# second-state/qwen3_asr_rs

Hardware: AMD Instinct MI355X
Metric: audio-seconds/sec (RTFx) Qwen3-ASR-0.6B greedy, 30s clips (higher is better)
Workload: dtype bf16; 1 GPU; Qwen3-ASR-0.6b bf16, batch=1 x 30s synthetic 16kHz clip per GPU, 100 new tokens (fixed, EOS ignored); clips_per_gpu=1, parallelism=dp1 (independent utterances per GPU, no data-path collective)

## Files before the change

qwen3_asr_rs_amd/build.py:

```python
from __future__ import annotations

import hashlib
import os
import re
import subprocess
import sys
from concurrent.futures import ThreadPoolExecutor

HERE = os.path.dirname(os.path.abspath(__file__))
ROOT = os.path.dirname(HERE)
CSRC = os.path.join(HERE, "csrc")
OBJ_DIR = os.path.join(ROOT, "build", "q3asr")
LIB_DIR = os.path.join(HERE, "lib")
LIB_PATH = os.path.join(LIB_DIR, "libq3asr_hip.so")
BIN_DIR = os.path.join(HERE, "bin")
CLI_PATH = os.path.join(BIN_DIR, "asr")

SOURCES = ["engine.cpp", "model.cpp", "k_gemm.hip", "k_mel.hip", "k_conv1.hip", "k_norm.hip", "k_attn.hip", "k_decode.hip", "k_gemv.hip", "k_dattn.hip", "k_fattn.hip", "k_skinny.hip", "k_gemm16.hip", "k_gemm256.hip", "k_peaks.hip", "k_align.hip",
           "host_audio.cpp", "host_text.cpp", "host_abi.cpp", "host_align.cpp", "group.cpp", "ops.cpp", "k_ops.hip"]
HEADERS = ["dev.h", "kernels.h", "argmax.h", "model.h", "json.h", "host.h", "ops.h", "unicode_tables.h", os.path.join("..", "..", "include", "q3asr.h"),
           os.path.join("..", "..", "include", "q3asr_ops.h")]
HIPCC = os.environ.get("HIPCC", "/opt/rocm/bin/hipcc")
FLAGS = ["--offload-arch=gfx950", "-O3", "-std=c++17", "-fPIC", "-fno-slp-vectorize", "-Wall", "-Wno-unused-function", "-Wno-unused-variable"]
HIP_FLAGS = ["-x", "hip", "-save-temps=obj"]

_VARIANT = os.environ.get("Q3A_BUILD_VARIANT", "")
if _VARIANT:
    FLAGS = FLAGS + os.environ.get("Q3A_BUILD_DEFINES", "").split()
    OBJ_DIR = OBJ_DIR + "_" + _VARIANT
    LIB_PATH = os.path.join(LIB_DIR, f"libq3asr_hip_{_VARIANT}.so")
    CLI_PATH = os.path.join(BIN_DIR, f"asr_{_VARIANT}")


def _hash(paths) -> str:
    h = hashlib.sha1()
    for p in paths:
        with open(p, "rb") as f:
            h.update(f.read())
    h.update(" ".join(FLAGS + HIP_FLAGS).encode())
    return h.hexdigest()


def have_hipcc() -> bool:
    return os.path.exists(HIPCC) and os.access(HIPCC, os.X_OK)


def _compile(src: str, hdr_hash: str, force: bool) -> str:
    spath = os.path.join(CSRC, src)
    obj = os.path.join(OBJ_DIR, src + ".o")
    stamp = obj + ".stamp"
    want = _hash([spath]) + hdr_hash
    is_hip = src.endswith(".hip")
    if not force and os.path.exists(obj) and os.path.exists(stamp) and open(stamp).read() == want and (not is_hip or os.path.exists(isa_path(src))):
        return obj
    cmd = [HIPCC] + FLAGS + (HIP_FLAGS if is_hip else []) + ["-c", spath, "-o", obj]
    r = subprocess.run(cmd, capture_output=True, text=True)
    if r.returncode != 0:
        raise RuntimeError(f"hipcc failed for {src}:\n{r.stdout}\n{r.stderr}")
    if r.stderr.strip():
        sys.stderr.write(r.stderr)
    with open(stamp, "w") as f:
        f.write(want)
    return obj


_LABEL = re.compile(r"^([A-Za-z_][\w$]*):")
_PK_F32 = re.compile(r"^\s*(v_pk_(?:mul|fma|add)_f32)\b.*\bop_sel:\[([01,]+)\]")


def isa_path(src: str) -> str:
    return os.path.join(OBJ_DIR, os.path.splitext(src)[0] + "-hip-amdgcn-amd-amdhsa-gfx950.s")


def scan_isa(paths=None):
    if paths is None:
        paths = [isa_path(s) for s in SOURCES if s.endswith(".hip")]
    found = []
    for path in paths:
        kernel = "?"
        if not os.path.exists(path):
            raise RuntimeError(f"scan_isa: {path} is missing -- rebuild (`python -m qwen3_asr_rs_amd.build`): the device assembly is kept by "
                               "-save-temps=obj and an object without it is treated as stale")
        with open(path) as f:
            for line in f:
                lm = _LABEL.match(line)
                if lm:
                    kernel = lm.group(1)
                m = _PK_F32.match(line)
                if m and "1" in m.group(2):
                    found.append((os.path.basename(path), kernel, line.strip()))
    return found


def build(force: bool = False, verbose: bool = True) -> str:
    os.makedirs(OBJ_DIR, exist_ok=True)
    os.makedirs(LIB_DIR, exist_ok=True)
    hdr_hash = _hash([os.path.join(CSRC, h) for h in HEADERS])
    with ThreadPoolExecutor(max_workers=min(8, len(SOURCES))) as ex:
        objs = list(ex.map(lambda s: _compile(s, hdr_hash, force), SOURCES))
    hazards = scan_isa()
    if hazards and os.environ.get("Q3A_ALLOW_ISA_HAZARD", "0") in ("", "0"):
        lines = "\n".join(f"  {f}: {k}: {i}" for f, k, i in hazards[:20])
        raise RuntimeError(f"{len(hazards)} packed fp32 instruction(s) with an op_sel bit set in the device code (csrc/dev.h: unsafe on gfx950; "
                           f"Q3A_ALLOW_ISA_HAZARD=1 builds experiment variants anyway):\n{lines}")
    link_stamp = LIB_PATH + ".stamp"
    want = _hash(objs)
    if force or not os.path.exists(LIB_PATH) or not os.path.exists(link_stamp) or open(link_stamp).read() != want:
        cmd = [HIPCC, "--offload-arch=gfx950", "-shared", "-fPIC", "-o", LIB_PATH] + objs + ["-ldl", "-lpthread"]
        r = subprocess.run(cmd, capture_output=True, text=True)
        if r.returncode != 0:
            raise RuntimeError(f"link failed:\n{r.stdout}\n{r.stderr}")
        with open(link_stamp, "w") as f:
            f.write(want)
        if verbose:
            print(f"[q3asr build] linked {LIB_PATH}")
    elif verbose:
        print(f"[q3asr build] up to date: {LIB_PATH}")
    os.makedirs(BIN_DIR, exist_ok=True)
    cli_src = os.path.join(CSRC, "asr_main.cpp")
    cli_stamp = CLI_PATH + ".stamp"
    cli_want = _hash([cli_src, os.path.join(ROOT, "include", "q3asr.h")]) + want
    if force or not os.path.exists(CLI_PATH) or not os.path.exists(cli_stamp) or open(cli_stamp).read() != cli_want:
        cmd = ["g++", "-O2", "-std=c++17", "-o", CLI_PATH, cli_src, "-L" + LIB_DIR, "-lq3asr_hip", "-Wl,-rpath,$ORIGIN/../lib",
               "-Wl,-rpath,/opt/rocm/lib"]
        r = subprocess.run(cmd, capture_output=True, text=True)
        if r.returncode != 0:
            raise RuntimeError(f"CLI link failed:\n{r.stdout}\n{r.stderr}")
        with open(cli_stamp, "w") as f:
            f.write(cli_want)
        if verbose:
            print(f"[q3asr build] linked {CLI_PATH}")
    return LIB_PATH


if __name__ == "__main__":
    build(force="--force" in sys.argv)
```

qwen3_asr_rs_amd/csrc/engine.cpp:

```cpp
#include <hip/hip_runtime.h>

#include <sched.h>

#include <algorithm>
#include <atomic>
#include <chrono>
#include <cmath>
#include <cstdio>
#include <cstring>
#include <map>
#include <memory>
#include <mutex>
#include <string>
#include <thread>
#include <vector>

#include "../../include/q3asr.h"
#include "kernels.h"
#include "model.h"

using namespace q3a;

namespace {

thread_local std::string g_last_error;

#define HIPCHK(expr)                                                                                    \
  do {                                                                                                  \
    hipError_t _e = (expr);                                                                             \
    if (_e != hipSuccess)                                                                               \
      fail(std::string("HIP error: ") + hipGetErrorString(_e) + " at " + __FILE__ + ":" + std::to_string(__LINE__) + " (" #expr ")"); \
  } while (0)
#define KCHK(expr)                                  \
  do {                                              \
    const char* _m = (expr);                        \
    if (_m) fail(std::string("kernel launch: ") + _m); \
  } while (0)

constexpr int kAudioPad = 151676, kEos0 = 151643, kEos1 = 151645;
constexpr int kGemvMaxSeq = 2;

struct DevBuf {
  void* p = nullptr;
  size_t cap = 0;
  bool grew = false;
  void ensure(size_t bytes) {
    if (bytes <= cap) return;
    if (p) (void)hipFree(p);
    p = nullptr;
    cap = 0;
    size_t want = (bytes + 255) & ~size_t(255);
    HIPCHK(hipMalloc(&p, want));
    cap = want;
    grew = true;
  }
  void release() {
    if (p) (void)hipFree(p);
    p = nullptr;
    cap = 0;
  }
  template <typename T> T* as() const { return reinterpret_cast<T*>(p); }
};

template <typename T>
void upload(DevBuf& b, const std::vector<T>& v, hipStream_t s) {
  b.ensure(std::max<size_t>(v.size() * sizeof(T), 16));
  if (!v.empty()) HIPCHK(hipMemcpyAsync(b.p, v.data(), v.size() * sizeof(T), hipMemcpyHostToDevice, s));
}

struct ProfEvent {
  int kclass;
  double bytes;
  hipEvent_t a, b;
};

}

namespace q3a {
void set_thread_error(const std::string& msg) { g_last_error = msg; }
}
namespace q3a {
Knobs& knobs() {
  static Knobs k;
  static std::once_flag once;
  std::call_once(once, [] {
    auto env = [](const char* name, std::atomic<int>& dst) { if (const char* e = getenv(name)) dst.store(atoi(e)); };
    env("Q3A_GEMM256_MIN_TILES", k.gemm256_min_tiles);
    env("Q3A_GEMM256_PERSIST", k.gemm256_persist);
    env("Q3A_GEMM256_GROUP_M", k.gemm256_group_m);
    env("Q3A_DATTN_BATCHED_MIN_WGS", k.dattn_batched_min_wgs);
    env("Q3A_DECODE_GROUP", k.decode_group_size);
    env("Q3A_DECODE_PARALLEL", k.decode_parallel_groups);
    env("Q3A_FUSE_QKROPE", k.fuse_qkrope);
    env("Q3A_SKINNY_Q", k.skinny_q);
    env("Q3A_EOS_RUN_AHEAD", k.eos_run_ahead);
    env("Q3A_SKINNY_GLU_HP3", k.skinny_glu_hp3);
    env("Q3A_LM_HEAD_PRUNE", k.lm_head_prune);
  });
  return k;
}
}

struct q3a_engine {
  Dims d;
  ArenaLayout L;
  q3a_opts opts{};
  int device = 0;
  hipStream_t stream = nullptr;
  uint8_t* arena = nullptr;
  bool own_arena = false;
  uint32_t arena_flags = 0;
  std::string err;

  DevBuf dft, filt_t, pos_emb, rope_cos, rope_sin;
  int rope_positions = 0;

  int B = 0;
  std::vector<int64_t> n_samples, pcm_off, mel_off;
  std::vector<int> n_frames, n_chunks, T, tok_off;
  int total_chunks = 0, total_T = 0, max_frames = 0;
  bool have_mel = false, have_enc = false, have_prefill = false;
  std::vector<int> P, seq_off;
  int total_P = 0, max_ctx = 0, max_new = 0;
  std::vector<AttnSeg> enc_segs_h;
  int enc_max_seg = 0;

  DevBuf pcm, d_pcm_off, d_n_samples, d_mel_off, d_n_frames, mel, gmax, d_chunk_utt, d_chunk_frame0;
  DevBuf conv1, conv2, conv3, conv3_rowmap, convout_rowmap;
  DevBuf enc_x, enc_ln, enc_qkv, enc_ctx, enc_ffn, enc_segs, audio_embeds;
  DevBuf ids, audio_rowmap, row_seq, row_pos, dec_segs, last_rows;
  DevBuf dec_x, dec_ln, dec_qkv, dec_ctx, dec_act, kcache, vcache;
  DevBuf x_dec, d_pos, next_tok, out_ids, step_count, done, s_ln, s_qkv, s_ctx, s_act, logits, forced_tok, part_val, part_idx;
  DevBuf blk_lo, blk_hi;
  DevBuf part_sum, out_lp;
  DevBuf lm_q, lm_qs;
  int lm_q_cols = 0;
  DevBuf prune_stats;
  DevBuf attn_pm, attn_pl, attn_po;
  DevBuf nn_x, nn_ss;
  DevBuf rope_cur;
  DevBuf enc_ctx16, dec_ctx16;
  DevBuf dec_q16;
  int n_cu = 256;
  DevBuf n_done;
  int* host_prog = nullptr;
  int* host_prog_dev = nullptr;
  DevBuf zero_page;
  int part_stride = 0, attn_nsplit = 0;
  size_t kv_layer_elems = 0;

  int gsize = 32;
  int k_parallel_groups = 1, k_skinny_q = 1, k_dattn_batched_min_wgs = 128, k_skinny_glu_hp3 = 1, k_lm_head_prune = 1;
  std::vector<hipStream_t> chain_streams;
  std::vector<hipEvent_t> join_ev;
  hipEvent_t fork_ev = nullptr;

  static constexpr size_t kGraphCacheMax = 16;
  std::vector<std::pair<std::string, hipGraphExec_t>> graph_cache;
  int pos_hi_ = 0, live_nsplit_ = 0;
  int min_P_ = 0;

  hipStream_t up_stream = nullptr;
  void* pin_p = nullptr;
  size_t pin_cap = 0;
  std::vector<hipEvent_t> up_ev;
  hipEvent_t up_t0 = nullptr, up_t1 = nullptr;
  q3a_io_timings io{};
  bool geom_valid = false;

  q3a_timings timings{};
  hipEvent_t ev[5] = {nullptr, nullptr, nullptr, nullptr, nullptr};
  std::vector<ProfEvent>* prof = nullptr;
  std::map<std::string, DevBuf> taps;
  std::map<std::string, size_t> tap_bytes;

  bool precise() const { return opts.precise != 0; }
  bool token_lp() const { return opts.token_logprobs != 0; }
  bool kv_f32() const { return opts.precise != 0; }
  size_t kv_elem() const { return kv_f32() ? 4 : 2; }
  size_t act_elem() const { return precise() ? 4 : 2; }
  template <typename T> const T* w(uint64_t off) const { return reinterpret_cast<const T*>(arena + off); }
  const float* wf(uint64_t off) const { return w<float>(off); }
  const uint16_t* wh(uint64_t off) const { return w<uint16_t>(off); }

  static bool light_tap(const char* name) { return strcmp(name, "dec_last_hidden") == 0 || strcmp(name, "head_in") == 0; }
  void tap(const char* name, const void* ptr, size_t bytes) {
    if (!opts.debug_taps || bytes == 0 || (opts.debug_taps == 2 && !light_tap(name))) return;
    DevBuf& t = taps[name];
    t.ensure(bytes);
    tap_bytes[name] = bytes;
    HIPCHK(hipMemcpyAsync(t.p, ptr, bytes, hipMemcpyDeviceToDevice, stream));
  }
  void tap_act(const char* name, const void* ptr, size_t elems) {
    if (!opts.debug_taps || elems == 0 || opts.debug_taps == 2) return;
    if (precise()) return tap(name, ptr, elems * 4);
    DevBuf& t = taps[name];
    t.ensure(elems * 4);
    tap_bytes[name] = elems * 4;
    KCHK(launch_from_bf16((const uint16_t*)ptr, t.as<float>(), elems, stream));
  }

  void act_gemm(const DevBuf& x, int lda, const uint16_t* W, int M, int N, int K, const GemmEpilogue& ep, bool glu) {
    if (precise()) KCHK(launch_gemm(x.as<float>(), lda, W, M, N, K, ep, glu, true, stream));
    else KCHK(launch_gemm16(x.as<uint16_t>(), lda, W, M, N, K, ep, glu, stream));
  }
  void act_conv(const DevBuf& x, int imgs, int H, int Wd, int C, const uint16_t* W, int Cout, const GemmEpilogue& ep) {
    if (precise()) KCHK(launch_conv3x3s2_gemm(x.as<float>(), imgs, H, Wd, C, W, Cout, ep, true, stream));
    else KCHK(launch_conv3x3s2_gemm16(x.as<uint16_t>(), zero_page.as<uint16_t>(), imgs, H, Wd, C, W, Cout, ep, stream));
  }
  void act_out(GemmEpilogue& ep, const DevBuf& buf) const {
    if (precise()) ep.out = buf.as<float>(); else ep.out16 = buf.as<uint16_t>();
  }
  uint16_t* act16(const DevBuf& buf) const { return precise() ? nullptr : buf.as<uint16_t>(); }

  template <class F> void timed(int kclass, double bytes, F&& fn) {
    if (!prof) {
      fn();
      return;
    }
    ProfEvent pe{kclass, bytes, nullptr, nullptr};
    HIPCHK(hipEventCreate(&pe.a));
    HIPCHK(hipEventCreate(&pe.b));
    HIPCHK(hipEventRecord(pe.a, stream));
    fn();
    HIPCHK(hipEventRecord(pe.b, stream));
    prof->push_back(pe);
  }

  void init_common(const std::string& model_dir, int dev, const q3a_opts* o) {
    if (o) opts = *o; else q3a_opts_default(&opts);
    if (opts.max_new_tokens <= 0) opts.max_new_tokens = 4096;
    d = parse_config_file(model_dir + "/config.json");
    validate_dims(d);
    L = plan_arena(d);
    device = dev;
    int n_dev = 0;
    hipError_t e = hipGetDeviceCount(&n_dev);
    if (e != hipSuccess || n_dev == 0)
      fail("no HIP device available: libq3asr_hip has no CPU fallback (hipGetDeviceCount: " + std::string(hipGetErrorString(e)) + ")");
    if (dev < 0 || dev >= n_dev) fail("device index out of range");
    HIPCHK(hipSetDevice(dev));
    KCHK(skinny_init());
    (void)hipDeviceGetAttribute(&n_cu, hipDeviceAttributeMultiprocessorCount, dev);
    HIPCHK(hipStreamCreateWithFlags(&stream, hipStreamNonBlocking));
    for (auto& x : ev) HIPCHK(hipEventCreate(&x));
    HIPCHK(hipHostMalloc((void**)&host_prog, 64, hipHostMallocMapped));
    memset(host_prog, 0, 64);
    HIPCHK(hipHostGetDevicePointer((void**)&host_prog_dev, host_prog, 0));
    n_done.ensure(64);
    prune_stats.ensure(8);
    HIPCHK(hipMemsetAsync(prune_stats.p, 0, 8, stream));
  }

  void init_tables() {
    auto dftm = make_dft_matrix(400, 416);
    auto filt = make_mel_filterbank_T(d.n_mels, 400, 16000, 202);
    auto pe = make_sinusoid_rows(d.tokens_per_chunk(), d.enc_d);
    upload(dft, dftm, stream);
    upload(filt_t, filt, stream);
    upload(pos_emb, pe, stream);
    zero_page.ensure(256);
    HIPCHK(hipMemsetAsync(zero_page.p, 0, 256, stream));
    ensure_rope(8192);
    HIPCHK(hipStreamSynchronize(stream));
  }

  void ensure_rope(int n_pos) {
    if (n_pos <= rope_positions) return;
    int n = std::max(n_pos, 8192);
    std::vector<float> c, s;
    make_rope_tables(n, d.head_dim, d.rope_theta, c, s);
    HIPCHK(hipStreamSynchronize(stream));
    upload(rope_cos, c, stream);
    upload(rope_sin, s, stream);
    HIPCHK(hipStreamSynchronize(stream));
    rope_positions = n;
  }

  void init_lm_head_q() {
    const int cols = lm_head_q_cols(d.hidden);
    if (precise() || d.aligner() || cols == 0 || d.hidden % 8 != 0) return;
    lm_q.ensure((size_t)d.vocab * cols);
    lm_qs.ensure((size_t)d.vocab * 16);
    KCHK(launch_lm_head_quantize(wh(L.lm_head), d.vocab, d.hidden, lm_q.as<int8_t>(), lm_qs.as<float>(), stream));
    HIPCHK(hipStreamSynchronize(stream));
    lm_q_cols = cols;
  }

  void check_arena_header() {
    ArenaHeader h;
    HIPCHK(hipMemcpy(&h, arena, sizeof(h), hipMemcpyDeviceToHost));
    if (h.magic != kArenaMagic || h.version != kArenaVersion) fail("weight arena: bad magic/version");
    if (h.total_bytes != L.total) fail("weight arena: size does not match config.json");
    arena_flags = h.flags;
  }

  void set_batch(const int64_t* ns, int b) {
    have_mel = have_enc = have_prefill = false;
    if (b <= 0) { B = 0; fail("batch must be >= 1"); }
    if (geom_valid && b == B && (int)n_samples.size() == b && std::equal(ns, ns + b, n_samples.begin())) return;
    geom_valid = false;
    B = 0;
    for (int u = 0; u < b; ++u)
      if (ns[u] < 161) fail("utterance too short: reflection padding needs more than 160 samples (src/mel.rs:63-65)");
    n_samples.assign(ns, ns + b);
    pcm_off.resize(b); mel_off.resize(b); n_frames.resize(b); n_chunks.resize(b); T.resize(b); tok_off.resize(b);
    std::vector<int> chunk_utt, chunk_frame0, convout_map, conv3_map;
    enc_segs_h.clear();
    int64_t po = 0, mo = 0;
    int tok = 0;
    total_chunks = 0; max_frames = 0; enc_max_seg = 0;
    const int cf = d.chunk_frames(), tpc = d.tokens_per_chunk(), cpw = d.chunks_per_window();
    for (int u = 0; u < b; ++u) {
      pcm_off[u] = po;
      po += (ns[u] + 3) & ~int64_t(3);
      int F = (int)((ns[u] + 159) / 160);
      n_frames[u] = F;
      max_frames = std::max(max_frames, F);
      mel_off[u] = mo;
      mo += (int64_t)F * d.n_mels;
      int nc = (F + cf - 1) / cf;
      n_chunks[u] = nc;
      tok_off[u] = tok;
      std::vector<int> valid(nc);
      for (int c = 0; c < nc; ++c) {
        int frames = std::min(cf, F - c * cf);
        valid[c] = Dims::feat_len(frames);
        chunk_utt.push_back(u);
        chunk_frame0.push_back(c * cf);
        for (int t = 0; t < tpc; ++t) convout_map.push_back(t < valid[c] ? tok + t : -1);
        tok += valid[c];
      }
      T[u] = tok - tok_off[u];
      int t0 = tok_off[u];
      if (nc <= cpw) {
        enc_segs_h.push_back(AttnSeg{t0, T[u], (int64_t)t0 * 3 * d.enc_d});
        enc_max_seg = std::max(enc_max_seg, T[u]);
      } else {
        for (int c0 = 0; c0 < nc; c0 += cpw) {
          int len = 0;
          for (int c = c0; c < std::min(nc, c0 + cpw); ++c) len += valid[c];
          enc_segs_h.push_back(AttnSeg{t0, len, (int64_t)t0 * 3 * d.enc_d});
          enc_max_seg = std::max(enc_max_seg, len);
          t0 += len;
        }
      }
      total_chunks += nc;
    }
    total_T = tok;
    const int f3 = d.freq3();
    conv3_map.resize((size_t)total_chunks * f3 * tpc);
    for (int c = 0; c < total_chunks; ++c)
      for (int f = 0; f < f3; ++f)
        for (int t = 0; t < tpc; ++t) conv3_map[((size_t)c * f3 + f) * tpc + t] = (c * tpc + t) * f3 + f;
    pcm.ensure((size_t)po * 4);
    upload(d_pcm_off, pcm_off, stream);
    upload(d_n_samples, n_samples, stream);
    upload(d_mel_off, mel_off, stream);
    upload(d_n_frames, n_frames, stream);
    upload(d_chunk_utt, chunk_utt, stream);
    upload(d_chunk_frame0, chunk_frame0, stream);
    upload(convout_rowmap, convout_map, stream);
    upload(conv3_rowmap, conv3_map, stream);
    upload(enc_segs, enc_segs_h, stream);
    mel.ensure((size_t)mo * 4);
    gmax.ensure((size_t)b * 4);
    HIPCHK(hipStreamSynchronize(stream));
    B = b;
    geom_valid = true;
  }

  void upload_pcm(const float* host, const int64_t* ns, int b) {
    set_batch(ns, b);
    int64_t src = 0;
    for (int u = 0; u < b; ++u) {
      HIPCHK(hipMemcpyAsync(pcm.as<float>() + pcm_off[u], host + src, (size_t)ns[u] * 4, hipMemcpyHostToDevice, stream));
      src += ns[u];
    }
    HIPCHK(hipStreamSynchronize(stream));
  }

  void upload_ptrs_and_mel(const float* const* ptrs, const int64_t* ns, int b) {
    const auto w0 = std::chrono::steady_clock::now();
    set_batch(ns, b);
    static const int mode = [] { const char* e = getenv("Q3A_UPLOAD_MODE"); return e ? atoi(e) : 1; }();
    static const int thr_env = [] { const char* e = getenv("Q3A_UPLOAD_THREADS"); return e ? atoi(e) : -1; }();
    static const int pieces_env = [] { const char* e = getenv("Q3A_UPLOAD_PIECES"); return e ? atoi(e) : 8; }();
    io = q3a_io_timings{};
    io.mode = mode;
    HIPCHK(hipEventRecord(ev[0], stream));
    const size_t total = (size_t)(pcm_off[b - 1] + ((ns[b - 1] + 3) & ~int64_t(3))) * 4;
    bool staged = mode != 0;
    if (staged && total > pin_cap) {
      if (up_stream) HIPCHK(hipStreamSynchronize(up_stream));
      if (pin_p) (void)hipHostFree(pin_p);
      pin_p = nullptr; pin_cap = 0;
      const size_t want = (total + (size_t(1) << 20) - 1) & ~((size_t(1) << 20) - 1);
      if (hipHostMalloc(&pin_p, want, hipHostMallocDefault) == hipSuccess && pin_p) pin_cap = want;
      else { (void)hipGetLastError(); pin_p = nullptr; staged = false; io.mode = 0; }
    }
    if (!staged) {
      for (int u = 0; u < b; ++u)
        HIPCHK(hipMemcpyAsync(pcm.as<float>() + pcm_off[u], ptrs[u], (size_t)ns[u] * 4, hipMemcpyHostToDevice, stream));
      HIPCHK(hipStreamSynchronize(stream));
// ... 104 lines not shown
    ChunkTable ct{d_chunk_utt.as<int>(), d_chunk_frame0.as<int>()};
    KCHK(launch_conv1(mel.as<float>(), d_mel_off.as<int64_t>(), d_n_frames.as<int>(), ct, total_chunks, d.n_mels,
                      d.chunk_frames(), wf(L.conv1_w), wf(L.conv1_b), C, conv1.as<float>(), stream, act16(conv1)));
    tap_act("conv1", conv1.p, nch * H1 * W1 * C);
    {
      GemmEpilogue ep;
      act_out(ep, conv2); ep.ldo = C; ep.bias = wf(L.conv2_b); ep.act = 1;
      act_conv(conv1, total_chunks, H1, W1, C, wh(L.conv2_w), C, ep);
      tap_act("conv2", conv2.p, nch * H2 * W2 * C);
    }
    {
      GemmEpilogue ep;
      act_out(ep, conv3); ep.ldo = C; ep.bias = wf(L.conv3_b); ep.act = 1; ep.rowmap = conv3_rowmap.as<int>();
      act_conv(conv2, total_chunks, H2, W2, C, wh(L.conv3_w), C, ep);
      tap_act("conv3", conv3.p, nch * H3 * W3 * C);
    }
    {
      GemmEpilogue ep;
      ep.out = enc_x.as<float>(); ep.ldo = D;
      ep.bias = (arena_flags & kFlagConvOutBias) ? wf(L.conv_out_b) : nullptr;
      ep.rowmap = convout_rowmap.as<int>();
      ep.addend = pos_emb.as<float>(); ep.addend_period = W3;
      act_gemm(conv3, H3 * C, wh(L.conv_out_w), total_chunks * W3, D, H3 * C, ep, false);
      tap("enc_in", enc_x.p, Tt * D * 4);
    }
    AttnArgs at{};
    at.q = enc_qkv.as<float>(); at.q_rs = 3 * D;
    at.k = enc_qkv.as<float>() + D; at.v = enc_qkv.as<float>() + 2 * D; at.kv_hs = 64; at.kv_rs = 3 * D;
    if (qkv16) {
      at.q16 = enc_qkv.as<uint16_t>();
      at.k = enc_qkv.as<uint16_t>() + D; at.v = enc_qkv.as<uint16_t>() + 2 * D;
    }
    at.o = enc_ctx.as<float>(); at.o_rs = D;
    at.o16 = valu_attn ? nullptr : enc_ctx.as<uint16_t>();
    at.segs = enc_segs.as<AttnSeg>(); at.n_segs = (int)enc_segs_h.size(); at.max_len = enc_max_seg;
    at.n_kv_heads = d.enc_heads; at.scale_div = 8.0f;
    const DevBuf& ctx_in = (valu_attn && !sp) ? enc_ctx16 : enc_ctx;
    for (int li = 0; li < d.enc_layers; ++li) {
      const EncLayerOff& e = L.enc[li];
      KCHK(launch_layernorm(enc_x.as<float>(), wf(e.ln1_w), wf(e.ln1_b), enc_ln.as<float>(), total_T, D, 1e-5f, stream, act16(enc_ln)));
      {
        GemmEpilogue ep; ep.ldo = 3 * D; ep.bias = wf(e.qkv_b);
        if (qkv16) ep.out16 = enc_qkv.as<uint16_t>(); else ep.out = enc_qkv.as<float>();
        act_gemm(enc_ln, D, wh(e.qkv_w), total_T, 3 * D, D, ep, false);
      }
      if (valu_attn) {
        KCHK(launch_attn_enc(at, stream));
        if (!sp) KCHK(launch_to_bf16(enc_ctx.as<float>(), enc_ctx16.as<uint16_t>(), Tt * D, stream));
      } else {
        KCHK(launch_fattn_enc(at, stream));
      }
      {
        GemmEpilogue ep; ep.out = enc_x.as<float>(); ep.ldo = D; ep.bias = wf(e.out_b); ep.resid = enc_x.as<float>();
        act_gemm(ctx_in, D, wh(e.out_w), total_T, D, D, ep, false);
      }
      KCHK(launch_layernorm(enc_x.as<float>(), wf(e.ln2_w), wf(e.ln2_b), enc_ln.as<float>(), total_T, D, 1e-5f, stream, act16(enc_ln)));
      {
        GemmEpilogue ep; act_out(ep, enc_ffn); ep.ldo = Fn; ep.bias = wf(e.fc1_b); ep.act = 1;
        act_gemm(enc_ln, D, wh(e.fc1_w), total_T, Fn, D, ep, false);
      }
      {
        GemmEpilogue ep; ep.out = enc_x.as<float>(); ep.ldo = D; ep.bias = wf(e.fc2_b); ep.resid = enc_x.as<float>();
        act_gemm(enc_ffn, Fn, wh(e.fc2_w), total_T, D, Fn, ep, false);
      }
      if (li == 0) tap("enc_layer0", enc_x.p, Tt * D * 4);
      static const bool enc_layer_taps = [] { const char* e = getenv("Q3A_DEBUG_LAYER_TAPS"); return e && atoi(e) != 0; }();
      if (enc_layer_taps && opts.debug_taps == 1) {
        char name[32];
        snprintf(name, sizeof(name), "E%02d_x", li);
        tap(name, enc_x.p, Tt * D * 4);
      }
    }
    tap("enc_last", enc_x.p, Tt * D * 4);
    KCHK(launch_layernorm(enc_x.as<float>(), wf(L.ln_post_w), wf(L.ln_post_b), enc_ln.as<float>(), total_T, D, 1e-5f, stream, act16(enc_ln)));
    {
      GemmEpilogue ep; act_out(ep, enc_ffn); ep.ldo = D; ep.bias = wf(L.proj1_b); ep.act = 1;
      act_gemm(enc_ln, D, wh(L.proj1_w), total_T, D, D, ep, false);
    }
    {
      GemmEpilogue ep; ep.out = audio_embeds.as<float>(); ep.ldo = d.enc_out; ep.bias = wf(L.proj2_b);
      act_gemm(enc_ffn, D, wh(L.proj2_w), total_T, d.enc_out, D, ep, false);
    }
    tap("audio_embeds", audio_embeds.p, Tt * d.enc_out * 4);
    HIPCHK(hipGetLastError());
    have_enc = true;
  }

  void setup_prompts(const int32_t* ids_h, const int32_t* lens, int b, int max_new_req, bool before_encoder = false) {
    if (!have_enc && !before_encoder) fail("q3a_prefill: no encoder output (call q3a_encode first)");
    if (b != B) fail("q3a_prefill: batch size differs from the encoded batch");
    P.assign(lens, lens + b);
    seq_off.resize(b);
    std::vector<int> rowseq, rowpos, amap((size_t)total_T, -1), last(b);
    int off = 0, maxP = 0;
    for (int s = 0; s < b; ++s) {
      seq_off[s] = off;
      int na = 0;
      for (int i = 0; i < P[s]; ++i) {
        rowseq.push_back(s);
        rowpos.push_back(i);
        int id = ids_h[off + i];
        if (id < 0 || id >= d.vocab) fail("q3a_prefill: token id out of range");
        if (id == kAudioPad) {
          if (na >= T[s]) fail("q3a_prefill: more <|audio_pad|> tokens than encoder tokens");
          amap[(size_t)tok_off[s] + na] = off + i;
          ++na;
        }
      }
      if (na != T[s]) fail("q3a_prefill: number of <|audio_pad|> tokens does not match the encoder output length");
      if (P[s] <= 0) fail("q3a_prefill: empty prompt");
      last[s] = off + P[s] - 1;
      off += P[s];
      maxP = std::max(maxP, P[s]);
    }
    total_P = off;
    max_new = std::min(std::max(max_new_req, 1), opts.max_new_tokens);
    max_ctx = ((maxP + max_new + 1 + 127) / 128) * 128;
    pos_hi_ = maxP;
    min_P_ = *std::min_element(P.begin(), P.end());
    {
      static const int pad = [] { const char* e = getenv("Q3A_CTX_PAD"); return e ? atoi(e) : 0; }();
      if (pad > 0) max_ctx += (pad + 127) / 128 * 128;
    }
    ensure_rope(max_ctx + 1);
    std::vector<int> ids_v(ids_h, ids_h + total_P);
    std::vector<AttnSeg> segs(b);
    for (int s = 0; s < b; ++s)
      segs[s] = AttnSeg{seq_off[s], P[s], (int64_t)s * d.n_kv * max_ctx * 128};
    upload(ids, ids_v, stream);
    upload(row_seq, rowseq, stream);
    upload(row_pos, rowpos, stream);
    upload(audio_rowmap, amap, stream);
    upload(last_rows, last, stream);
    upload(dec_segs, segs, stream);
    upload(d_pos, P, stream);
    const size_t Pt = (size_t)total_P, H = d.hidden;
    const bool valu_attn = kv_f32() || opts.valu_attention;
    dec_x.ensure(Pt * H * 4); dec_ln.ensure(Pt * H * act_elem()); dec_qkv.ensure(Pt * d.qkv_dim() * 4);
    dec_ctx.ensure(Pt * d.q_dim() * (valu_attn ? 4 : act_elem())); dec_act.ensure(Pt * d.inter * act_elem());
    if (!valu_attn) dec_q16.ensure(Pt * d.q_dim() * 2);
    if (valu_attn && !precise()) dec_ctx16.ensure(Pt * d.q_dim() * 2);
    kv_layer_elems = (size_t)b * d.n_kv * max_ctx * 128;
    kcache.ensure(kv_layer_elems * d.dec_layers * kv_elem());
    vcache.ensure(kv_layer_elems * d.dec_layers * kv_elem());
    rope_cur.ensure((size_t)b * 128 * 4);
    {
      Knobs& kn = knobs();
      const int gs = kn.decode_group_size.load();
      gsize = (gs >= 1 && gs <= 32) ? gs : 32;
      k_parallel_groups = kn.decode_parallel_groups.load(); k_skinny_q = kn.skinny_q.load();
      k_dattn_batched_min_wgs = kn.dattn_batched_min_wgs.load();
      k_skinny_glu_hp3 = kn.skinny_glu_hp3.load();
      k_lm_head_prune = kn.lm_head_prune.load();
    }
    const size_t ng = (size_t)n_groups(b);
    nn_x.ensure(ng * 32 * H * 2); nn_ss.ensure((size_t)ng * (H / 8) * 32 * 4);
    x_dec.ensure((size_t)b * H * 4); next_tok.ensure((size_t)b * 4); forced_tok.ensure((size_t)b * 4);
    out_ids.ensure((size_t)b * max_new * 4); step_count.ensure((size_t)b * 4); done.ensure((size_t)b);
    s_ln.ensure((size_t)b * H * 4); s_qkv.ensure((size_t)b * d.qkv_dim() * 4); s_ctx.ensure(ng * 32 * d.q_dim() * 4);
    s_act.ensure(ng * 32 * d.inter * 4); logits.ensure((size_t)b * d.vocab * 4);
    part_stride = std::max(128, (d.vocab + 3) / 4);
    part_val.ensure((size_t)b * part_stride * 4); part_idx.ensure((size_t)b * part_stride * 4);
    if (token_lp()) { part_sum.ensure((size_t)b * part_stride * 4); out_lp.ensure((size_t)b * max_new * 4); }
    {
      const size_t nblk4 = ((size_t)(d.vocab + 15) / 16 + 3) & ~size_t(3);
      blk_lo.ensure(nblk4 * 4); blk_hi.ensure(nblk4 * 4);
    }
    attn_nsplit = (max_ctx + dattn_keys_per_split(kv_f32()) - 1) / dattn_keys_per_split(kv_f32());
    attn_pm.ensure((size_t)b * d.n_q * attn_nsplit * 4); attn_pl.ensure((size_t)b * d.n_q * attn_nsplit * 4);
    attn_po.ensure((size_t)b * d.n_q * attn_nsplit * 128 * 4);
    HIPCHK(hipMemsetAsync(step_count.p, 0, (size_t)b * 4, stream));
    HIPCHK(hipMemsetAsync(done.p, 0, (size_t)b, stream));
    HIPCHK(hipMemsetAsync(n_done.p, 0, 64, stream));
    HIPCHK(hipMemsetAsync(out_ids.p, 0, (size_t)b * max_new * 4, stream));
    if (token_lp()) HIPCHK(hipMemsetAsync(out_lp.p, 0, (size_t)b * max_new * 4, stream));
    HIPCHK(hipStreamSynchronize(stream));
    for (auto cs : chain_streams) HIPCHK(hipStreamSynchronize(cs));
    __atomic_store_n(&host_prog[0], 0, __ATOMIC_RELAXED);
    __atomic_store_n(&host_prog[1], 0, __ATOMIC_RELAXED);
    drain_retired_graphs();
    {
      bool any = false;
      for (auto* sb : step_bufs()) { any = any || sb->grew; sb->grew = false; }
      if (any) drop_graphs();
    }
  }

  std::vector<DevBuf*> step_bufs() {
    return {&kcache, &vcache, &x_dec, &d_pos, &next_tok, &out_ids, &step_count, &done, &s_ln, &s_qkv, &s_ctx, &s_act, &logits,
            &part_val, &part_idx, &part_sum, &out_lp, &blk_lo, &blk_hi, &prune_stats, &attn_pm, &attn_pl, &attn_po, &nn_x, &nn_ss, &rope_cur, &rope_cos, &rope_sin, &n_done, &forced_tok};
  }
  std::vector<const DevBuf*> step_bufs() const {
    auto v = const_cast<q3a_engine*>(this)->step_bufs();
    return std::vector<const DevBuf*>(v.begin(), v.end());
  }

  void* kc_layer(int l) { return (uint8_t*)kcache.p + (size_t)l * kv_layer_elems * kv_elem(); }
  void* vc_layer(int l) { return (uint8_t*)vcache.p + (size_t)l * kv_layer_elems * kv_elem(); }

  LmHeadPruneArgs prune_args(const GemvArgs& g) {
    LmHeadPruneArgs pa{};
    pa.g = g; pa.Wq = lm_q.as<int8_t>(); pa.qcols = lm_q_cols; pa.qs = lm_qs.as<float>();
    pa.blk_lo = blk_lo.as<float>(); pa.blk_hi = blk_hi.as<float>(); pa.stats = prune_stats.as<int>();
    return pa;
  }

  void run_head(int advance) {
    const int S = B, H = d.hidden, V = d.vocab;
    tap("head_in", x_dec.p, (size_t)S * H * 4);
    const double wbytes = 2.0 * V * H;
    int n_part = 0;
    const ArgmaxPartials part{part_val.as<float>(), part_idx.as<int>(), token_lp() ? part_sum.as<float>() : nullptr, part_stride};
    if (S <= kGemvMaxSeq) {
      GemvArgs g{};
      g.fast_math = precise() ? 0 : 1;
      g.x = x_dec.as<float>(); g.ldx = H; g.rms_w = wf(L.final_norm); g.eps = d.rms_eps;
      g.W = wh(L.lm_head); g.N = V; g.K = H; g.mode = 3; g.out = logits.as<float>(); g.ldo = V;
      g.part = part;
      LmHeadPruneArgs pa{};
      const bool prunable = S == 1 && !precise() && lm_q_cols > 0 && (pa = prune_args(g), !lm_head_prune_check(pa));
      if (prunable && opts.debug_taps == 1) {
        DevBuf& t = taps["lm_head_bound"];
        t.ensure((size_t)V * 8);
        tap_bytes["lm_head_bound"] = (size_t)V * 8;
        LmHeadPruneArgs pd = pa;
        pd.dbg = t.as<float>(); pd.stats = nullptr;
        KCHK(launch_lm_head_approx(pd, stream));
      }
      if (prunable && k_lm_head_prune && !head_logits_) {
        g.out = nullptr; pa.g.out = nullptr;
        n_part = lm_head_rescore_groups(g, n_cu);
        timed(Q3A_KC_GEMV_LM_HEAD, (double)V * lm_q_cols, [&] { KCHK(launch_lm_head_approx(pa, stream)); });
        timed(Q3A_KC_ARGMAX, 0, [&] { KCHK(launch_lm_head_rescore(pa, n_part, stream)); });
      } else {
        n_part = gemv_blocks(g);
        timed(Q3A_KC_GEMV_LM_HEAD, wbytes, [&] { KCHK(launch_gemv(g, S, stream)); });
      }
    } else if (!precise()) {
      timed(Q3A_KC_NORM, 0, [&] { KCHK(launch_rmsnorm(x_dec.as<float>(), wf(L.final_norm), s_ln.as<float>(), S, H, d.rms_eps, stream, s_ln.as<uint16_t>())); });
      GemmEpilogue ep; ep.out = logits.as<float>(); ep.ldo = V;
      if (S <= 32 && V % 4 == 0 && H % 64 == 0 && part_stride >= (V + 63) / 64) {
        ep.part = part;
        if (!head_logits_) ep.out = nullptr;
        n_part = (V + 63) / 64;
        timed(Q3A_KC_GEMM, wbytes, [&] { KCHK(launch_gemm16(s_ln.as<uint16_t>(), H, wh(L.lm_head), S, V, H, ep, false, stream)); });
      } else {
        timed(Q3A_KC_GEMM, wbytes, [&] { KCHK(launch_gemm16(s_ln.as<uint16_t>(), H, wh(L.lm_head), S, V, H, ep, false, stream)); });
        n_part = 128;
        timed(Q3A_KC_ARGMAX, 0, [&] { KCHK(launch_argmax_partials(logits.as<float>(), V, S, part, n_part, stream)); });
      }
    } else {
      timed(Q3A_KC_NORM, 0, [&] { KCHK(launch_rmsnorm(x_dec.as<float>(), wf(L.final_norm), s_ln.as<float>(), S, H, d.rms_eps, stream)); });
      timed(Q3A_KC_GEMM, wbytes, [&] { batched_proj(s_ln.as<float>(), H, wh(L.lm_head), V, H, nullptr, 0, logits.as<float>(), V, nullptr); });
      n_part = 128;
      timed(Q3A_KC_ARGMAX, 0, [&] { KCHK(launch_argmax_partials(logits.as<float>(), V, S, part, n_part, stream)); });
    }
    FinalizeArgs f{};
    f.part = part; f.n_part = n_part; f.out_lp = part.sum ? out_lp.as<float>() : nullptr;
    f.V = V; f.next_tok = next_tok.as<int>(); f.out_ids = out_ids.as<int>();
    f.out_stride = max_new; f.step_count = step_count.as<int>(); f.pos = d_pos.as<int>(); f.advance = advance;
    f.done = done.as<uint8_t>(); f.n_done = n_done.as<int>(); f.n_seq = S; f.host_progress = host_prog_dev; f.embed = wh(L.embed); f.H = H; f.x_next = x_dec.as<float>(); f.eos0 = kEos0; f.eos1 = kEos1;
    f.cos_t = rope_cos.as<float>(); f.sin_t = rope_sin.as<float>(); f.rope_cur = rope_cur.as<float>();
    f.nn = first_layer_norm_out();
    timed(Q3A_KC_ARGMAX, 0, [&] { KCHK(launch_argmax_finalize(f, S, stream)); });
  }

  void run_prefill() {
    run_prefill_layers();
    const int H = d.hidden;
    KCHK(launch_gather_rows(dec_x.as<float>(), last_rows.as<int>(), B, H, x_dec.as<float>(), stream));
    tap("dec_last_hidden", x_dec.p, (size_t)B * H * 4);
    run_head(0);
    tap("logits", logits.p, (size_t)B * d.vocab * 4);
    HIPCHK(hipGetLastError());
    have_prefill = true;
  }

  void run_prefill_layers() {
    const int H = d.hidden, I = d.inter, QD = d.q_dim(), QKV = d.qkv_dim();
    const bool sp = precise();
    KCHK(launch_embed(ids.as<int>(), total_P, wh(L.embed), H, kAudioPad, dec_x.as<float>(), stream));
    scatter_audio_rows();
    tap("dec_embed", dec_x.p, (size_t)total_P * H * 4);
    AttnArgs at{};
    at.q = dec_qkv.as<float>(); at.q_rs = QKV; at.kv_hs = (int64_t)max_ctx * 128; at.kv_rs = 128;
    at.o = dec_ctx.as<float>(); at.o_rs = QD; at.segs = dec_segs.as<AttnSeg>(); at.n_segs = B;
    at.max_len = *std::max_element(P.begin(), P.end()); at.n_kv_heads = d.n_kv;
    at.scale_div = sqrtf((float)d.head_dim);
    const bool valu_attn = kv_f32() || opts.valu_attention;
    at.o16 = valu_attn ? nullptr : dec_ctx.as<uint16_t>();
    if (!valu_attn) { at.q16 = dec_q16.as<uint16_t>(); at.q_rs = QD; }
    const DevBuf& ctx_in = (valu_attn && !sp) ? dec_ctx16 : dec_ctx;
    const bool qkv_bias = arena_flags & kFlagDecQkvBias, o_bias = arena_flags & kFlagDecOBias, mlp_bias = arena_flags & kFlagDecMlpBias;
    const bool fuse_rope = knobs().fuse_qkrope.load() != 0 && !valu_attn && !precise() && d.head_dim == 128 && gemm256_eligible(total_P, QKV, H) && H % 64 == 0;
    for (int li = 0; li < d.dec_layers; ++li) {
      const DecLayerOff& l = L.dec[li];
      KCHK(launch_rmsnorm(dec_x.as<float>(), wf(l.in_ln), dec_ln.as<float>(), total_P, H, d.rms_eps, stream, act16(dec_ln)));
      RopeKvArgs rk{};
      rk.qkv = dec_qkv.as<float>(); rk.row_seq = row_seq.as<int>(); rk.row_pos = row_pos.as<int>();
      rk.q_norm = wf(l.q_norm); rk.k_norm = wf(l.k_norm); rk.eps = d.rms_eps;
      rk.cos_t = rope_cos.as<float>(); rk.sin_t = rope_sin.as<float>();
      rk.kcache = kc_layer(li); rk.vcache = vc_layer(li); rk.n_q = d.n_q; rk.n_kv = d.n_kv; rk.max_ctx = max_ctx;
      rk.q16 = valu_attn ? nullptr : dec_q16.as<uint16_t>();
      if (fuse_rope) {
        KCHK(launch_gemm256_qkrope(dec_ln.as<uint16_t>(), H, wh(l.qkv_w), total_P, H, qkv_bias ? wf(l.qkv_b) : nullptr, rk, stream));
      } else {
        GemmEpilogue ep; ep.out = dec_qkv.as<float>(); ep.ldo = QKV; ep.bias = qkv_bias ? wf(l.qkv_b) : nullptr;
        act_gemm(dec_ln, H, wh(l.qkv_w), total_P, QKV, H, ep, false);
        KCHK(launch_qknorm_rope_kv(rk, total_P, kv_f32(), stream));
      }
      at.k = kc_layer(li); at.v = vc_layer(li);
      static const bool layer_taps = [] { const char* e = getenv("Q3A_DEBUG_LAYER_TAPS"); return e && atoi(e) != 0; }();
      auto ltap = [&](const char* what, const void* ptr, size_t bytes) {
        if (!layer_taps || !opts.debug_taps) return;
        char name[32];
        snprintf(name, sizeof(name), "L%02d_%s", li, what);
        tap(name, ptr, bytes);
      };
      const size_t act_b = sp ? 4 : 2;
      if (fuse_rope) {
        ltap("qkvs", dec_qkv.p, std::min((size_t)1024, (size_t)total_P) * QKV * 4);
      }
      ltap("k", kc_layer(li), (size_t)B * d.n_kv * max_ctx * 128 * kv_elem());
      ltap("v", vc_layer(li), (size_t)B * d.n_kv * max_ctx * 128 * kv_elem());
      if (valu_attn) {
        KCHK(launch_attn_prefill(at, d.n_q / d.n_kv, kv_f32(), stream));
        if (!sp) KCHK(launch_to_bf16(dec_ctx.as<float>(), dec_ctx16.as<uint16_t>(), (size_t)total_P * QD, stream));
      } else {
        KCHK(launch_fattn_prefill(at, d.n_q / d.n_kv, stream));
      }
      ltap("attn", ctx_in.p, (size_t)total_P * QD * act_b);
      {
        GemmEpilogue ep; ep.out = dec_x.as<float>(); ep.ldo = H; ep.resid = dec_x.as<float>(); ep.bias = o_bias ? wf(l.o_b) : nullptr;
        act_gemm(ctx_in, QD, wh(l.o_w), total_P, H, QD, ep, false);
      }
      ltap("o", dec_x.p, (size_t)total_P * H * 4);
      KCHK(launch_rmsnorm(dec_x.as<float>(), wf(l.post_ln), dec_ln.as<float>(), total_P, H, d.rms_eps, stream, act16(dec_ln)));
      ltap("ln2", dec_ln.p, (size_t)total_P * H * act_b);
      {
        GemmEpilogue ep; act_out(ep, dec_act); ep.ldo = I; ep.bias = mlp_bias ? wf(l.gu_b) : nullptr;
        act_gemm(dec_ln, H, wh(l.gu_w), total_P, 2 * I, H, ep, true);
      }
      ltap("act", dec_act.p, (size_t)total_P * I * act_b);
      {
        GemmEpilogue ep; ep.out = dec_x.as<float>(); ep.ldo = H; ep.resid = dec_x.as<float>(); ep.bias = mlp_bias ? wf(l.down_b) : nullptr;
        act_gemm(dec_act, I, wh(l.down_w), total_P, H, I, ep, false);
      }
      ltap("x", dec_x.p, (size_t)total_P * H * 4);
      if (li == 0) tap("dec_layer0", dec_x.p, (size_t)total_P * H * 4);
    }
  }

  void require_asr(const char* what) const {
    if (d.aligner()) fail(std::string(what) + ": this engine holds a forced aligner (classify_num in config.json); use q3a_align*");
  }
  void require_aligner(const char* what) const {
    if (!d.aligner()) fail(std::string(what) + ": not a forced-aligner checkpoint (config.json has no thinker_config.classify_num)");
  }
  std::vector<int> align_marker_rows(const int32_t* ids_h, const int32_t* lens, int b, int stride, int32_t* counts) const {
    std::vector<int> rows;
    int off = 0;
    for (int s = 0; s < b; ++s) {
      int n = 0;
      for (int i = 0; i < lens[s]; ++i)
        if (ids_h[off + i] == d.timestamp_token_id) { rows.push_back(off + i); ++n; }
      if (n > stride)
        fail("q3a_align: utterance " + std::to_string(s) + " has " + std::to_string(n) + " timestamp markers, more than stride " + std::to_string(stride));
      counts[s] = n;
      off += lens[s];
    }
    return rows;
  }
  void run_align(const std::vector<int>& rows, const int32_t* counts, int stride, int32_t* out_classes, float* logits_out) {
    const int M = (int)rows.size(), N = d.classify_num, H = d.hidden;
    have_prefill = false;
    HIPCHK(hipEventRecord(ev[2], stream));
    run_prefill_layers();
    HIPCHK(hipEventRecord(ev[3], stream));
    if (M > 0) {
      upload(align_rows, rows, stream);
      const int planes = precise() ? 2 : 1, n_part = align_head_parts(N);
      align_xn.ensure((size_t)planes * align_rows_padded(M) * H * 2);
      align_pval.ensure((size_t)M * n_part * 4); align_pidx.ensure((size_t)M * n_part * 4);
      align_cls.ensure((size_t)M * 4);
      if (logits_out) align_logits.ensure((size_t)M * N * 4);
      AlignHeadArgs a{};
      a.x = dec_x.as<float>(); a.ldx = H; a.rows = align_rows.as<int>(); a.M = M;
      a.norm_w = wf(L.final_norm); a.eps = d.rms_eps; a.W = wh(L.lm_head); a.N = N; a.K = H;
      a.planes = planes; a.xn = align_xn.as<uint16_t>();
      a.part = ArgmaxPartials{align_pval.as<float>(), align_pidx.as<int>(), nullptr, n_part};
      a.classes = align_cls.as<int>();
      a.logits = logits_out ? align_logits.as<float>() : nullptr; a.ldl = N;
      KCHK(launch_align_head(a, stream));
    }
    HIPCHK(hipEventRecord(ev[4], stream));
    HIPCHK(hipStreamSynchronize(stream));
    HIPCHK(hipGetLastError());
    std::vector<int> cls((size_t)M);
    if (M > 0) HIPCHK(hipMemcpy(cls.data(), align_cls.p, (size_t)M * 4, hipMemcpyDeviceToHost));
    if (M > 0 && logits_out) HIPCHK(hipMemcpy(logits_out, align_logits.p, (size_t)M * N * 4, hipMemcpyDeviceToHost));
    for (int s = 0, k = 0; s < B; ++s)
      for (int i = 0; i < counts[s]; ++i) out_classes[(size_t)s * stride + i] = cls[k++];
    float ms = 0.f;
    HIPCHK(hipEventElapsedTime(&ms, ev[2], ev[4])); timings.prefill_ms = ms;
    HIPCHK(hipEventElapsedTime(&ms, ev[3], ev[4])); align_head_ms = ms;
    timings.decode_ms = 0.f; timings.decode_steps = 0; timings.batch = B; timings.total_audio_tokens = total_T;
    timings.total_prompt_tokens = total_P;
  }
  DevBuf align_rows, align_xn, align_pval, align_pidx, align_cls, align_logits;
  float align_head_ms = 0.f;

  void scatter_audio_rows();

  bool prenorm_path() const { return B > kGemvMaxSeq && !precise(); }
  bool skinny_q() const {
    auto whole = [](int K) { const int st = K / 32, per = (st + 7) / 8, unr = per <= 2 ? 2 : per <= 4 ? 4 : per <= 8 ? 8 : 12; return K % 256 == 0 && per % unr == 0; };
// ... 9 lines not shown
  float* s_act_g(int g) const { return s_act.as<float>() + (size_t)g * 32 * d.inter; }
  NextNormOut first_layer_norm_out() const {
    NextNormOut nn{};
    if (prenorm_path()) {
      nn.next_w = wf(L.dec[0].in_ln); nn.next_xw16f = nn_x.as<uint16_t>(); nn.next_ss = nn_ss.as<float>(); nn.nparts = nn_parts();
      nn.group_stride_x = (long)nn_x_stride(); nn.group_stride_ss = (long)nn_ss_stride(); nn.group_size = gsize;
    }
    return nn;
  }

  void batched_proj(const float* x, int ldx, const uint16_t* W, int N, int K, const float* bias, int mode, float* out,
                    int ldo, const float* resid) {
    const int S = B;
    if (S <= 32) {
      SkinnyArgs sk{};
      sk.fast_math = precise() ? 0 : 1;
      sk.x = x; sk.ldx = ldx; sk.S = S; sk.W = W; sk.N = N; sk.K = K; sk.bias = bias; sk.mode = mode; sk.out = out; sk.ldo = ldo; sk.resid = resid;
      KCHK(launch_skinny(sk, precise(), stream));
    } else {
      GemmEpilogue ep; ep.out = out; ep.ldo = ldo; ep.bias = bias; ep.resid = (mode == 1) ? resid : nullptr;
      KCHK(launch_gemm(x, ldx, W, S, N, K, ep, mode == 2, precise(), stream));
    }
  }

  void decode_layer(int li, int grp, int s0, int S, hipStream_t ks) {
    const int H = d.hidden, I = d.inter, QD = d.q_dim(), QKV = d.qkv_dim();
    const bool qkv_bias = arena_flags & kFlagDecQkvBias, o_bias = arena_flags & kFlagDecOBias, mlp_bias = arena_flags & kFlagDecMlpBias;
    const bool gemv = B <= kGemvMaxSeq;
    const DecLayerOff& l = L.dec[li];
    float* const x = x_dec.as<float>() + (size_t)s0 * H;
    float* const qkv = s_qkv.as<float>() + (size_t)s0 * QKV;
    const size_t kv_seq = (size_t)d.n_kv * max_ctx * 128 * kv_elem();
    DecodeAttnArgs da{};
    da.qkv = qkv; da.pos = d_pos.as<int>() + s0; da.eps = d.rms_eps;
    da.rope_cur = rope_cur.as<float>() + (size_t)s0 * 128;
    da.pm = attn_pm.as<float>() + (size_t)s0 * d.n_q * attn_nsplit; da.pl = attn_pl.as<float>() + (size_t)s0 * d.n_q * attn_nsplit;
    da.po = attn_po.as<float>() + (size_t)s0 * d.n_q * attn_nsplit * 128; da.nsplit = live_nsplit_;
    da.n_q = d.n_q; da.n_kv = d.n_kv; da.max_ctx = max_ctx; da.scale_div = sqrtf((float)d.head_dim);
    da.q_norm = wf(l.q_norm); da.k_norm = wf(l.k_norm);
    da.kcache = (uint8_t*)kc_layer(li) + (size_t)s0 * kv_seq; da.vcache = (uint8_t*)vc_layer(li) + (size_t)s0 * kv_seq;
    if (gemv) {
      GemvArgs g{};
      g.fast_math = precise() ? 0 : 1;
      g.x = x; g.ldx = H; g.rms_w = wf(l.in_ln); g.eps = d.rms_eps; g.W = wh(l.qkv_w); g.N = QKV; g.K = H;
      g.bias = qkv_bias ? wf(l.qkv_b) : nullptr; g.mode = 0; g.out = qkv; g.ldo = QKV;
      timed(Q3A_KC_GEMV, 2.0 * QKV * H, [&] { KCHK(launch_gemv(g, S, ks)); });
      timed(Q3A_KC_DECODE_ATTN, 0, [&] { KCHK(launch_decode_attn(da, S, kv_f32(), ks)); });
      GemvArgs o{};
      o.fast_math = precise() ? 0 : 1;
      if (std::min(S, 4) * d.n_q * live_nsplit_ <= GEMV_ATTN_MAX_TABLE) {
        o.attn_pm = da.pm; o.attn_pl = da.pl; o.attn_po = da.po;
        o.attn_nsplit = live_nsplit_; o.attn_heads = d.n_q; o.attn_fast_exp = precise() ? 0 : 1;
      } else {
        timed(Q3A_KC_DECODE_ATTN, 0, [&] { KCHK(launch_attn_combine(da.pm, da.pl, da.po, live_nsplit_, S, d.n_q, s_ctx_g(grp), ks)); });
        o.x = s_ctx_g(grp);
      }
      o.ldx = QD; o.W = wh(l.o_w); o.N = H; o.K = QD; o.bias = o_bias ? wf(l.o_b) : nullptr;
      o.mode = 1; o.out = x; o.ldo = H; o.resid = x;
      timed(Q3A_KC_GEMV_O, 2.0 * H * QD, [&] { KCHK(launch_gemv(o, S, ks)); });
      GemvArgs u{};
      u.fast_math = precise() ? 0 : 1;
      u.x = x; u.ldx = H; u.rms_w = wf(l.post_ln); u.eps = d.rms_eps; u.W = wh(l.gu_w); u.N = 2 * I; u.K = H;
      u.bias = mlp_bias ? wf(l.gu_b) : nullptr; u.mode = 2; u.out = s_act_g(grp); u.ldo = I;
      timed(Q3A_KC_GEMV, 4.0 * I * H, [&] { KCHK(launch_gemv(u, S, ks)); });
      GemvArgs dn{};
      dn.fast_math = precise() ? 0 : 1;
      dn.x = s_act_g(grp); dn.ldx = I; dn.W = wh(l.down_w); dn.N = H; dn.K = I; dn.bias = mlp_bias ? wf(l.down_b) : nullptr;
      dn.mode = 1; dn.out = x; dn.ldo = H; dn.resid = x;
      timed(Q3A_KC_GEMV_DOWN, 2.0 * H * I, [&] { KCHK(launch_gemv(dn, S, ks)); });
      return;
    }
    const bool b16 = !precise(), pre = prenorm_path();
    SkinnyArgs q{};
    q.fast_math = precise() ? 0 : 1;
    q.x = x; q.ldx = H; q.S = S; q.eps = d.rms_eps; q.W = wh(l.qkv_w); q.N = QKV; q.K = H;
    if (pre) { q.xw16f = nn_x_g(grp); q.ss_parts = nn_ss_g(grp); q.ss_nparts = nn_parts(); }
    else q.rms_w = wf(l.in_ln);
    q.bias = qkv_bias ? wf(l.qkv_b) : nullptr; q.mode = 0; q.out = qkv; q.ldo = QKV;
    timed(Q3A_KC_GEMM, 2.0 * QKV * H, [&] { KCHK(launch_skinny(q, precise(), ks)); });
    if (S * d.n_kv >= k_dattn_batched_min_wgs) {
      if (b16) { da.out16 = reinterpret_cast<uint16_t*>(s_ctx_g(grp)); da.out_frag = 1; } else da.out = s_ctx_g(grp);
      da.trim_prologue = min_P_ < 2 * 128;
      timed(Q3A_KC_DECODE_ATTN, 0, [&] { KCHK(launch_decode_attn_batched(da, S, kv_f32(), ks)); });
    } else {
      timed(Q3A_KC_DECODE_ATTN, 0, [&] { KCHK(launch_decode_attn(da, S, kv_f32(), ks)); });
      timed(Q3A_KC_DECODE_ATTN, 0, [&] { KCHK(launch_attn_combine(da.pm, da.pl, da.po, live_nsplit_, S, d.n_q, s_ctx_g(grp), ks, b16 ? reinterpret_cast<uint16_t*>(s_ctx_g(grp)) : nullptr, b16)); });
    }
    SkinnyArgs o{};
    o.fast_math = precise() ? 0 : 1;
    o.x = s_ctx_g(grp); o.x16 = b16 ? reinterpret_cast<uint16_t*>(s_ctx_g(grp)) : nullptr; o.x16_frag = b16; o.ldx = QD; o.S = S; o.W = wh(l.o_w); o.N = H; o.K = QD;
    o.bias = o_bias ? wf(l.o_b) : nullptr; o.mode = 1; o.out = x; o.ldo = H; o.resid = x;
    if (pre) { o.next_w = wf(l.post_ln); o.next_xw16f = nn_x_g(grp); o.next_ss = nn_ss_g(grp); }
    o.qsplit = b16 && skinny_q();
    timed(Q3A_KC_GEMM, 2.0 * H * QD, [&] { KCHK(launch_skinny(o, precise(), ks)); });
    SkinnyArgs u{};
    u.fast_math = precise() ? 0 : 1;
    u.x = x; u.ldx = H; u.S = S; u.eps = d.rms_eps; u.W = wh(l.gu_w); u.N = 2 * I; u.K = H;
    if (pre) { u.xw16f = nn_x_g(grp); u.ss_parts = nn_ss_g(grp); u.ss_nparts = nn_parts(); }
    else u.rms_w = wf(l.post_ln);
    u.bias = mlp_bias ? wf(l.gu_b) : nullptr; u.mode = 2; u.out = s_act_g(grp); u.out16 = b16 ? reinterpret_cast<uint16_t*>(s_act_g(grp)) : nullptr; u.out16_frag = b16; u.ldo = I;
    u.n_cu = n_cu;
    u.glu_hp3 = k_skinny_glu_hp3;
    timed(Q3A_KC_GEMM, 4.0 * I * H, [&] { KCHK(launch_skinny(u, precise(), ks)); });
    SkinnyArgs dn{};
    dn.fast_math = precise() ? 0 : 1;
    dn.x = s_act_g(grp); dn.x16 = b16 ? reinterpret_cast<uint16_t*>(s_act_g(grp)) : nullptr; dn.x16_frag = b16; dn.ldx = I; dn.S = S; dn.W = wh(l.down_w); dn.N = H; dn.K = I;
    dn.bias = mlp_bias ? wf(l.down_b) : nullptr; dn.mode = 1; dn.out = x; dn.ldo = H; dn.resid = x;
    dn.qsplit = b16 && skinny_q();
    if (pre && li + 1 < d.dec_layers) {
      dn.next_w = wf(L.dec[li + 1].in_ln); dn.next_xw16f = nn_x_g(grp); dn.next_ss = nn_ss_g(grp);
    }
    timed(Q3A_KC_GEMM, 2.0 * H * I, [&] { KCHK(launch_skinny(dn, precise(), ks)); });
  }

  void enqueue_decode_step() {
    const int ng = n_groups(B);
    const bool chains = ng > 1 && !prof && k_parallel_groups != 0;
    if (chains) {
      ensure_chain_streams(ng - 1);
      HIPCHK(hipEventRecord(fork_ev, stream));
    }
    for (int g = 0; g < ng; ++g) {
      const int s0 = ng == 1 ? 0 : g * gsize;
      const int S = ng == 1 ? B : std::min(gsize, B - s0);
      hipStream_t ks = (chains && g > 0) ? chain_streams[g - 1] : stream;
      if (chains && g > 0) HIPCHK(hipStreamWaitEvent(ks, fork_ev, 0));
      for (int li = 0; li < d.dec_layers; ++li) decode_layer(li, g, s0, S, ks);
      if (chains && g > 0) {
        HIPCHK(hipEventRecord(join_ev[g - 1], ks));
        HIPCHK(hipStreamWaitEvent(stream, join_ev[g - 1], 0));
      }
    }
    run_head(1);
  }
  void ensure_chain_streams(int n) {
    while ((int)chain_streams.size() < n) {
      hipStream_t s2;
      hipEvent_t e2;
      HIPCHK(hipStreamCreateWithFlags(&s2, hipStreamNonBlocking));
      HIPCHK(hipEventCreateWithFlags(&e2, hipEventDisableTiming));
      chain_streams.push_back(s2);
      join_ev.push_back(e2);
    }
    if (!fork_ev) HIPCHK(hipEventCreateWithFlags(&fork_ev, hipEventDisableTiming));
  }

  std::string make_graph_sig() const {
    uint64_t h = 1469598103934665603ull;
    for (const DevBuf* sb : step_bufs()) {
      uint64_t v = (uint64_t)(uintptr_t)sb->p;
      for (int i = 0; i < 8; ++i) { h ^= (v >> (8 * i)) & 0xff; h *= 1099511628211ull; }
    }
    char buf[256];
    snprintf(buf, sizeof(buf), "%d.%d.%d.%d.%d.%d.%d.%d.%d.%d/%d/%d/%d/%p/%016llx", B, gsize, k_parallel_groups, k_skinny_q,
             k_dattn_batched_min_wgs, k_skinny_glu_hp3, k_lm_head_prune, (int)(min_P_ < 256), (int)head_logits_, (int)token_lp(), live_nsplit_,
             max_ctx, max_new, (const void*)arena, (unsigned long long)h);
    return buf;
  }

  bool uses_key_splits() const {
    if (B <= kGemvMaxSeq) return true;
    const int ng = n_groups(B);
    const int smallest = ng == 1 ? B : std::min(gsize, B - (ng - 1) * gsize);
    return smallest * d.n_kv < k_dattn_batched_min_wgs;
  }
  hipGraphExec_t graph_for_step() {
    const std::string sig = make_graph_sig();
    for (size_t i = 0; i < graph_cache.size(); ++i)
      if (graph_cache[i].first == sig) {
        if (i + 1 != graph_cache.size()) std::rotate(graph_cache.begin() + i, graph_cache.begin() + i + 1, graph_cache.end());
        return graph_cache.back().second;
      }
    hipGraph_t g = nullptr;
    hipGraphExec_t exec = nullptr;
    HIPCHK(hipStreamBeginCapture(stream, hipStreamCaptureModeThreadLocal));
    try {
      enqueue_decode_step();
    } catch (...) {
      hipGraph_t tmp = nullptr;
      (void)hipStreamEndCapture(stream, &tmp);
      if (tmp) (void)hipGraphDestroy(tmp);
      throw;
    }
    HIPCHK(hipStreamEndCapture(stream, &g));
    const hipError_t ie = hipGraphInstantiate(&exec, g, nullptr, nullptr, 0);
    (void)hipGraphDestroy(g);
    HIPCHK(ie);
    if (graph_cache.size() >= kGraphCacheMax) {
      retired_graphs.push_back(graph_cache.front().second);
      graph_cache.erase(graph_cache.begin());
    }
    graph_cache.emplace_back(sig, exec);
    return exec;
  }
  std::vector<hipGraphExec_t> retired_graphs;
  void drain_retired_graphs() {
    for (auto ge : retired_graphs) (void)hipGraphExecDestroy(ge);
    retired_graphs.clear();
  }
  void drop_graphs() {
    drain_retired_graphs();
    for (auto& ge : graph_cache) (void)hipGraphExecDestroy(ge.second);
    graph_cache.clear();
  }

  void decode_steps(int n) {
    if (!have_prefill) fail("decode: no prefill state");
    if (n <= 0) return;
    const bool eager = !opts.use_graph || prof;
    const int kps = dattn_keys_per_split(kv_f32());
    for (int i = 0; i < n; ++i) {
      live_nsplit_ = uses_key_splits() ? std::min(attn_nsplit, pos_hi_ / kps + 1) : attn_nsplit;
      if (eager) enqueue_decode_step();
      else HIPCHK(hipGraphLaunch(graph_for_step(), stream));
      ++pos_hi_;
    }
    if (eager) HIPCHK(hipGetLastError());
  }

  void prepare_prompts(const int32_t* lang_ids, int n_prefix, int max_new_req, int fixed_new) {
    if (B <= 0) fail("q3a_run_resident: no batch uploaded");
    if (fixed_new > 0) max_new_req = fixed_new;
    if (max_new_req <= 0) max_new_req = opts.max_new_tokens;
    std::vector<int32_t> ids_v, lens(B);
    for (int s = 0; s < B; ++s) {
      int32_t len = 0;
      q3a_build_prompt(T[s], lang_ids, n_prefix, nullptr, &len);
      size_t o = ids_v.size();
      ids_v.resize(o + len);
      q3a_build_prompt(T[s], lang_ids, n_prefix, ids_v.data() + o, &len);
      lens[s] = len;
    }
    setup_prompts(ids_v.data(), lens.data(), B, max_new_req, true);
  }

  void run_resident(int fixed_new, bool mel_enqueued = false) {
    if (B <= 0) fail("q3a_run_resident: no batch uploaded");
    if (!mel_enqueued) {
      HIPCHK(hipEventRecord(ev[0], stream));
      run_mel();
      HIPCHK(hipEventRecord(ev[1], stream));
    }
    run_encoder();
    HIPCHK(hipEventRecord(ev[2], stream));
    run_prefill();
    HIPCHK(hipEventRecord(ev[3], stream));
    int steps = 0;
    static const bool host_timing = [] { const char* e = getenv("Q3A_DEBUG_HOST_TIMING"); return e && atoi(e) != 0; }();
    const auto h0 = std::chrono::steady_clock::now();
    if (fixed_new > 0) {
      steps = fixed_new - 1;
      decode_steps(steps);
      if (host_timing) fprintf(stderr, "[q3a host timing] %d graph launches enqueued in %.1f us\n", steps,
                               std::chrono::duration<double, std::micro>(std::chrono::steady_clock::now() - h0).count());
    } else {
      const int ahead = std::max(1, knobs().eos_run_ahead.load());
      const int limit = max_new - 1;
      unsigned spins = 0;
      while (steps < limit) {
        if (__atomic_load_n(&host_prog[1], __ATOMIC_RELAXED)) break;
        const int fin = __atomic_load_n(&host_prog[0], __ATOMIC_RELAXED);
        if (steps - std::max(fin - 1, 0) < ahead) {
          decode_steps(1);
          ++steps;
          spins = 0;
        } else if (++spins > 64) {
          sched_yield();
          if ((spins & 0xffff) == 0) {
            const hipError_t q = hipStreamQuery(stream);
            if (q != hipSuccess && q != hipErrorNotReady) HIPCHK(q);
            if (q == hipSuccess && steps - std::max(__atomic_load_n(&host_prog[0], __ATOMIC_RELAXED) - 1, 0) >= ahead)
              fail("greedy loop: the stream drained but the device-side progress counter did not advance");
          }
        }
      }
    }
    HIPCHK(hipEventRecord(ev[4], stream));
    HIPCHK(hipStreamSynchronize(stream));
    HIPCHK(hipGetLastError());
    float ms;
    HIPCHK(hipEventElapsedTime(&ms, ev[0], ev[1])); timings.mel_ms = ms;
    HIPCHK(hipEventElapsedTime(&ms, ev[1], ev[2])); timings.encoder_ms = ms;
    HIPCHK(hipEventElapsedTime(&ms, ev[2], ev[3])); timings.prefill_ms = ms;
    HIPCHK(hipEventElapsedTime(&ms, ev[3], ev[4])); timings.decode_ms = ms;
    HIPCHK(hipEventElapsedTime(&ms, ev[0], ev[4])); timings.total_ms = ms;
    timings.decode_steps = steps; timings.batch = B; timings.total_audio_tokens = total_T; timings.total_prompt_tokens = total_P;
  }

  void fetch_ids(int32_t* out, int stride, int32_t* out_lens) {
    if (!have_prefill) fail("q3a_fetch_ids: nothing generated");
    std::vector<int> all((size_t)B * max_new);
    HIPCHK(hipMemcpy(all.data(), out_ids.p, all.size() * 4, hipMemcpyDeviceToHost));
    generated_lens(all, out_lens);
    for (int s = 0; s < B; ++s)
      for (int i = 0; i < std::min(out_lens[s], stride); ++i) out[(size_t)s * stride + i] = all[(size_t)s * max_new + i];
  }
  void generated_lens(const std::vector<int>& all, int32_t* out_lens) {
    std::vector<int> sc(B);
    HIPCHK(hipMemcpy(sc.data(), step_count.p, (size_t)B * 4, hipMemcpyDeviceToHost));
    for (int s = 0; s < B; ++s) {
      int n = std::min(sc[s], max_new), len = 0;
      for (; len < n; ++len) {
        int t = all[(size_t)s * max_new + len];
        if (!fixed_mode_ && (t == kEos0 || t == kEos1)) break;
      }
      out_lens[s] = len;
    }
  }
// ... 368 lines not shown
  for (int u = 0; u < B; ++u)
    if (!pcm16k[u]) fail("q3a_transcribe_batch: null utterance pointer");
  const auto w0 = std::chrono::steady_clock::now();
  HIPCHK(hipSetDevice(e->device));
  e->fixed_mode_ = fixed_new_tokens > 0;
  e->head_logits_ = e->opts.debug_taps != 0;
  e->set_batch(n_samples, B);
  e->prepare_prompts(lang_prefix_ids, n_prefix, max_new, fixed_new_tokens);
  e->upload_ptrs_and_mel(pcm16k, n_samples, B);
  e->run_resident(fixed_new_tokens, true);
  e->fetch_ids(out_ids, stride, out_lens);
  if (e->io.mode != 0) {
    float ms = 0.f;
    if (hipEventSynchronize(e->up_t1) != hipSuccess || hipEventElapsedTime(&ms, e->up_t0, e->up_t1) != hipSuccess) { (void)hipGetLastError(); ms = 0.f; }
    e->io.h2d_ms = ms;
  }
  e->io.wall_ms = std::chrono::duration<float, std::milli>(std::chrono::steady_clock::now() - w0).count();
  Q3A_CATCH(e)
}

int32_t q3a_transcribe_batch(q3a_engine* e, const float* pcm16k, const int64_t* n_samples, int32_t B,
                             const int32_t* lang_prefix_ids, int32_t n_prefix, int32_t max_new, int32_t fixed_new_tokens,
                             int32_t* out_ids, int32_t stride, int32_t* out_lens) {
  if (!e) return 1;
  if (e->d.aligner()) {
    e->err = g_last_error = "q3a_transcribe_batch: this engine holds a forced aligner (classify_num in config.json); use q3a_align*";
    return 1;
  }
  if (!pcm16k || !n_samples || B < 1) { e->err = "q3a_transcribe_batch: bad argument"; return 1; }
  std::vector<const float*> ptrs((size_t)B);
  int64_t off = 0;
  for (int u = 0; u < B; ++u) { ptrs[u] = pcm16k + off; off += n_samples[u]; }
  return q3a_transcribe_batch_ptrs(e, ptrs.data(), n_samples, B, lang_prefix_ids, n_prefix, max_new, fixed_new_tokens, out_ids, stride, out_lens);
}

int32_t q3a_io_timings_last(const q3a_engine* e, q3a_io_timings* out) {
  if (!e || !out) return 1;
  *out = e->io;
  return 0;
}

int32_t q3a_stage_timings(const q3a_engine* e, q3a_timings* out) {
  if (!e || !out) return 1;
  *out = e->timings;
  return 0;
}

int32_t q3a_profile_decode_step(q3a_engine* e, q3a_kernel_profile* out) {
  if (!e || !out) return 1;
  Q3A_TRY(e)
  HIPCHK(hipSetDevice(e->device));
  if (!e->have_prefill) fail("q3a_profile_decode_step: no decode state");
  std::vector<ProfEvent> evs;
  e->prof = &evs;
  try {
    e->decode_steps(1);
    HIPCHK(hipStreamSynchronize(e->stream));
  } catch (...) {
    e->prof = nullptr;
    throw;
  }
  e->prof = nullptr;
  memset(out, 0, sizeof(*out));
  for (auto& pe : evs) {
    float ms = 0.f;
    HIPCHK(hipEventElapsedTime(&ms, pe.a, pe.b));
    out->total_us[pe.kclass] += ms * 1000.f;
    out->launches[pe.kclass] += 1;
    out->weight_bytes[pe.kclass] += pe.bytes;
    (void)hipEventDestroy(pe.a);
    (void)hipEventDestroy(pe.b);
  }
  Q3A_CATCH(e)
}

int32_t q3a_profile_weight_stream(q3a_engine* e, int32_t reps, float* avg_us, double* bytes_per_launch, int32_t* launches) {
  if (!e) return 1;
  Q3A_TRY(e)
  HIPCHK(hipSetDevice(e->device));
  if (!e->have_prefill) fail("q3a_profile_weight_stream: no decode state");
  if (e->B > kGemvMaxSeq) fail("q3a_profile_weight_stream: the GEMV path serves at most 2 sequences");
  if (reps < 1) reps = 1;
  const Dims& d = e->d;
  const int S = e->B, H = d.hidden, I = d.inter, QKV = d.qkv_dim();
  auto sweep = [&]() {
    for (int li = 0; li < d.dec_layers; ++li) {
      const DecLayerOff& l = e->L.dec[li];
      GemvArgs g{};
      g.fast_math = e->precise() ? 0 : 1;
      g.x = e->x_dec.as<float>(); g.ldx = H; g.rms_w = e->wf(l.in_ln); g.eps = d.rms_eps; g.W = e->wh(l.qkv_w); g.N = QKV; g.K = H;
      g.mode = 0; g.out = e->s_qkv.as<float>(); g.ldo = QKV;
      KCHK(launch_gemv(g, S, e->stream));
      GemvArgs u{};
      u.fast_math = e->precise() ? 0 : 1;
      u.x = e->x_dec.as<float>(); u.ldx = H; u.rms_w = e->wf(l.post_ln); u.eps = d.rms_eps; u.W = e->wh(l.gu_w); u.N = 2 * I; u.K = H;
      u.mode = 2; u.out = e->s_act.as<float>(); u.ldo = I;
      KCHK(launch_gemv(u, S, e->stream));
    }
  };
  hipGraph_t g = nullptr;
  hipGraphExec_t ge = nullptr;
  HIPCHK(hipStreamBeginCapture(e->stream, hipStreamCaptureModeThreadLocal));
  try {
    for (int r = 0; r < reps; ++r) sweep();
  } catch (...) {
    hipGraph_t tmp = nullptr;
    (void)hipStreamEndCapture(e->stream, &tmp);
    if (tmp) (void)hipGraphDestroy(tmp);
    throw;
  }
  HIPCHK(hipStreamEndCapture(e->stream, &g));
  HIPCHK(hipGraphInstantiate(&ge, g, nullptr, nullptr, 0));
  (void)hipGraphDestroy(g);
  HIPCHK(hipGraphLaunch(ge, e->stream));
  HIPCHK(hipStreamSynchronize(e->stream));
  hipEvent_t a, b;
  HIPCHK(hipEventCreate(&a));
  HIPCHK(hipEventCreate(&b));
  float ms = 0.f;
  constexpr int kReplays = 3;
  for (int rep = 0; rep < kReplays; ++rep) {
    HIPCHK(hipEventRecord(a, e->stream));
    HIPCHK(hipGraphLaunch(ge, e->stream));
    HIPCHK(hipEventRecord(b, e->stream));
    HIPCHK(hipStreamSynchronize(e->stream));
    float t = 0.f;
    HIPCHK(hipEventElapsedTime(&t, a, b));
    ms += t / kReplays;
  }
  HIPCHK(hipGetLastError());
  (void)hipEventDestroy(a);
  (void)hipEventDestroy(b);
  (void)hipGraphExecDestroy(ge);
  const int n = reps * d.dec_layers * 2;
  if (avg_us) *avg_us = ms * 1000.f / (float)n;
  if (bytes_per_launch) *bytes_per_launch = (2.0 * QKV * H + 4.0 * I * H) / 2.0;
  if (launches) *launches = n;
  Q3A_CATCH(e)
}

int32_t q3a_debug_read(q3a_engine* e, const char* name, void* dst, uint64_t bytes, uint64_t* actual) {
  if (!e) return 1;
  Q3A_TRY(e)
  HIPCHK(hipSetDevice(e->device));
  if (strcmp(name, "lm_head_prune_stats") == 0) {
    if (actual) *actual = 8;
    if (dst) {
      if (bytes < 8) fail("q3a_debug_read: destination too small");
      HIPCHK(hipStreamSynchronize(e->stream));
      HIPCHK(hipMemcpy(dst, e->prune_stats.p, 8, hipMemcpyDeviceToHost));
    }
    return 0;
  }
  if (strcmp(name, "align_head_ms") == 0) {
    if (actual) *actual = 4;
    if (dst) {
      if (bytes < 4) fail("q3a_debug_read: destination too small");
      memcpy(dst, &e->align_head_ms, 4);
    }
    return 0;
  }
  auto it = e->taps.find(name);
  if (it == e->taps.end()) fail(std::string("q3a_debug_read: no tap named '") + name + "' (opts.debug_taps set?)");
  size_t n = e->tap_bytes[name];
  if (actual) *actual = n;
  if (dst) {
    if (bytes < n) fail("q3a_debug_read: destination too small");
    HIPCHK(hipStreamSynchronize(e->stream));
    HIPCHK(hipMemcpy(dst, it->second.p, n, hipMemcpyDeviceToHost));
  }
  Q3A_CATCH(e)
}

int32_t q3a_debug_set(const char* key, int32_t value) {
  if (!key) return 1;
  Knobs& kn = knobs();
  if (strcmp(key, "gemm256_min_tiles") == 0) { kn.gemm256_min_tiles = value; return 0; }
  if (strcmp(key, "gemm256_persist") == 0) { kn.gemm256_persist = value; return 0; }
  if (strcmp(key, "gemm256_group_m") == 0) { kn.gemm256_group_m = value; return 0; }
  if (strcmp(key, "dattn_batched_min_wgs") == 0) { kn.dattn_batched_min_wgs = value; return 0; }
  if (strcmp(key, "decode_group_size") == 0) { kn.decode_group_size = value; return 0; }
  if (strcmp(key, "decode_parallel_groups") == 0) { kn.decode_parallel_groups = value; return 0; }
  if (strcmp(key, "fuse_qkrope") == 0) { kn.fuse_qkrope = value; return 0; }
  if (strcmp(key, "skinny_q") == 0) { kn.skinny_q = value; return 0; }
  if (strcmp(key, "eos_run_ahead") == 0) { kn.eos_run_ahead = value; return 0; }
  if (strcmp(key, "skinny_glu_hp3") == 0) { kn.skinny_glu_hp3 = value; return 0; }
  if (strcmp(key, "lm_head_prune") == 0) { kn.lm_head_prune = value; return 0; }
  g_last_error = std::string("q3a_debug_set: unknown key '") + key + "'";
  return 1;
}

int32_t q3a_selftest_gemm(int32_t device, int32_t M, int32_t N, int32_t K, int32_t split, float* max_abs_err,
                          float* ref_abs_max) {
  q3a_engine* e = nullptr;
  Q3A_TRY(e)
  int n_dev = 0;
  if (hipGetDeviceCount(&n_dev) != hipSuccess || n_dev == 0) fail("no HIP device available");
  HIPCHK(hipSetDevice(device));
  std::vector<float> X((size_t)M * K);
  std::vector<uint16_t> W((size_t)N * K);
  uint32_t st = 12345u;
  auto rnd = [&]() { st = st * 1664525u + 1013904223u; return ((st >> 8) & 0xffff) / 65536.0f - 0.5f; };
  for (auto& v : X) v = rnd();
  for (auto& v : W) { float f = rnd(); uint32_t u; memcpy(&u, &f, 4); v = (uint16_t)(u >> 16); }
  DevBuf dX, dW, dY, dR;
  dX.ensure(X.size() * 4); dW.ensure(W.size() * 2); dY.ensure((size_t)M * N * 4); dR.ensure((size_t)M * N * 4);
  HIPCHK(hipMemcpy(dX.p, X.data(), X.size() * 4, hipMemcpyHostToDevice));
  HIPCHK(hipMemcpy(dW.p, W.data(), W.size() * 2, hipMemcpyHostToDevice));
  GemmEpilogue ep; ep.out = dY.as<float>(); ep.ldo = N;
  KCHK(launch_gemm(dX.as<float>(), K, dW.as<uint16_t>(), M, N, K, ep, false, split != 0, nullptr));
  launch_gemm_ref(dX.as<float>(), dW.as<uint16_t>(), dR.as<float>(), M, N, K, nullptr);
  HIPCHK(hipDeviceSynchronize());
  HIPCHK(hipGetLastError());
  std::vector<float> Y((size_t)M * N), R((size_t)M * N);
  HIPCHK(hipMemcpy(Y.data(), dY.p, Y.size() * 4, hipMemcpyDeviceToHost));
  HIPCHK(hipMemcpy(R.data(), dR.p, R.size() * 4, hipMemcpyDeviceToHost));
  float me = 0.f, rm = 0.f;
  for (size_t i = 0; i < Y.size(); ++i) { me = std::max(me, std::fabs(Y[i] - R[i])); rm = std::max(rm, std::fabs(R[i])); }
  if (max_abs_err) *max_abs_err = me;
  if (ref_abs_max) *ref_abs_max = rm;
  dX.release(); dW.release(); dY.release(); dR.release();
  Q3A_CATCH(e)
}

int32_t q3a_selftest_gemm16(int32_t device, int32_t M, int32_t N, int32_t K, int32_t reps, float* max_abs_err,
                            float* ref_abs_max, float* avg_us_bf16, float* avg_us_f32) {
  q3a_engine* e = nullptr;
  Q3A_TRY(e)
  int n_dev = 0;
  if (hipGetDeviceCount(&n_dev) != hipSuccess || n_dev == 0) fail("no HIP device available");
  HIPCHK(hipSetDevice(device));
  std::vector<float> X((size_t)M * K);
  std::vector<uint16_t> W((size_t)N * K);
  uint32_t st = 777u;
  auto rnd = [&]() { st = st * 1664525u + 1013904223u; return ((st >> 8) & 0xffff) / 65536.0f - 0.5f; };
  auto trunc16 = [](float f) { uint32_t u; memcpy(&u, &f, 4); u &= 0xffff0000u; memcpy(&f, &u, 4); return f; };
  for (auto& v : X) v = trunc16(rnd());
  for (auto& v : W) { float f = rnd(); uint32_t u; memcpy(&u, &f, 4); v = (uint16_t)(u >> 16); }
  DevBuf dX, dX16, dW, dY, dR;
  dX.ensure(X.size() * 4); dX16.ensure(X.size() * 2); dW.ensure(W.size() * 2); dY.ensure((size_t)M * N * 4); dR.ensure((size_t)M * N * 4);
  HIPCHK(hipMemcpy(dX.p, X.data(), X.size() * 4, hipMemcpyHostToDevice));
  HIPCHK(hipMemcpy(dW.p, W.data(), W.size() * 2, hipMemcpyHostToDevice));
  KCHK(launch_to_bf16(dX.as<float>(), dX16.as<uint16_t>(), X.size(), nullptr));
  GemmEpilogue ep; ep.out = dY.as<float>(); ep.ldo = N;
  KCHK(launch_gemm16(dX16.as<uint16_t>(), K, dW.as<uint16_t>(), M, N, K, ep, false, nullptr));
  launch_gemm_ref(dX.as<float>(), dW.as<uint16_t>(), dR.as<float>(), M, N, K, nullptr);
  HIPCHK(hipDeviceSynchronize());
  HIPCHK(hipGetLastError());
  std::vector<float> Y((size_t)M * N), R((size_t)M * N);
  HIPCHK(hipMemcpy(Y.data(), dY.p, Y.size() * 4, hipMemcpyDeviceToHost));
  HIPCHK(hipMemcpy(R.data(), dR.p, R.size() * 4, hipMemcpyDeviceToHost));
  float me = 0.f, rm = 0.f;
  for (size_t i = 0; i < Y.size(); ++i) { me = std::max(me, std::fabs(Y[i] - R[i])); rm = std::max(rm, std::fabs(R[i])); }
  {
    const int P = 7;
    std::vector<float> bias(N), addend((size_t)P * N), resid((size_t)M * N);
    std::vector<int> rowmap(M);
    for (auto& v : bias) v = rnd();
    for (auto& v : addend) v = rnd();
    for (auto& v : resid) v = rnd();
    for (int m = 0; m < M; ++m) rowmap[m] = (m % 11 == 5) ? -1 : M - 1 - m;
    DevBuf dB, dA, dS, dM, dY2, dY16;
    dB.ensure(bias.size() * 4); dA.ensure(addend.size() * 4); dS.ensure(resid.size() * 4); dM.ensure(rowmap.size() * 4);
    dY2.ensure((size_t)M * N * 4); dY16.ensure((size_t)M * N * 2);
    HIPCHK(hipMemcpy(dB.p, bias.data(), bias.size() * 4, hipMemcpyHostToDevice));
    HIPCHK(hipMemcpy(dA.p, addend.data(), addend.size() * 4, hipMemcpyHostToDevice));
    HIPCHK(hipMemcpy(dS.p, resid.data(), resid.size() * 4, hipMemcpyHostToDevice));
    HIPCHK(hipMemcpy(dM.p, rowmap.data(), rowmap.size() * 4, hipMemcpyHostToDevice));
    HIPCHK(hipMemset(dY2.p, 0, (size_t)M * N * 4));
    GemmEpilogue e2; e2.out = dY2.as<float>(); e2.ldo = N; e2.bias = dB.as<float>(); e2.addend = dA.as<float>(); e2.addend_period = P;
    e2.rowmap = dM.as<int>(); e2.resid = dS.as<float>();
    KCHK(launch_gemm16(dX16.as<uint16_t>(), K, dW.as<uint16_t>(), M, N, K, e2, false, nullptr));
    HIPCHK(hipDeviceSynchronize());
    std::vector<float> Y2((size_t)M * N);
    HIPCHK(hipMemcpy(Y2.data(), dY2.p, Y2.size() * 4, hipMemcpyDeviceToHost));
    std::vector<char> hit(M, 0);
    for (int m = 0; m < M; ++m) {
      const int o = rowmap[m];
      if (o < 0) continue;
      hit[o] = 1;
      for (int n = 0; n < N; ++n) {
        const float want = R[(size_t)m * N + n] + bias[n] + addend[(size_t)(m % P) * N + n] + resid[(size_t)o * N + n];
        me = std::max(me, std::fabs(Y2[(size_t)o * N + n] - want));
      }
    }
    for (int o = 0; o < M; ++o)
      if (!hit[o])
        for (int n = 0; n < N; ++n)
          if (Y2[(size_t)o * N + n] != 0.f) fail("selftest_gemm16: a row dropped by the row map was written");
    auto bf = [](uint16_t h) { uint32_t u = (uint32_t)h << 16; float f; memcpy(&f, &u, 4); return f; };
    GemmEpilogue e3; e3.out16 = dY16.as<uint16_t>(); e3.ldo = N; e3.bias = dB.as<float>();
    KCHK(launch_gemm16(dX16.as<uint16_t>(), K, dW.as<uint16_t>(), M, N, K, e3, false, nullptr));
    HIPCHK(hipDeviceSynchronize());
    std::vector<uint16_t> Y16((size_t)M * N);
    HIPCHK(hipMemcpy(Y16.data(), dY16.p, Y16.size() * 2, hipMemcpyDeviceToHost));
    for (size_t i = 0; i < Y16.size(); ++i) {
      const float want = R[i] + bias[i % N];
      if (std::fabs(bf(Y16[i]) - want) > std::fabs(want) / 128.f + 1e-4f * std::max(rm, 1.f)) fail("selftest_gemm16: bf16 output with bias is off by more than an ulp");
    }
    if (N % 32 == 0) {
      GemmEpilogue e4; e4.out16 = dY16.as<uint16_t>(); e4.ldo = N / 2;
      KCHK(launch_gemm16(dX16.as<uint16_t>(), K, dW.as<uint16_t>(), M, N, K, e4, true, nullptr));
      HIPCHK(hipDeviceSynchronize());
      HIPCHK(hipMemcpy(Y16.data(), dY16.p, (size_t)M * (N / 2) * 2, hipMemcpyDeviceToHost));
      for (int m = 0; m < M; ++m)
        for (int c = 0; c < N / 2; ++c) {
          const float g = R[(size_t)m * N + (c / 16) * 32 + c % 16], u = R[(size_t)m * N + (c / 16) * 32 + 16 + c % 16];
          const float want = g / (1.f + std::exp(-g)) * u;
          if (std::fabs(bf(Y16[(size_t)m * (N / 2) + c]) - want) > std::fabs(want) / 64.f + 1e-3f * std::max(rm * rm, 1.f))
            fail("selftest_gemm16: SwiGLU epilogue is off");
        }
    }
    dB.release(); dA.release(); dS.release(); dM.release(); dY2.release(); dY16.release();
  }
  if (max_abs_err) *max_abs_err = me;
  if (ref_abs_max) *ref_abs_max = rm;
  if (reps > 0) {
    hipEvent_t a, b;
    HIPCHK(hipEventCreate(&a));
    HIPCHK(hipEventCreate(&b));
    float ms = 0.f;
    HIPCHK(hipEventRecord(a, nullptr));
    for (int r = 0; r < reps; ++r) KCHK(launch_gemm16(dX16.as<uint16_t>(), K, dW.as<uint16_t>(), M, N, K, ep, false, nullptr));
    HIPCHK(hipEventRecord(b, nullptr));
    HIPCHK(hipEventSynchronize(b));
    HIPCHK(hipEventElapsedTime(&ms, a, b));
    if (avg_us_bf16) *avg_us_bf16 = ms * 1000.f / reps;
    HIPCHK(hipEventRecord(a, nullptr));
    for (int r = 0; r < reps; ++r) KCHK(launch_gemm(dX.as<float>(), K, dW.as<uint16_t>(), M, N, K, ep, false, false, nullptr));
    HIPCHK(hipEventRecord(b, nullptr));
    HIPCHK(hipEventSynchronize(b));
    HIPCHK(hipEventElapsedTime(&ms, a, b));
    if (avg_us_f32) *avg_us_f32 = ms * 1000.f / reps;
    (void)hipEventDestroy(a);
    (void)hipEventDestroy(b);
  }
  dX.release(); dX16.release(); dW.release(); dY.release(); dR.release();
  Q3A_CATCH(e)
}

// ... 2 lines not shown
```

qwen3_asr_rs_amd/csrc/k_decode.hip:

```cpp
#include "argmax.h"

namespace q3a {

namespace {

__global__ void embed_kernel(const int* __restrict__ ids, const uint16_t* __restrict__ embed, int H, int skip_id,
                             float* __restrict__ out) {
  const int r = blockIdx.x;
  const int id = ids[r];
  if (id == skip_id) return;
  const uint2* src = reinterpret_cast<const uint2*>(embed + (size_t)id * H);
  float4* dst = reinterpret_cast<float4*>(out + (size_t)r * H);
  for (int i = threadIdx.x; i < H / 4; i += blockDim.x) {
    const uint2 v = src[i];
    dst[i] = make_float4(bf16lo(v.x), bf16hi(v.x), bf16lo(v.y), bf16hi(v.y));
  }
}

__device__ __forceinline__ void embed_row(const uint16_t* __restrict__ embed, int id, int H, float* __restrict__ x_next, int s,
                                          const NextNormOut& nn, float* red) {
  const int tid = threadIdx.x, nthr = blockDim.x;
  const uint2* src = reinterpret_cast<const uint2*>(embed + (size_t)id * H);
  float4* dst = reinterpret_cast<float4*>(x_next + (size_t)s * H);
  const int gs = nn.group_size > 0 ? nn.group_size : 32;
  const int sl = s % gs;
  uint16_t* const xw = nn.next_xw16f + (size_t)(s / gs) * nn.group_stride_x;
  float* const nss = nn.next_ss + (size_t)(s / gs) * nn.group_stride_ss;
  float ss = 0.f;
  for (int i = tid; i < H / 4; i += nthr) {
    const uint2 v = src[i];
    const float4 f = make_float4(bf16lo(v.x), bf16hi(v.x), bf16lo(v.y), bf16hi(v.y));
    dst[i] = f;
    if (nn.next_w) {
      const float4 w = reinterpret_cast<const float4*>(nn.next_w)[i];
      ss += f.x * f.x + f.y * f.y + f.z * f.z + f.w * f.w;
      uint2 pk;
      pk.x = pack_bf16x2(f.x * w.x, f.y * w.y);
      pk.y = pack_bf16x2(f.z * w.z, f.w * w.w);
      *reinterpret_cast<uint2*>(xw + skinny_frag_index(sl, 4 * i)) = pk;
    }
  }
  if (nn.next_w) {
    ss = wave_sum(ss);
    if ((tid & 63) == 0) red[tid >> 6] = ss;
    __syncthreads();
    if (tid == 0) {
      float t = 0.f;
      for (int w = 0; w < (nthr + 63) / 64; ++w) t += red[w];
      nss[sl] = t;
    }
    for (int p = 1 + tid; p < nn.nparts; p += nthr) nss[(size_t)p * 32 + sl] = 0.f;
  }
}

__global__ void set_tokens_kernel(const int* __restrict__ tok, const uint16_t* __restrict__ embed, int H,
                                  float* __restrict__ x_next, int* __restrict__ next_tok, NextNormOut nn) {
  __shared__ float red[16];
  const int s = blockIdx.x;
  const int id = tok[s];
  if (threadIdx.x == 0) next_tok[s] = id;
  embed_row(embed, id, H, x_next, s, nn, red);
}

template <typename KVT>
__global__ __launch_bounds__(256) void qknorm_rope_kv_kernel(RopeKvArgs a, int rows) {
  const int lane = threadIdx.x & 63;
  const int nvec = a.n_q + 2 * a.n_kv;
  const long vi = (long)blockIdx.x * 4 + (threadIdx.x >> 6);
  if (vi >= (long)rows * nvec) return;
  const int row = (int)(vi / nvec), hv = (int)(vi % nvec);
  float* base = a.qkv + (size_t)row * nvec * 128 + (size_t)hv * 128;
  float x1 = base[lane], x2 = base[lane + 64];
  const int pos = a.row_pos[row], seq = a.row_seq[row];
  if (hv < a.n_q) {
    head_norm_rope(x1, x2, a.q_norm, a.eps, a.cos_t, a.sin_t, pos, lane);
    if (a.q16) {
      uint16_t* q = a.q16 + (size_t)row * a.n_q * 128 + (size_t)hv * 128;
      q[lane] = (uint16_t)f32_to_bf16_bits(x1);
      q[lane + 64] = (uint16_t)f32_to_bf16_bits(x2);
    } else {
      base[lane] = x1;
      base[lane + 64] = x2;
    }
  } else {
    const bool is_k = hv < a.n_q + a.n_kv;
    const int kvh = is_k ? hv - a.n_q : hv - a.n_q - a.n_kv;
    if (is_k) head_norm_rope(x1, x2, a.k_norm, a.eps, a.cos_t, a.sin_t, pos, lane);
    KVT* c = reinterpret_cast<KVT*>(is_k ? a.kcache : a.vcache) + (((size_t)seq * a.n_kv + kvh) * a.max_ctx + pos) * 128;
    KvIo<KVT>::store(c + lane, x1);
    KvIo<KVT>::store(c + lane + 64, x2);
  }
}

template <bool LP>
__global__ __launch_bounds__(256) void argmax_partial_kernel(const float* __restrict__ logits, int V, ArgmaxPartials p) {
  __shared__ float bv[4], bs[LP ? 4 : 1];
  __shared__ int bi[4];
  const int s = blockIdx.y, tid = threadIdx.x, lane = tid & 63, wave = tid >> 6;
  const int per = (V + gridDim.x - 1) / gridDim.x;
  const int lo = blockIdx.x * per, hi = min(V, lo + per);
  const float* lg = logits + (size_t)s * V;
  ArgmaxAcc<LP> m;
  for (int i = lo + tid; i < hi; i += 256) {
    const float v = lg[i];
    if constexpr (LP) {
      if (v > m.v) m.s = lse_term(m.s, m.v, v) + 1.f;
      else m.s += lse_term(1.f, v, m.v);
    }
    if (v > m.v) { m.v = v; m.i = i; }
  }
#pragma unroll
  for (int o = 32; o > 0; o >>= 1) m.merge_lane(o);
  if (lane == 0) {
    bv[wave] = m.v; bi[wave] = m.i;
    if constexpr (LP) bs[wave] = m.s;
  }
  __syncthreads();
  if (tid == 0) {
    for (int w = 1; w < 4; ++w) m.merge(bv[w], bi[w], bs[LP ? w : 0]);
    m.store(p, s, blockIdx.x);
  }
}

template <bool LP>
__global__ __launch_bounds__(1024) void argmax_finalize_kernel(FinalizeArgs a) {
  __shared__ float bv[16], bs[LP ? 16 : 1];
  __shared__ int bi[16];
  __shared__ int tok_s;
  const int s = blockIdx.x, tid = threadIdx.x, lane = tid & 63, wave = tid >> 6;
  constexpr int FIN_PRE = 10;
  const int np = a.pos[s] + a.advance;
  const int sc = a.step_count[s];
  const int was_done = a.done[s];
  ArgmaxAcc<LP> pre[FIN_PRE];
#pragma unroll
  for (int j = 0; j < FIN_PRE; ++j) {
    const int i = tid + j * 1024;
    pre[j] = ArgmaxAcc<LP>::load(a.part, s, i < a.n_part ? i : a.n_part - 1);
  }
  float rope_v = 0.f;
  if (a.rope_cur && tid < 128) rope_v = tid < 64 ? a.cos_t[(size_t)np * 64 + tid] : a.sin_t[(size_t)np * 64 + tid - 64];
  ArgmaxAcc<LP> m;
#pragma unroll
  for (int j = 0; j < FIN_PRE; ++j) {
    const bool in = tid + j * 1024 < a.n_part;
    m.merge(in ? pre[j].v : -INFINITY, pre[j].i, LP && in ? pre[j].s : 0.f);
  }
  for (int i = tid + FIN_PRE * 1024; i < a.n_part; i += 1024) m.merge(ArgmaxAcc<LP>::load(a.part, s, i));
#pragma unroll
  for (int o = 32; o > 0; o >>= 1) m.merge_lane(o);
  if (lane == 0) {
    bv[wave] = m.v; bi[wave] = m.i;
    if constexpr (LP) bs[wave] = m.s;
  }
  __syncthreads();
  if (tid == 0) {
    for (int w = 1; w < 16; ++w) m.merge(bv[w], bi[w], bs[LP ? w : 0]);
    int idx = m.i;
    float lp = 0.f;
    if constexpr (LP) {
      lp = -logf(m.s);
      if (lp > 0.f) lp = 0.f;
    }
    if (idx < 0 || idx >= a.V) { idx = 0; lp = __int_as_float(0x7fc00000); }
    tok_s = idx;
    a.next_tok[s] = idx;
    if (sc < a.out_stride) a.out_ids[(size_t)s * a.out_stride + sc] = idx;
    if constexpr (LP) {
      if (sc < a.out_stride) a.out_lp[(size_t)s * a.out_stride + sc] = lp;
    }
    a.step_count[s] = sc + 1;
    a.pos[s] = np;
    if ((idx == a.eos0 || idx == a.eos1) && !was_done) {
      a.done[s] = 1;
      if (a.n_done) {
        const int n = atomicAdd(a.n_done, 1) + 1;
        if (n == a.n_seq && a.host_progress) __hip_atomic_store(a.host_progress + 1, 1, __ATOMIC_RELAXED, __HIP_MEMORY_SCOPE_SYSTEM);
      }
    }
    if (s == 0 && a.host_progress) __hip_atomic_store(a.host_progress, sc + 1, __ATOMIC_RELAXED, __HIP_MEMORY_SCOPE_SYSTEM);
  }
  __syncthreads();
  if (a.rope_cur && tid < 128) a.rope_cur[(size_t)s * 128 + tid] = rope_v;
  embed_row(a.embed, tok_s, a.H, a.x_next, s, a.nn, bv);
}

}

const char* launch_embed(const int* ids, int rows, const uint16_t* embed, int H, int skip_id, float* out,
                         hipStream_t s) {
  if (rows <= 0) return nullptr;
  hipLaunchKernelGGL(embed_kernel, dim3(rows), dim3(256), 0, s, ids, embed, H, skip_id, out);
  return nullptr;
}
const char* launch_set_tokens(const int* tok, int S, const uint16_t* embed, int H, float* x_next, int* next_tok,
                              hipStream_t s, const NextNormOut& nn) {
  if (nn.next_w && S > 32 && (nn.group_stride_x <= 0 || nn.group_stride_ss <= 0)) return "set_tokens: more than 32 sequences need group strides";
  hipLaunchKernelGGL(set_tokens_kernel, dim3(S), dim3(256), 0, s, tok, embed, H, x_next, next_tok, nn);
  return nullptr;
}
const char* launch_qknorm_rope_kv(const RopeKvArgs& a, int rows, bool kv_f32, hipStream_t s) {
  if (rows <= 0) return nullptr;
  const long nvec = (long)rows * (a.n_q + 2 * a.n_kv);
  const int blocks = (int)((nvec + 3) / 4);
  if (kv_f32) hipLaunchKernelGGL((qknorm_rope_kv_kernel<float>), dim3(blocks), dim3(256), 0, s, a, rows);
  else hipLaunchKernelGGL((qknorm_rope_kv_kernel<uint16_t>), dim3(blocks), dim3(256), 0, s, a, rows);
  return nullptr;
}
const char* launch_argmax_partials(const float* logits, int V, int S, const ArgmaxPartials& p, int nblk, hipStream_t s) {
  if (S <= 0) return nullptr;
  if (!p.val) return "argmax: partial buffer missing";
  if (const char* e = argmax_partials_check(p, nblk)) return e;
  if (p.sum) hipLaunchKernelGGL(argmax_partial_kernel<true>, dim3(nblk, S), dim3(256), 0, s, logits, V, p);
  else hipLaunchKernelGGL(argmax_partial_kernel<false>, dim3(nblk, S), dim3(256), 0, s, logits, V, p);
  return nullptr;
}
const char* launch_argmax_finalize(const FinalizeArgs& a, int S, hipStream_t s) {
  if (S <= 0) return nullptr;
  if (!a.part.val) return "argmax_finalize: partial buffer missing";
  if (const char* e = argmax_partials_check(a.part, a.n_part)) return e;
  if (!a.part.sum != !a.out_lp) return "argmax_finalize: part.sum and out_lp go together";
  if (a.part.sum) hipLaunchKernelGGL(argmax_finalize_kernel<true>, dim3(S), dim3(1024), 0, s, a);
  else hipLaunchKernelGGL(argmax_finalize_kernel<false>, dim3(S), dim3(1024), 0, s, a);
  return nullptr;
}

}
```

qwen3_asr_rs_amd/csrc/k_gemv.hip:

```cpp
#include <algorithm>

#include "argmax.h"


namespace q3a {

int gemv_rows_per_wave(const GemvArgs& a) {
  const int logical = (a.mode == 2) ? a.N / 2 : a.N;
  static const int mid = [] { const char* e = getenv("Q3A_GEMV_PR_MID"); return e ? atoi(e) : 2; }();
  static const int small = [] { const char* e = getenv("Q3A_GEMV_PR_SMALL"); return e ? atoi(e) : 1; }();
  if (logical >= 32768 && a.K <= 2048) return 4;
  if (logical >= 4096 || a.mode == 2) return (mid == 4 || mid == 2) ? mid : 2;
  return (small == 1 || small == 2 || small == 4) ? small : 1;
}
int gemv_blocks(const GemvArgs& a) {
  const int pr = gemv_rows_per_wave(a);
  const int rows_per_wave = (a.mode == 2) ? pr / 2 : pr;
  const int logical = (a.mode == 2) ? a.N / 2 : a.N;
  return (logical + 4 * rows_per_wave - 1) / (4 * rows_per_wave);
}

namespace {

constexpr int ATTN_F_MAX = 1024;
struct AttnTables {
  float m[ATTN_F_MAX], l[ATTN_F_MAX], f[ATTN_F_MAX];
};
__device__ __forceinline__ void attn_scales(const GemvArgs& a, int nb, AttnTables& t) {
  const int ns = a.attn_nsplit, n = nb * a.attn_heads * ns;
  for (int i = threadIdx.x; i < n; i += 256) {
    t.m[i] = a.attn_pm[i];
    t.l[i] = a.attn_pl[i];
  }
  __syncthreads();
  for (int i = threadIdx.x; i < n; i += 256) {
    const int base = (i / ns) * ns;
    float M = -INFINITY;
    for (int sp = 0; sp < ns; ++sp) M = fmaxf(M, t.m[base + sp]);
    float L = 0.f;
    for (int sp = 0; sp < ns; ++sp) {
      const float m = t.m[base + sp];
      if (m != -INFINITY) L += t.l[base + sp] * expf(m - M);
    }
    const float mi = t.m[i];
    t.f[i] = (mi == -INFINITY) ? 0.f : expf(mi - M) / L;
  }
  __syncthreads();
}
__device__ __forceinline__ void attn_combined8(const GemvArgs& a, int b, int k, const AttnTables& t, float (&x)[8]) {
  const int h = k >> 7, d = k & 127;
  const int ns = a.attn_nsplit;
  const int base = (b * a.attn_heads + h) * ns;
#pragma unroll
  for (int e = 0; e < 8; ++e) x[e] = 0.f;
  for (int sp0 = 0; sp0 < ns; sp0 += 4) {
    float4 o0[4], o1[4];
    float f[4];
#pragma unroll
    for (int j = 0; j < 4; ++j) {
      const int sp = sp0 + j, spc = sp < ns ? sp : ns - 1;
      f[j] = sp < ns ? t.f[base + spc] : 0.f;
      o0[j] = *reinterpret_cast<const float4*>(a.attn_po + (size_t)(base + spc) * 128 + d);
      o1[j] = *reinterpret_cast<const float4*>(a.attn_po + (size_t)(base + spc) * 128 + d + 4);
    }
#pragma unroll
    for (int j = 0; j < 4; ++j) {
      x[0] += o0[j].x * f[j]; x[1] += o0[j].y * f[j]; x[2] += o0[j].z * f[j]; x[3] += o0[j].w * f[j];
      x[4] += o1[j].x * f[j]; x[5] += o1[j].y * f[j]; x[6] += o1[j].z * f[j]; x[7] += o1[j].w * f[j];
    }
  }
}

template <bool FAST, int CH>
__device__ __forceinline__ void attn_merge8_ch(const GemvArgs& a, int b, int k, float (&x)[8]) {
  auto ex = [](float v) { return FAST ? __expf(v) : expf(v); };
  const int h = k >> 7, d = k & 127;
  const int ns = a.attn_nsplit;
  const int base = (b * a.attn_heads + h) * ns;
  float M = -INFINITY, L = 0.f;
#pragma unroll
  for (int e = 0; e < 8; ++e) x[e] = 0.f;
  for (int sp0 = 0; sp0 < ns; sp0 += CH) {
    float m[CH], l[CH];
    float4 o0[CH], o1[CH];
#pragma unroll
    for (int j = 0; j < CH; ++j) {
      const int sp = sp0 + j, spc = sp < ns ? sp : ns - 1;
      m[j] = a.attn_pm[base + spc];
      l[j] = a.attn_pl[base + spc];
      if (sp >= ns) m[j] = -INFINITY;
      o0[j] = *reinterpret_cast<const float4*>(a.attn_po + (size_t)(base + spc) * 128 + d);
      o1[j] = *reinterpret_cast<const float4*>(a.attn_po + (size_t)(base + spc) * 128 + d + 4);
    }
#ifndef Q3A_NO_MERGE_FENCE
    asm volatile("" ::: "memory");
#endif
    float Mn = M;
#pragma unroll
    for (int j = 0; j < CH; ++j) Mn = fmaxf(Mn, m[j]);
    if (Mn == -INFINITY) continue;
    if (sp0 > 0) {
      const float sc = (M == -INFINITY) ? 0.f : ex(M - Mn);
      L *= sc;
#pragma unroll
      for (int e = 0; e < 8; ++e) x[e] *= sc;
    }
#pragma unroll
    for (int j = 0; j < CH; ++j) {
      const float f = ex(m[j] - Mn);
      L += l[j] * f;
      x[0] += o0[j].x * f; x[1] += o0[j].y * f; x[2] += o0[j].z * f; x[3] += o0[j].w * f;
      x[4] += o1[j].x * f; x[5] += o1[j].y * f; x[6] += o1[j].z * f; x[7] += o1[j].w * f;
    }
    M = Mn;
  }
  const float inv = 1.0f / L;
#pragma unroll
  for (int e = 0; e < 8; ++e) x[e] *= inv;
}
template <bool FAST>
__device__ __forceinline__ void attn_merge8(const GemvArgs& a, int b, int k, float (&x)[8]) {
  if (a.attn_nsplit <= 4) attn_merge8_ch<FAST, 4>(a, b, k, x);
  else attn_merge8_ch<FAST, 8>(a, b, k, x);
}

template <int PR>
__device__ __forceinline__ void gemv_rows(const GemvArgs& a, int g, int (&prow)[PR]) {
#pragma unroll
  for (int i = 0; i < PR; ++i) {
    if (a.mode == 2) {
      const int j = g * (PR / 2) + (i >> 1);
      prow[i] = (j / 16) * 32 + (j % 16) + ((i & 1) ? 16 : 0);
    } else {
      prow[i] = g * PR + i;
    }
    if (prow[i] >= a.N) prow[i] = -1;
  }
}

__device__ __forceinline__ float dot8(const uint4& w, const float (&x)[8], float s) {
  f32x2_t a = f32x2_t{bf16lo(w.x), bf16hi(w.x)} * f32x2_t{x[0], x[1]};
  a += f32x2_t{bf16lo(w.y), bf16hi(w.y)} * f32x2_t{x[2], x[3]};
  a += f32x2_t{bf16lo(w.z), bf16hi(w.z)} * f32x2_t{x[4], x[5]};
  a += f32x2_t{bf16lo(w.w), bf16hi(w.w)} * f32x2_t{x[6], x[7]};
  return s + (a.x + a.y);
}

template <int NB, int PR, bool LP>
__device__ __forceinline__ void gemv_epilogue(const GemvArgs& a, int g, const int (&prow)[PR], float (&acc)[PR][NB],
                                              float (*am_v)[NB], int (*am_i)[NB], float (*am_s)[NB]) {
  const int tid = threadIdx.x, lane = tid & 63, wave = tid >> 6;
  if (a.mode == 3) {
    ArgmaxAcc<LP> m[NB];
    float lv[LP ? PR : 1][NB];
#pragma unroll
// ... 107 lines not shown
  };
  auto request_w = [&]() {
#pragma unroll
    for (int it = 0; it < KI; ++it)
#pragma unroll
      for (int i = 0; i < PR; ++i) {
        const int row = prow[i] >= 0 ? prow[i] : a.N - 1;
        wq[it][i] = ld_stream16(a.W + (size_t)row * K + kk[it]);
      }
  };
  constexpr int MCH = MF > 0 ? MF : 1;
  float mg_m[MCH], mg_l[MCH];
  float4 mg_o0[MCH], mg_o1[MCH];
  const int mg_k = lane * 8 + wave * 512;
  const bool mg_on = wave < KI && mg_k < K;
  if constexpr (ATTN && MF > 0) {
    const int kc = mg_k < K ? mg_k : 0;
    const int h = kc >> 7, d = kc & 127, ns = a.attn_nsplit, base = h * ns;
    typedef float __attribute__((ext_vector_type(4), aligned(4))) f4u_t;
#pragma unroll
    for (int j = 0; j < MCH; j += 4) {
      const f4u_t m4 = *reinterpret_cast<const f4u_t*>(a.attn_pm + base + j), l4 = *reinterpret_cast<const f4u_t*>(a.attn_pl + base + j);
#pragma unroll
      for (int e = 0; e < 4; ++e) {
        mg_m[j + e] = j + e < ns ? m4[e] : -INFINITY;
        mg_l[j + e] = l4[e];
      }
    }
#pragma unroll
    for (int j = 0; j < MCH; ++j) {
      const int spc = j < ns ? j : ns - 1;
      mg_o0[j] = *reinterpret_cast<const float4*>(a.attn_po + (size_t)(base + spc) * 128 + d);
      mg_o1[j] = *reinterpret_cast<const float4*>(a.attn_po + (size_t)(base + spc) * 128 + d + 4);
    }
    __builtin_amdgcn_sched_barrier(0);
  }
  if (RMS || XL) { request_x(); request_w(); } else { request_w(); request_x(); }
  float bv[PR], rv[PR];
#pragma unroll
  for (int i = 0; i < PR; ++i) {
    const int n = prow[i] >= 0 ? prow[i] : 0;
    bv[i] = a.bias ? a.bias[n] : 0.f;
    rv[i] = a.mode == 1 ? a.resid[n] : 0.f;
  }
  __builtin_amdgcn_sched_barrier(0);
  Q3A_STAMP_AT(a.stamp, blockIdx.x, 1);
  if constexpr (ATTN && MF > 0) {
    if (mg_on) {
      const bool fast = a.attn_fast_exp != 0;
      float Mn = -INFINITY;
#pragma unroll
      for (int j = 0; j < MCH; ++j) Mn = fmaxf(Mn, mg_m[j]);
      float L = 0.f, v[8];
#pragma unroll
      for (int e = 0; e < 8; ++e) v[e] = 0.f;
#pragma unroll
      for (int j = 0; j < MCH; ++j) {
        const float f = fast ? __expf(mg_m[j] - Mn) : expf(mg_m[j] - Mn);
        L += mg_l[j] * f;
        v[0] += mg_o0[j].x * f; v[1] += mg_o0[j].y * f; v[2] += mg_o0[j].z * f; v[3] += mg_o0[j].w * f;
        v[4] += mg_o1[j].x * f; v[5] += mg_o1[j].y * f; v[6] += mg_o1[j].z * f; v[7] += mg_o1[j].w * f;
      }
      const float inv = 1.0f / L;
#pragma unroll
      for (int e = 0; e < 8; ++e) v[e] *= inv;
      *reinterpret_cast<float4*>(x_s + mg_k) = make_float4(v[0], v[1], v[2], v[3]);
      *reinterpret_cast<float4*>(x_s + mg_k + 4) = make_float4(v[4], v[5], v[6], v[7]);
    }
    __syncthreads();
#pragma unroll
    for (int it = 0; it < KI; ++it) {
      xr[it][0] = *reinterpret_cast<const float4*>(x_s + kk[it]);
      xr[it][1] = *reinterpret_cast<const float4*>(x_s + kk[it] + 4);
    }
  } else if (ATTN) {
#pragma unroll
    for (int it = 0; it < KI; ++it) {
      if ((it & 3) == wave && kin[it]) {
        float v[8];
        if (a.attn_fast_exp) attn_merge8<true>(a, 0, kk[it], v); else attn_merge8<false>(a, 0, kk[it], v);
        *reinterpret_cast<float4*>(x_s + kk[it]) = make_float4(v[0], v[1], v[2], v[3]);
        *reinterpret_cast<float4*>(x_s + kk[it] + 4) = make_float4(v[4], v[5], v[6], v[7]);
      }
    }
    __syncthreads();
#pragma unroll
    for (int it = 0; it < KI; ++it) {
      xr[it][0] = *reinterpret_cast<const float4*>(x_s + kk[it]);
      xr[it][1] = *reinterpret_cast<const float4*>(x_s + kk[it] + 4);
    }
  }
  if constexpr (XL) {
#pragma unroll
    for (int j = 0; j < XLN; ++j) {
      const int k = (tid + j * 256) * 4;
      if (k < KI * 512) {
        *reinterpret_cast<float4*>(xl_x + k) = xl_rx[j];
        if (RMS) *reinterpret_cast<float4*>(xl_w + k) = xl_rw[j];
      }
    }
    __syncthreads();
#pragma unroll
    for (int it = 0; it < KI; ++it) {
      xr[it][0] = *reinterpret_cast<const float4*>(xl_x + kk[it]);
      xr[it][1] = *reinterpret_cast<const float4*>(xl_x + kk[it] + 4);
      if (RMS) {
        nr[it][0] = *reinterpret_cast<const float4*>(xl_w + kk[it]);
        nr[it][1] = *reinterpret_cast<const float4*>(xl_w + kk[it] + 4);
      }
    }
  }
  Q3A_STAMP_AT(a.stamp, blockIdx.x, 2);
  float x[KI][8];
  float ss = 0.f;
#pragma unroll
  for (int it = 0; it < KI; ++it) {
    const float4 v0 = xr[it][0], v1 = xr[it][1];
    const float xv[8] = {v0.x, v0.y, v0.z, v0.w, v1.x, v1.y, v1.z, v1.w};
#pragma unroll
    for (int e = 0; e < 8; ++e) x[it][e] = (K == KI * 512 || kin[it]) ? xv[e] : 0.f;
    if (RMS) {
      const float4 w0 = nr[it][0], w1 = nr[it][1];
      const float wv[8] = {w0.x, w0.y, w0.z, w0.w, w1.x, w1.y, w1.z, w1.w};
#pragma unroll
      for (int e = 0; e < 8; ++e) { ss += x[it][e] * x[it][e]; x[it][e] *= wv[e]; }
    }
  }
  float acc[PR][1];
#pragma unroll
  for (int i = 0; i < PR; ++i) acc[i][0] = 0.f;
#pragma unroll
  for (int it = 0; it < KI; ++it)
#pragma unroll
    for (int i = 0; i < PR; ++i) acc[i][0] = dot8(wq[it][i], x[it], acc[i][0]);
  if (wave == 0) asm volatile("" ::"v"(acc[0][0]));
  Q3A_STAMP_AT(a.stamp, blockIdx.x, 3);
  float rstd = 1.0f;
  if (RMS) rstd = rstd_of(wave_sum_fast(ss) / (float)K + a.eps, a.fast_math != 0);
#pragma unroll
  for (int i = 0; i < PR; ++i) acc[i][0] = wave_sum_fast(acc[i][0]) * rstd + bv[i];
  if (lane != 0) return;
  if (a.mode != 2) {
#pragma unroll
    for (int i = 0; i < PR; ++i)
      if (prow[i] >= 0) a.out[prow[i]] = acc[i][0] + rv[i];
  } else {
#pragma unroll
    for (int i = 0; i + 1 < PR; i += 2)
      if (prow[i] >= 0) a.out[g * (PR / 2) + (i >> 1)] = silu_sel(acc[i][0], a.fast_math != 0) * acc[i + 1][0];
  }
  Q3A_STAMP_AT(a.stamp, blockIdx.x, 4);
}

template <int PR, int KI, bool LP = false>
__device__ __forceinline__ void gemv1_head_block(const GemvArgs& a, int blk, float (&am_v)[4][1], int (&am_i)[4][1], float* am_s,
                                                 ArgmaxAcc<LP>& out) {
  const int tid = threadIdx.x, lane = tid & 63, wave = tid >> 6;
  const int K = a.K;
  const int g = blk * 4 + wave;
  int prow[PR];
  gemv_rows<PR>(a, g, prow);
  bool kin[KI];
  int kk[KI];
#pragma unroll
  for (int it = 0; it < KI; ++it) {
    const int k = lane * 8 + it * 512;
    kin[it] = k < K;
    kk[it] = kin[it] ? k : 0;
  }
  float4 xr[KI][2], nr[KI][2];
  uint4 wq[KI][PR];
#pragma unroll
  for (int it = 0; it < KI; ++it) {
    xr[it][0] = *reinterpret_cast<const float4*>(a.x + kk[it]);
    xr[it][1] = *reinterpret_cast<const float4*>(a.x + kk[it] + 4);
    nr[it][0] = *reinterpret_cast<const float4*>(a.rms_w + kk[it]);
    nr[it][1] = *reinterpret_cast<const float4*>(a.rms_w + kk[it] + 4);
  }
#pragma unroll
  for (int it = 0; it < KI; ++it)
#pragma unroll
    for (int i = 0; i < PR; ++i) {
      const int row = prow[i] >= 0 ? prow[i] : a.N - 1;
      wq[it][i] = ld_stream16(a.W + (size_t)row * K + kk[it]);
    }
  float bv[PR];
#pragma unroll
  for (int i = 0; i < PR; ++i) bv[i] = a.bias ? a.bias[prow[i] >= 0 ? prow[i] : 0] : 0.f;
  __builtin_amdgcn_sched_barrier(0);
  float x[KI][8];
  float ss = 0.f;
#pragma unroll
  for (int it = 0; it < KI; ++it) {
    const float4 v0 = xr[it][0], v1 = xr[it][1];
    const float xv[8] = {v0.x, v0.y, v0.z, v0.w, v1.x, v1.y, v1.z, v1.w};
#pragma unroll
    for (int e = 0; e < 8; ++e) x[it][e] = (K == KI * 512 || kin[it]) ? xv[e] : 0.f;
    const float4 w0 = nr[it][0], w1 = nr[it][1];
    const float wv[8] = {w0.x, w0.y, w0.z, w0.w, w1.x, w1.y, w1.z, w1.w};
#pragma unroll
    for (int e = 0; e < 8; ++e) { ss += x[it][e] * x[it][e]; x[it][e] *= wv[e]; }
  }
  float acc[PR];
#pragma unroll
  for (int i = 0; i < PR; ++i) acc[i] = 0.f;
#pragma unroll
  for (int it = 0; it < KI; ++it)
#pragma unroll
    for (int i = 0; i < PR; ++i) acc[i] = dot8(wq[it][i], x[it], acc[i]);
  const float rstd = rstd_of(wave_sum_fast(ss) / (float)K + a.eps, a.fast_math != 0);
#pragma unroll
  for (int i = 0; i < PR; ++i) acc[i] = wave_sum_fast(acc[i]) * rstd + bv[i];
  ArgmaxAcc<LP> m;
#pragma unroll
  for (int i = 0; i < PR; ++i) {
    if (prow[i] < 0) continue;
    if (lane == 0 && a.out) a.out[prow[i]] = acc[i];
    if (acc[i] > m.v) { m.v = acc[i]; m.i = prow[i]; }
  }
  if (lane == 0) { am_v[wave][0] = m.v; am_i[wave][0] = m.i; }
  if constexpr (LP) {
    float ws = 0.f;
#pragma unroll
    for (int i = 0; i < PR; ++i) ws += prow[i] < 0 ? 0.f : lse_term(1.f, acc[i], m.v);
    if (lane == 0) am_s[wave] = ws;
  }
  __syncthreads();
  if (tid == 0) {
    out = {am_v[0][0], am_i[0][0], LP ? am_s[0] : 0.f};
    for (int w = 1; w < 4; ++w) out.merge(am_v[w][0], am_i[w][0], LP ? am_s[w] : 0.f);
  }
}

template <int PR, int KI, bool LP = false>
__global__ __launch_bounds__(256) void gemv1_head_kernel(GemvArgs a) {
  __shared__ float am_v[4][1];
  __shared__ int am_i[4][1];
  __shared__ float am_s[LP ? 4 : 1];
  ArgmaxAcc<LP> r;
  gemv1_head_block<PR, KI, LP>(a, blockIdx.x, am_v, am_i, am_s, r);
  if (threadIdx.x == 0) r.store(a.part, 0, blockIdx.x);
}

struct LmHeadArgsDev {
  GemvArgs g;
  const int8_t* Wq; const float* qs; int qcols;
  float gamma;
  float* blk_lo; float* blk_hi; int n_blk;
  float* dbg;
  int* stats;
};

__device__ __forceinline__ float dotq8(uint32_t lo, uint32_t hi, const float (&x)[8], float s) {
  f32x2_t a = f32x2_t{(float)(int8_t)lo, (float)(int8_t)(lo >> 8)} * f32x2_t{x[0], x[1]};
  a += f32x2_t{(float)(int8_t)(lo >> 16), (float)((int32_t)lo >> 24)} * f32x2_t{x[2], x[3]};
  a += f32x2_t{(float)(int8_t)hi, (float)(int8_t)(hi >> 8)} * f32x2_t{x[4], x[5]};
  a += f32x2_t{(float)(int8_t)(hi >> 16), (float)((int32_t)hi >> 24)} * f32x2_t{x[6], x[7]};
  return s + (a.x + a.y);
}

__global__ __launch_bounds__(256) void lm_head_quantize_kernel(const uint16_t* W, int N, int K, int cols, int8_t* Q, float* qs) {
  const int lane = threadIdx.x & 63, r = blockIdx.x * 4 + (threadIdx.x >> 6);
  if (r >= N) return;
  const uint16_t* w = W + (size_t)r * K;
  float m = 0.f;
  for (int k = lane; k < K; k += 64) m = fmaxf(m, fabsf(__uint_as_float((uint32_t)w[k] << 16)));
  m = wave_max(m);
  const bool fin = isfinite(m);
  const float s = fin ? (float)((double)m / 127.0) : 0.f;
  double dn = 0.0, wn = 0.0, qn = 0.0;
  for (int k = lane; k < K; k += 64) {
    const double v = __uint_as_float((uint32_t)w[k] << 16);
    const double q = s > 0.f ? fmin(127.0, fmax(-127.0, rint(v / (double)s))) : 0.0;
    Q[(size_t)r * cols + ((k % 512) / 8) * (cols / 64) + (k / 512) * 8 + k % 8] = (int8_t)q;
    const double e = v - (double)s * q;
    dn += e * e; wn += v * v; qn += q * q;
  }
#pragma unroll
  for (int o = 32; o >= 1; o >>= 1) {
    dn += __shfl_xor(dn, o); wn += __shfl_xor(wn, o); qn += __shfl_xor(qn, o);
  }
  if (lane == 0) {
    auto up = [](double v) {
      v *= 1.0 + 0x1p-40;
      const float f = (float)v;
      return (double)f < v ? nextafterf(f, INFINITY) : f;
    };
    float4 o = make_float4(s, up(sqrt(dn)), up(sqrt(wn)), up((double)s * sqrt(qn)));
    if (!fin || !isfinite(o.y) || !isfinite(o.z)) o = make_float4(0.f, INFINITY, INFINITY, 0.f);
    reinterpret_cast<float4*>(qs)[r] = o;
  }
}

template <int KI>
__global__ __launch_bounds__(256) void lm_head_approx_kernel(LmHeadArgsDev p) {
  constexpr int R = 16, NQ = KI / 2;
  const GemvArgs& a = p.g;
  const int lane = threadIdx.x & 63, wave = threadIdx.x >> 6;
  const int K = a.K, blk = blockIdx.x * 4 + wave;
  if (blk >= p.n_blk) return;
  bool kin[KI];
  int kk[KI];
#pragma unroll
  for (int it = 0; it < KI; ++it) {
    const int k = lane * 8 + it * 512;
    kin[it] = k < K;
    kk[it] = kin[it] ? k : 0;
  }
  float4 xr[KI][2], nr[KI][2];
#pragma unroll
  for (int it = 0; it < KI; ++it) {
    xr[it][0] = *reinterpret_cast<const float4*>(a.x + kk[it]);
    xr[it][1] = *reinterpret_cast<const float4*>(a.x + kk[it] + 4);
    nr[it][0] = *reinterpret_cast<const float4*>(a.rms_w + kk[it]);
    nr[it][1] = *reinterpret_cast<const float4*>(a.rms_w + kk[it] + 4);
  }
  uint4 wq[R][NQ];
#pragma unroll
  for (int i = 0; i < R; ++i) {
    const int r = blk * R + i, row = r < a.N ? r : a.N - 1;
#pragma unroll
    for (int j = 0; j < NQ; ++j) wq[i][j] = ld_stream16(p.Wq + (size_t)row * p.qcols + lane * (KI * 8) + j * 16);
  }
  const int my_r = blk * R + lane;
  const bool my_valid = lane < R && my_r < a.N;
  const float4 q = reinterpret_cast<const float4*>(p.qs)[my_valid ? my_r : 0];
  __builtin_amdgcn_sched_barrier(0);
  float x[KI][8];
  float ss = 0.f, yy = 0.f;
#pragma unroll
  for (int it = 0; it < KI; ++it) {
    const float4 v0 = xr[it][0], v1 = xr[it][1];
    const float xv[8] = {v0.x, v0.y, v0.z, v0.w, v1.x, v1.y, v1.z, v1.w};
#pragma unroll
    for (int e = 0; e < 8; ++e) x[it][e] = (K == KI * 512 || kin[it]) ? xv[e] : 0.f;
    const float4 w0 = nr[it][0], w1 = nr[it][1];
    const float wv[8] = {w0.x, w0.y, w0.z, w0.w, w1.x, w1.y, w1.z, w1.w};
#pragma unroll
    for (int e = 0; e < 8; ++e) { ss += x[it][e] * x[it][e]; x[it][e] *= wv[e]; }
#pragma unroll
    for (int e = 0; e < 8; ++e) yy += x[it][e] * x[it][e];
  }
  float acc[R];
#pragma unroll
  for (int i = 0; i < R; ++i) {
    acc[i] = 0.f;
#pragma unroll
    for (int j = 0; j < NQ; ++j) {
      acc[i] = dotq8(wq[i][j].x, wq[i][j].y, x[2 * j], acc[i]);
      acc[i] = dotq8(wq[i][j].z, wq[i][j].w, x[2 * j + 1], acc[i]);
    }
  }
  const float rstd = rstd_of(wave_sum_fast(ss) / (float)K + a.eps, a.fast_math != 0);
  const float ny = sqrtf(wave_sum_fast(yy));
  float mine = 0.f;
#pragma unroll
  for (int i = 0; i < R; ++i) {
    const float t = wave_sum_fast(acc[i]);
    if (lane == i) mine = t;
  }
  const float av = (mine * q.x) * rstd;
  const float ev = (rstd * ny) * (q.y + p.gamma * (q.z + q.w)) * (1.0f + 0x1p-10f) + fabsf(av) * 0x1p-20f + 1e-30f;
  float lo = -INFINITY, hi = -INFINITY;
  if (my_valid) {
    lo = av - ev;
    hi = av + ev;
    if (!(lo <= hi) || hi == INFINITY) { lo = -INFINITY; hi = INFINITY; }
    if (p.dbg) { p.dbg[(size_t)my_r * 2] = av; p.dbg[(size_t)my_r * 2 + 1] = ev; }
  }
  lo = wave_max(lo);
  hi = wave_max(hi);
  if (lane == 0) { p.blk_lo[blk] = lo; p.blk_hi[blk] = hi; }
}

template <int PR, int KI>
__global__ __launch_bounds__(256) void lm_head_rescore_kernel(LmHeadArgsDev p) {
  __shared__ float am_v[4][1];
  __shared__ int am_i[4][1];
  __shared__ float red[4];
  __shared__ int cand[256];
  constexpr int PRE = 10;
  const int tid = threadIdx.x, lane = tid & 63, wave = tid >> 6;
  const int nb = p.n_blk, n4 = (nb + 3) / 4, G = gridDim.x;
  const float4* lo4 = reinterpret_cast<const float4*>(p.blk_lo);
  float4 lv[PRE];
#pragma unroll
  for (int j = 0; j < PRE; ++j) {
    const int i4 = tid + j * 256;
    lv[j] = lo4[i4 < n4 ? i4 : n4 - 1];
  }
  const int mb = blockIdx.x + tid * G;
  const float hv = p.blk_hi[mb < nb ? mb : nb - 1];
  float t = -INFINITY;
  auto fold = [&](const float4& v, int i4) {
    const int i = i4 * 4;
    if (i < nb) t = fmaxf(t, v.x);
    if (i + 1 < nb) t = fmaxf(t, v.y);
    if (i + 2 < nb) t = fmaxf(t, v.z);
    if (i + 3 < nb) t = fmaxf(t, v.w);
  };
#pragma unroll
  for (int j = 0; j < PRE; ++j) fold(lv[j], tid + j * 256);
  for (int i4 = tid + PRE * 256; i4 < n4; i4 += 256) fold(lo4[i4], i4);
  t = wave_max(t);
  if (lane == 0) red[wave] = t;
  cand[tid] = 0;
  __syncthreads();
  const float T = fmaxf(fmaxf(red[0], red[1]), fmaxf(red[2], red[3]));
  if (mb < nb) cand[tid] = !(hv < T);
  __syncthreads();
  const int nj = (nb - blockIdx.x + G - 1) / G;
  ArgmaxAcc<false> best;
  int nc = 0;
  for (int j = 0; j < nj; ++j) {
    if (!cand[j]) continue;
    ArgmaxAcc<false> r;
    gemv1_head_block<PR, KI>(p.g, blockIdx.x + j * G, am_v, am_i, nullptr, r);
    if (tid == 0) best.merge(r);
    ++nc;
    __syncthreads();
  }
  if (tid == 0) {
    best.store(p.g.part, 0, blockIdx.x);
    if (p.stats) {
      if (nc) atomicAdd(&p.stats[0], nc);
      if (blockIdx.x == 0) atomicAdd(&p.stats[1], 1);
    }
  }
}

template <int NB, int PR, int PF, bool LP = false>
__global__ __launch_bounds__(256) void gemvn_kernel(GemvArgs a) {
  extern __shared__ __attribute__((aligned(16))) float xs[];
  __shared__ float red[NB][4];
  __shared__ float am_v[4][NB];
  __shared__ int am_i[4][NB];
  __shared__ float am_s[LP ? 4 : 1][NB];
  const int tid = threadIdx.x, lane = tid & 63, wave = tid >> 6;
  const int K = a.K;
  const int g = blockIdx.x * 4 + wave;
  int prow[PR];
  gemv_rows<PR>(a, g, prow);
  uint4 wq[PF][PR];
#pragma unroll
  for (int it = 0; it < PF; ++it) {
    const int k = lane * 8 + it * 512;
#pragma unroll
    for (int i = 0; i < PR; ++i)
      wq[it][i] = ld_stream16(a.W + (size_t)(prow[i] >= 0 ? prow[i] : a.N - 1) * K + (k < K ? k : 0));
  }
  __shared__ AttnTables f_s;
  if (a.attn_po) attn_scales(a, NB, f_s);
#pragma unroll
  for (int b = 0; b < NB; ++b) {
    float ss = 0.f;
    for (int k = tid * 8; k < K; k += 2048) {
      float x[8];
      if (a.attn_po) {
        attn_combined8(a, b, k, f_s, x);
      } else {
        const float4 v0 = *reinterpret_cast<const float4*>(a.x + (size_t)b * a.ldx + k);
        const float4 v1 = *reinterpret_cast<const float4*>(a.x + (size_t)b * a.ldx + k + 4);
        x[0] = v0.x; x[1] = v0.y; x[2] = v0.z; x[3] = v0.w; x[4] = v1.x; x[5] = v1.y; x[6] = v1.z; x[7] = v1.w;
      }
      if (a.rms_w) {
        const float4 w0 = *reinterpret_cast<const float4*>(a.rms_w + k);
        const float4 w1 = *reinterpret_cast<const float4*>(a.rms_w + k + 4);
        const float wv[8] = {w0.x, w0.y, w0.z, w0.w, w1.x, w1.y, w1.z, w1.w};
#pragma unroll
        for (int e = 0; e < 8; ++e) { ss += x[e] * x[e]; x[e] *= wv[e]; }
      }
      *reinterpret_cast<float4*>(xs + (size_t)b * K + k) = make_float4(x[0], x[1], x[2], x[3]);
      *reinterpret_cast<float4*>(xs + (size_t)b * K + k + 4) = make_float4(x[4], x[5], x[6], x[7]);
    }
    if (a.rms_w) {
      ss = wave_sum_fast(ss);
      if (lane == 0) red[b][wave] = ss;
    }
  }
  __syncthreads();
  float acc[PR][NB];
#pragma unroll
  for (int i = 0; i < PR; ++i)
#pragma unroll
    for (int b = 0; b < NB; ++b) acc[i][b] = 0.f;
  auto fma_all = [&](const uint4 (&w)[PR], int k) {
#pragma unroll
    for (int b = 0; b < NB; ++b) {
      const float4 xa = *reinterpret_cast<const float4*>(xs + (size_t)b * K + k);
      const float4 xb = *reinterpret_cast<const float4*>(xs + (size_t)b * K + k + 4);
      const float x[8] = {xa.x, xa.y, xa.z, xa.w, xb.x, xb.y, xb.z, xb.w};
#pragma unroll
      for (int i = 0; i < PR; ++i) acc[i][b] = dot8(w[i], x, acc[i][b]);
    }
  };
#pragma unroll
  for (int it = 0; it < PF; ++it) {
    const int k = lane * 8 + it * 512;
    if (k < K) fma_all(wq[it], k);
  }
  for (int k = lane * 8 + PF * 512; k < K; k += 512) {
    uint4 w[PR];
#pragma unroll
    for (int i = 0; i < PR; ++i)
      w[i] = ld_stream16(a.W + (size_t)(prow[i] >= 0 ? prow[i] : a.N - 1) * K + k);
    fma_all(w, k);
  }
#pragma unroll
  for (int b = 0; b < NB; ++b) {
    float rstd = 1.0f;
    if (a.rms_w) rstd = rstd_of((red[b][0] + red[b][1] + red[b][2] + red[b][3]) / (float)K + a.eps, a.fast_math != 0);
#pragma unroll
    for (int i = 0; i < PR; ++i) acc[i][b] = wave_sum_fast(acc[i][b]) * rstd;
  }
  gemv_epilogue<NB, PR, LP>(a, g, prow, acc, am_v, am_i, am_s);
}

template <int PR, int KI>
void launch1k(const GemvArgs& a, hipStream_t s) {
  const dim3 grid(gemv_blocks(a)), block(256);
  if (a.attn_po) {
    if constexpr (KI <= 4) {
      if (a.attn_nsplit <= 4) { hipLaunchKernelGGL((gemv1_kernel<PR, KI, false, true, 4>), grid, block, 0, s, a); return; }
      if (a.attn_nsplit <= 8) { hipLaunchKernelGGL((gemv1_kernel<PR, KI, false, true, 8>), grid, block, 0, s, a); return; }
    }
    hipLaunchKernelGGL((gemv1_kernel<PR, KI, false, true>), grid, block, 0, s, a);
  } else if (a.rms_w) {
    if (a.mode == 3) {
      if (a.part.sum) hipLaunchKernelGGL((gemv1_head_kernel<PR, KI, true>), grid, block, 0, s, a);
      else hipLaunchKernelGGL((gemv1_head_kernel<PR, KI>), grid, block, 0, s, a);
      return;
    }
    if constexpr (KI == 2) { hipLaunchKernelGGL((gemv1_kernel<PR, KI, true, false, 0, true>), grid, block, 0, s, a); return; }
    hipLaunchKernelGGL((gemv1_kernel<PR, KI, true, false>), grid, block, 0, s, a);
  } else {
    hipLaunchKernelGGL((gemv1_kernel<PR, KI, false, false>), grid, block, 0, s, a);
  }
}
template <int PR>
void launch1(const GemvArgs& a, hipStream_t s) {
  if (a.K <= 1024) launch1k<PR, 2>(a, s);
  else if (a.K <= 2048) launch1k<PR, 4>(a, s);
  else if constexpr (PR < 4) {
    if (a.K <= 3072) launch1k<PR, 6>(a, s); else launch1k<PR, 12>(a, s);
  }
}
template <int NB, int PR, int PF>
void launchn(const GemvArgs& a, hipStream_t s) {
  if (a.part.sum) hipLaunchKernelGGL((gemvn_kernel<NB, PR, PF, true>), dim3(gemv_blocks(a)), dim3(256), (size_t)NB * a.K * sizeof(float), s, a);
  else hipLaunchKernelGGL((gemvn_kernel<NB, PR, PF>), dim3(gemv_blocks(a)), dim3(256), (size_t)NB * a.K * sizeof(float), s, a);
}

}

static LmHeadArgsDev lm_head_dev_args(const LmHeadPruneArgs& a) {
  LmHeadArgsDev p{};
  p.g = a.g; p.Wq = a.Wq; p.qs = a.qs; p.qcols = a.qcols; p.blk_lo = a.blk_lo; p.blk_hi = a.blk_hi; p.n_blk = lm_head_prune_blocks(a.g);
  p.dbg = a.dbg; p.stats = a.stats;
  const double nu = (double)a.qcols * 0x1p-24;
  p.gamma = (float)(nu / (1.0 - nu)) * (1.0f + 0x1p-20f);
  return p;
}
int lm_head_prune_blocks(const GemvArgs& g) { return (g.N + 15) / 16; }
const char* launch_lm_head_quantize(const uint16_t* W, int N, int K, int8_t* Q, float* qs, hipStream_t s) {
  const int cols = lm_head_q_cols(K);
  if (cols == 0 || K % 8 != 0) return "lm_head_quantize: hidden size beyond the one-sequence GEMV";
  if (hipMemsetAsync(Q, 0, (size_t)N * cols, s) != hipSuccess) return "lm_head_quantize: memset failed";
  hipLaunchKernelGGL(lm_head_quantize_kernel, dim3((N + 3) / 4), dim3(256), 0, s, W, N, K, cols, Q, qs);
  return nullptr;
}
const char* lm_head_prune_check(const LmHeadPruneArgs& a) {
  const GemvArgs& g = a.g;
  if (g.mode != 3 || !g.rms_w || !g.x || g.attn_po || g.bias) return "lm_head_prune: needs the plain mode-3 GEMV with a fused norm";
  if (g.part.sum) return "lm_head_prune: token log-probabilities need every logit (the full GEMV)";
  if (gemv_rows_per_wave(g) != 4 || gemv_blocks(g) != lm_head_prune_blocks(g)) return "lm_head_prune: the GEMV does not run 16-row blocks here";
  if (g.K % 8 != 0 || a.qcols != lm_head_q_cols(g.K)) return "lm_head_prune: int8 row width does not match the hidden size";
  if (!a.Wq || !a.qs || !a.blk_lo || !a.blk_hi || !g.part.val) return "lm_head_prune: missing buffer";
  if (const char* e = argmax_partials_check(g.part, 1)) return e;
  return nullptr;
}
const char* launch_lm_head_approx(const LmHeadPruneArgs& a, hipStream_t s) {
  if (const char* e = lm_head_prune_check(a)) return e;
  const LmHeadArgsDev p = lm_head_dev_args(a);
  const dim3 grid((p.n_blk + 3) / 4), block(256);
  if (a.qcols == 1024) hipLaunchKernelGGL(lm_head_approx_kernel<2>, grid, block, 0, s, p);
  else hipLaunchKernelGGL(lm_head_approx_kernel<4>, grid, block, 0, s, p);
  return nullptr;
}
int lm_head_rescore_groups(const GemvArgs& g, int n_cu) {
  const int nb = lm_head_prune_blocks(g);
  return std::min(nb, std::max(n_cu > 0 ? n_cu : 256, (nb + 255) / 256));
}
const char* launch_lm_head_rescore(const LmHeadPruneArgs& a, int groups, hipStream_t s) {
  if (const char* e = lm_head_prune_check(a)) return e;
  const LmHeadArgsDev p = lm_head_dev_args(a);
  if (groups < 1 || groups > a.g.part.stride || (p.n_blk + groups - 1) / groups > 256) return "lm_head_prune: bad rescore grid";
  if (a.qcols == 1024) hipLaunchKernelGGL((lm_head_rescore_kernel<4, 2>), dim3(groups), dim3(256), 0, s, p);
  else hipLaunchKernelGGL((lm_head_rescore_kernel<4, 4>), dim3(groups), dim3(256), 0, s, p);
  return nullptr;
}

const char* launch_gemv(const GemvArgs& a0, int NB, hipStream_t s) {
  if (a0.K % 8 != 0) return "gemv: K must be a multiple of 8";
  if (a0.K > 6144) return "gemv: K > 6144 unsupported";
  if (a0.mode == 2 && a0.N % 32 != 0) return "gemv: GLU needs N % 32 == 0";
  if (a0.mode == 3 && !a0.rms_w) return "gemv: mode 3 (the lm_head) needs the fused final norm";
  if (a0.mode == 3 && !a0.part.val) return "gemv: argmax partial buffer missing";
  if (const char* e = argmax_partials_check(a0.part, a0.mode == 3 ? gemv_blocks(a0) : 0)) return e;
  if (a0.part.sum && a0.mode != 3) return "gemv: log-sum partials need mode 3";
  if (a0.attn_po && (a0.K % 128 != 0 || a0.K != a0.attn_heads * 128)) return "gemv: attention-partial input needs K = heads*128";
  if (a0.attn_po && a0.rms_w) return "gemv: attention-partial input cannot be combined with a fused RMSNorm";
  if (a0.attn_po && (NB < 4 ? NB : 4) * a0.attn_heads * a0.attn_nsplit > ATTN_F_MAX) return "gemv: too many attention splits for the LDS scale table";
  const int pr = gemv_rows_per_wave(a0);
  const int nb_cap = (int)((64 * 1024) / ((size_t)a0.K * 4));
  int done = 0;
  while (done < NB) {
    GemvArgs a = a0;
    if (a0.x) a.x = a0.x + (size_t)done * a0.ldx;
    if (a0.out) a.out = a0.out + (size_t)done * a0.ldo;
    if (a0.resid) a.resid = a0.resid + (size_t)done * a0.ldo;
    a.part = a0.part.at(done);
    if (a0.attn_po) {
      const size_t adv = (size_t)done * a0.attn_heads * a0.attn_nsplit;
      a.attn_pm = a0.attn_pm + adv; a.attn_pl = a0.attn_pl + adv; a.attn_po = a0.attn_po + adv * 128;
    }
    int nb = NB - done;
    if (nb >= 4 && nb_cap >= 4) nb = 4;
    else if (nb >= 2 && nb_cap >= 2) nb = 2;
    else nb = 1;
    if (nb == 1) {
      if (pr == 4) launch1<4>(a, s); else if (pr == 2) launch1<2>(a, s); else launch1<1>(a, s);
    } else if (nb == 2) {
      if (pr == 4) launchn<2, 4, 2>(a, s); else if (pr == 2) launchn<2, 2, 4>(a, s); else launchn<2, 1, 6>(a, s);
    } else {
      if (pr == 4) launchn<4, 4, 2>(a, s); else if (pr == 2) launchn<4, 2, 4>(a, s); else launchn<4, 1, 6>(a, s);
    }
    done += nb;
  }
  return nullptr;
}

}
```

qwen3_asr_rs_amd/csrc/kernels.h:

```cpp
#pragma once
#include <hip/hip_runtime.h>
#include <stdint.h>

#include <atomic>

#ifndef Q3A_STAMP_FIELD
#ifdef Q3A_STAMP
#define Q3A_STAMP_FIELD unsigned long long* stamp = nullptr;
#else
#define Q3A_STAMP_FIELD
#endif
#endif

namespace q3a {

struct ArgmaxPartials {
  float* val = nullptr;
  int* idx = nullptr;
  float* sum = nullptr;
  int stride = 0;
  ArgmaxPartials at(size_t rows) const {
    const size_t o = rows * stride;
    return {val ? val + o : nullptr, idx ? idx + o : nullptr, sum ? sum + o : nullptr, stride};
  }
};
inline const char* argmax_partials_check(const ArgmaxPartials& p, int n_part) {
  if (!p.val != !p.idx) return "argmax partials: val and idx go together";
  if (p.sum && !p.val) return "argmax partials: the log-sum channel needs val and idx";
  if (p.val && p.stride < n_part) return "argmax partials: buffer too small";
  return nullptr;
}

struct AlignHeadArgs {
  const float* x; int ldx;
  const int* rows; int M;
  const float* norm_w; float eps;
  const uint16_t* W; int N; int K;
  int planes;
  uint16_t* xn;
  ArgmaxPartials part;
  int* classes;
  float* logits; int ldl;
};
int align_rows_padded(int M);
int align_head_parts(int N);
const char* launch_align_head(const AlignHeadArgs& a, hipStream_t s);

struct GemmEpilogue {
  float* out = nullptr;
  uint16_t* out16 = nullptr;
  int ldo = 0;
  const float* bias = nullptr;
  int act = 0;
  const float* resid = nullptr;
  const int* rowmap = nullptr;
  const float* addend = nullptr;
  int addend_period = 1;
  ArgmaxPartials part;
  Q3A_STAMP_FIELD
};
const char* launch_gemm(const float* X, int lda, const uint16_t* W, int M, int N, int K, const GemmEpilogue& ep,
                        bool glu, bool split, hipStream_t s);
const char* launch_conv3x3s2_gemm(const float* X, int imgs, int H, int Wd, int C, const uint16_t* Wt, int Cout,
                                  const GemmEpilogue& ep, bool split, hipStream_t s);
void launch_gemm_ref(const float* X, const uint16_t* W, float* Y, int M, int N, int K, hipStream_t s);
const char* launch_gemm16(const uint16_t* X, int lda, const uint16_t* W, int M, int N, int K, const GemmEpilogue& ep,
                          bool glu, hipStream_t s);
const char* launch_conv3x3s2_gemm16(const uint16_t* X, const uint16_t* zero_page, int imgs, int H, int Wd, int C,
                                    const uint16_t* Wt, int Cout, const GemmEpilogue& ep, hipStream_t s);
bool gemm256_eligible(int M, int N, int K);
const char* launch_gemm16_small(const uint16_t* X, int lda, const uint16_t* W, int M, int N, int K, const GemmEpilogue& ep,
                                bool glu, hipStream_t s);
struct Knobs {
  std::atomic<int> gemm256_min_tiles{128};
  std::atomic<int> gemm256_persist{1};
  std::atomic<int> gemm256_group_m{0};
  std::atomic<int> dattn_batched_min_wgs{128};
  std::atomic<int> decode_group_size{0};
  std::atomic<int> decode_parallel_groups{1};
  std::atomic<int> fuse_qkrope{1};
  std::atomic<int> skinny_q{1};
  std::atomic<int> eos_run_ahead{1};
  std::atomic<int> skinny_glu_hp3{1};
  std::atomic<int> lm_head_prune{1};
};
Knobs& knobs();
const char* launch_gemm256(const uint16_t* X, int lda, const uint16_t* W, int M, int N, int K, const GemmEpilogue& ep,
                           bool glu, hipStream_t s);
const char* launch_conv3x3s2_gemm256(const uint16_t* X, const uint16_t* zero_page, int imgs, int H, int Wd, int C,
                                     const uint16_t* Wt, int Cout, const GemmEpilogue& ep, hipStream_t s);
const char* launch_to_bf16(const float* x, uint16_t* y, size_t n, hipStream_t s);
const char* launch_from_bf16(const uint16_t* x, float* y, size_t n, hipStream_t s);

struct MelBatch {
  const float* pcm;
  const int64_t* pcm_off;
  const int64_t* n_samples;
  const int64_t* mel_off;
  const int* n_frames;
  float* mel;
  unsigned* gmax_key;
};
const char* launch_mel(const MelBatch& mb, int B, int max_frames, const float* dft ,
                       const float* filt_t , hipStream_t s);

struct ChunkTable {
  const int* chunk_utt;
  const int* chunk_frame0;
};
const char* launch_conv1(const float* mel, const int64_t* mel_off, const int* n_frames, const ChunkTable& ct,
                         int n_chunks, int n_mels, int chunk_frames, const float* w ,
                         const float* b, int Cout, float* out, hipStream_t s, uint16_t* out16 = nullptr);

const char* launch_layernorm(const float* x, const float* w, const float* b, float* y, int rows, int D, float eps,
                             hipStream_t s, uint16_t* y16 = nullptr);
const char* launch_rmsnorm(const float* x, const float* w, float* y, int rows, int D, float eps, hipStream_t s,
                           uint16_t* y16 = nullptr);

struct AttnSeg {
  int q_row0;
  int len;
  int64_t kv_off;
};
struct AttnArgs {
  const float* q; int q_rs;
  const uint16_t* q16;
  const void* k; const void* v; int64_t kv_hs; int kv_rs;
  float* o; int o_rs;
  uint16_t* o16;
  const AttnSeg* segs; int n_segs; int max_len;
  int n_kv_heads;
  float scale_div;
};
const char* launch_attn_enc(const AttnArgs& a, hipStream_t s);
const char* launch_attn_prefill(const AttnArgs& a, int group, bool kv_f32, hipStream_t s);
const char* launch_fattn_enc(const AttnArgs& a, hipStream_t s);
const char* launch_fattn_prefill(const AttnArgs& a, int group, hipStream_t s);

const char* launch_embed(const int* ids, int rows, const uint16_t* embed, int H, int skip_id, float* out, hipStream_t s);
struct RopeKvArgs {
  float* qkv;
  const int* row_seq;
  const int* row_pos;
  const float* q_norm; const float* k_norm; float eps;
  const float* cos_t; const float* sin_t;
  void* kcache; void* vcache;
  int n_q, n_kv, max_ctx;
  uint16_t* q16;
};
const char* launch_qknorm_rope_kv(const RopeKvArgs& a, int rows, bool kv_f32, hipStream_t s);
int gemm256_split_rows(int M, int N);
const char* launch_gemm256_qkrope(const uint16_t* X, int lda, const uint16_t* W, int M, int K, const float* bias,
                                  const RopeKvArgs& a, hipStream_t s);
const char* launch_gather_rows(const float* src, const int* row_idx, int n, int D, float* dst, hipStream_t s);
const char* launch_scatter_rows(const float* src, const int* dst_row, int n, int D, float* dst, hipStream_t s);

struct GemvArgs {
  const float* x; int ldx;
  const float* rms_w;
  float eps;
  const uint16_t* W; int N; int K;
  const float* bias;
  int mode;
  float* out; int ldo;
  const float* resid;
  ArgmaxPartials part;
  const float* attn_pm; const float* attn_pl; const float* attn_po; int attn_nsplit; int attn_heads;
  int attn_fast_exp;
  int fast_math;
  Q3A_STAMP_FIELD
};
const char* launch_gemv(const GemvArgs& a, int NB, hipStream_t s);
constexpr int GEMV_ATTN_MAX_TABLE = 1024;
int gemv_blocks(const GemvArgs& a);
int gemv_rows_per_wave(const GemvArgs& a);

struct LmHeadPruneArgs {
  GemvArgs g;
  const int8_t* Wq; int qcols;
  const float* qs;
  float* blk_lo; float* blk_hi;
  float* dbg;
  int* stats;
};
inline int lm_head_q_cols(int hidden) { return hidden <= 1024 ? 1024 : hidden <= 2048 ? 2048 : 0; }
const char* launch_lm_head_quantize(const uint16_t* W, int N, int K, int8_t* Q, float* qs, hipStream_t s);
int lm_head_prune_blocks(const GemvArgs& g);
int lm_head_rescore_groups(const GemvArgs& g, int n_cu);
const char* lm_head_prune_check(const LmHeadPruneArgs& a);
const char* launch_lm_head_approx(const LmHeadPruneArgs& a, hipStream_t s);
const char* launch_lm_head_rescore(const LmHeadPruneArgs& a, int groups, hipStream_t s);

struct SkinnyArgs {
  const float* x; int ldx; int S;
  const uint16_t* x16;
  int x16_frag;
  int out16_frag;
  const float* rms_w; float eps;
  const uint16_t* W; int N; int K;
  const float* bias;
  int mode;
  float* out; int ldo;
  uint16_t* out16;
  const float* resid;
  const uint16_t* xw16f; const float* ss_parts; int ss_nparts;
  const float* next_w; uint16_t* next_xw16f; float* next_ss;
  int qsplit;
  int qs_halves;
  int glu_hp3;
  int n_cu;
  int fast_math;
  Q3A_STAMP_FIELD
};
struct NextNormOut {
  const float* next_w;
  uint16_t* next_xw16f;
  float* next_ss;
  int nparts;
  long group_stride_x, group_stride_ss;
  int group_size;
};
const char* launch_skinny(const SkinnyArgs& a, bool split, hipStream_t s);
const char* skinny_init();
__host__ __device__ inline size_t skinny_frag_index(int s, int k) {
  return ((((size_t)(k >> 5) * 2 + (s >> 4)) * 4 + ((k >> 3) & 3)) * 16 + (s & 15)) * 8 + (k & 7);
}

struct DecodeAttnArgs {
  const float* qkv;
  const int* pos;
  const float* q_norm; const float* k_norm; float eps;
  const float* rope_cur;
  void* kcache; void* vcache;
  float* pm; float* pl;
  float* po;
  int nsplit;
  int n_q, n_kv, max_ctx;
  float scale_div;
  float* out;
  uint16_t* out16;
  int out_frag;
  int trim_prologue;
  Q3A_STAMP_FIELD
};
#ifndef Q3A_DATTN_SPLIT_KEYS
#define Q3A_DATTN_SPLIT_KEYS 128
#endif
constexpr int DATTN_KEYS_PER_SPLIT_BF16 = Q3A_DATTN_SPLIT_KEYS, DATTN_KEYS_PER_SPLIT_F32 = 128;
inline int dattn_keys_per_split(bool kv_f32) { return kv_f32 ? DATTN_KEYS_PER_SPLIT_F32 : DATTN_KEYS_PER_SPLIT_BF16; }
const char* launch_decode_attn(const DecodeAttnArgs& a, int S, bool kv_f32, hipStream_t s);
const char* launch_decode_attn_batched(const DecodeAttnArgs& a, int S, bool kv_f32, hipStream_t s);
const char* launch_attn_combine(const float* pm, const float* pl, const float* po, int nsplit, int S, int n_q, float* out,
                                hipStream_t s, uint16_t* out16 = nullptr, bool frag = false);

struct FinalizeArgs {
  ArgmaxPartials part;
  int n_part;
  int V;
  int* next_tok;
  int* out_ids;
  int out_stride;
  int* step_count;
  int* pos;
  int advance;
  uint8_t* done;
  int* n_done;
  int n_seq;
  int* host_progress;
  const uint16_t* embed; int H;
  float* x_next;
  int eos0, eos1;
  const float* cos_t; const float* sin_t;
  float* rope_cur;
  NextNormOut nn;
  float* out_lp;
};
const char* launch_argmax_partials(const float* logits, int V, int S, const ArgmaxPartials& p, int nblk, hipStream_t s);
const char* launch_argmax_finalize(const FinalizeArgs& a, int S, hipStream_t s);
const char* launch_set_tokens(const int* tok, int S, const uint16_t* embed, int H, float* x_next, int* next_tok, hipStream_t s,
                              const NextNormOut& nn = NextNormOut{});

}
```

Measured before the change: 486.0 audio-seconds/sec.

## Fuse LM-head candidate rescoring with argmax finalize in one select kernel

Adds an lm_head_select kernel that takes the int8 approximate LM-head bounds, gathers the candidate vocabulary rows whose upper bound reaches the threshold, rescans them exactly in bf16 and commits the token directly. If few rows survive, one workgroup does the work. Otherwise the work is spread across CUs and the last block to arrive on an atomic counter does the reduction. This replaces the separate rescore and argmax_finalize launches on each decode step, cutting launch and sync overhead. It depends on an atomic arrival counter and extra per-row and per-group bound buffers, and it only applies when no log-prob channel is requested.

```diff
diff --git a/qwen3_asr_rs_amd/build.py b/qwen3_asr_rs_amd/build.py
--- a/qwen3_asr_rs_amd/build.py
+++ b/qwen3_asr_rs_amd/build.py
@@ -18,7 +18,7 @@
 
 SOURCES = ["engine.cpp", "model.cpp", "k_gemm.hip", "k_mel.hip", "k_conv1.hip", "k_norm.hip", "k_attn.hip", "k_decode.hip", "k_gemv.hip", "k_dattn.hip", "k_fattn.hip", "k_skinny.hip", "k_gemm16.hip", "k_gemm256.hip", "k_peaks.hip", "k_align.hip",
            "host_audio.cpp", "host_text.cpp", "host_abi.cpp", "host_align.cpp", "group.cpp", "ops.cpp", "k_ops.hip"]
-HEADERS = ["dev.h", "kernels.h", "argmax.h", "model.h", "json.h", "host.h", "ops.h", "unicode_tables.h", os.path.join("..", "..", "include", "q3asr.h"),
+HEADERS = ["dev.h", "kernels.h", "argmax.h", "finalize.h", "model.h", "json.h", "host.h", "ops.h", "unicode_tables.h", os.path.join("..", "..", "include", "q3asr.h"),
            os.path.join("..", "..", "include", "q3asr_ops.h")]
 HIPCC = os.environ.get("HIPCC", "/opt/rocm/bin/hipcc")
 FLAGS = ["--offload-arch=gfx950", "-O3", "-std=c++17", "-fPIC", "-fno-slp-vectorize", "-Wall", "-Wno-unused-function", "-Wno-unused-variable"]
diff --git a/qwen3_asr_rs_amd/csrc/engine.cpp b/qwen3_asr_rs_amd/csrc/engine.cpp
--- a/qwen3_asr_rs_amd/csrc/engine.cpp
+++ b/qwen3_asr_rs_amd/csrc/engine.cpp
@@ -96,6 +96,7 @@
     env("Q3A_EOS_RUN_AHEAD", k.eos_run_ahead);
     env("Q3A_SKINNY_GLU_HP3", k.skinny_glu_hp3);
     env("Q3A_LM_HEAD_PRUNE", k.lm_head_prune);
+    env("Q3A_LM_HEAD_SELECT", k.lm_head_select);
   });
   return k;
 }
@@ -136,6 +137,9 @@
   DevBuf lm_q, lm_qs;
   int lm_q_cols = 0;
   DevBuf prune_stats;
+  DevBuf row_hi, grp_lo, grp_hi;
+  DevBuf sel_stats;
+  DevBuf sel_arrive;
   DevBuf attn_pm, attn_pl, attn_po;
   DevBuf nn_x, nn_ss;
   DevBuf rope_cur;
@@ -150,7 +154,7 @@
   size_t kv_layer_elems = 0;
 
   int gsize = 32;
-  int k_parallel_groups = 1, k_skinny_q = 1, k_dattn_batched_min_wgs = 128, k_skinny_glu_hp3 = 1, k_lm_head_prune = 1;
+  int k_parallel_groups = 1, k_skinny_q = 1, k_dattn_batched_min_wgs = 128, k_skinny_glu_hp3 = 1, k_lm_head_prune = 1, k_lm_head_select = 1;
   std::vector<hipStream_t> chain_streams;
   std::vector<hipEvent_t> join_ev;
   hipEvent_t fork_ev = nullptr;
@@ -250,6 +254,10 @@
     n_done.ensure(64);
     prune_stats.ensure(8);
     HIPCHK(hipMemsetAsync(prune_stats.p, 0, 8, stream));
+    sel_stats.ensure(16);
+    HIPCHK(hipMemsetAsync(sel_stats.p, 0, 16, stream));
+    sel_arrive.ensure(64);
+    HIPCHK(hipMemsetAsync(sel_arrive.p, 0, 64, stream));
   }
 
   void init_tables() {
@@ -660,6 +668,7 @@
       k_dattn_batched_min_wgs = kn.dattn_batched_min_wgs.load();
       k_skinny_glu_hp3 = kn.skinny_glu_hp3.load();
       k_lm_head_prune = kn.lm_head_prune.load();
+      k_lm_head_select = kn.lm_head_select.load();
     }
     const size_t ng = (size_t)n_groups(b);
     nn_x.ensure(ng * 32 * H * 2); nn_ss.ensure((size_t)ng * (H / 8) * 32 * 4);
@@ -673,6 +682,7 @@
     {
       const size_t nblk4 = ((size_t)(d.vocab + 15) / 16 + 3) & ~size_t(3);
       blk_lo.ensure(nblk4 * 4); blk_hi.ensure(nblk4 * 4);
+      row_hi.ensure((size_t)d.vocab * 4); grp_lo.ensure(nblk4); grp_hi.ensure(nblk4);
     }
     attn_nsplit = (max_ctx + dattn_keys_per_split(kv_f32()) - 1) / dattn_keys_per_split(kv_f32());
     attn_pm.ensure((size_t)b * d.n_q * attn_nsplit * 4); attn_pl.ensure((size_t)b * d.n_q * attn_nsplit * 4);
@@ -696,7 +706,7 @@
 
   std::vector<DevBuf*> step_bufs() {
     return {&kcache, &vcache, &x_dec, &d_pos, &next_tok, &out_ids, &step_count, &done, &s_ln, &s_qkv, &s_ctx, &s_act, &logits,
-            &part_val, &part_idx, &part_sum, &out_lp, &blk_lo, &blk_hi, &prune_stats, &attn_pm, &attn_pl, &attn_po, &nn_x, &nn_ss, &rope_cur, &rope_cos, &rope_sin, &n_done, &forced_tok};
+            &part_val, &part_idx, &part_sum, &out_lp, &blk_lo, &blk_hi, &prune_stats, &row_hi, &grp_lo, &grp_hi, &sel_stats, &sel_arrive, &attn_pm, &attn_pl, &attn_po, &nn_x, &nn_ss, &rope_cur, &rope_cos, &rope_sin, &n_done, &forced_tok};
   }
   std::vector<const DevBuf*> step_bufs() const {
     auto v = const_cast<q3a_engine*>(this)->step_bufs();
@@ -710,6 +720,7 @@
     LmHeadPruneArgs pa{};
     pa.g = g; pa.Wq = lm_q.as<int8_t>(); pa.qcols = lm_q_cols; pa.qs = lm_qs.as<float>();
     pa.blk_lo = blk_lo.as<float>(); pa.blk_hi = blk_hi.as<float>(); pa.stats = prune_stats.as<int>();
+    if (k_lm_head_select) { pa.row_hi = row_hi.as<float>(); pa.grp_lo = grp_lo.as<float>(); pa.grp_hi = grp_hi.as<float>(); }
     return pa;
   }
 
@@ -719,6 +730,13 @@
     const double wbytes = 2.0 * V * H;
     int n_part = 0;
     const ArgmaxPartials part{part_val.as<float>(), part_idx.as<int>(), token_lp() ? part_sum.as<float>() : nullptr, part_stride};
+    FinalizeArgs f{};
+    f.part = part; f.out_lp = part.sum ? out_lp.as<float>() : nullptr;
+    f.V = V; f.next_tok = next_tok.as<int>(); f.out_ids = out_ids.as<int>();
+    f.out_stride = max_new; f.step_count = step_count.as<int>(); f.pos = d_pos.as<int>(); f.advance = advance;
+    f.done = done.as<uint8_t>(); f.n_done = n_done.as<int>(); f.n_seq = S; f.host_progress = host_prog_dev; f.embed = wh(L.embed); f.H = H; f.x_next = x_dec.as<float>(); f.eos0 = kEos0; f.eos1 = kEos1;
+    f.cos_t = rope_cos.as<float>(); f.sin_t = rope_sin.as<float>(); f.rope_cur = rope_cur.as<float>();
+    f.nn = first_layer_norm_out();
     if (S <= kGemvMaxSeq) {
       GemvArgs g{};
       g.fast_math = precise() ? 0 : 1;
@@ -737,6 +755,15 @@
       }
       if (prunable && k_lm_head_prune && !head_logits_) {
         g.out = nullptr; pa.g.out = nullptr;
+        LmHeadSelectArgs sel{};
+        sel.groups = lm_head_select_groups(part, n_cu); sel.stats = sel_stats.as<int>();
+        sel.arrive = sel_arrive.as<unsigned int>(); sel.force_dist = k_lm_head_select == 2;
+        f.n_part = sel.groups;
+        if (k_lm_head_select && !lm_head_select_check(pa, f, sel)) {
+          timed(Q3A_KC_GEMV_LM_HEAD, (double)V * lm_q_cols, [&] { KCHK(launch_lm_head_approx(pa, stream)); });
+          timed(Q3A_KC_ARGMAX, 0, [&] { KCHK(launch_lm_head_select(pa, f, sel, stream)); });
+          return;
+        }
         n_part = lm_head_rescore_groups(g, n_cu);
         timed(Q3A_KC_GEMV_LM_HEAD, (double)V * lm_q_cols, [&] { KCHK(launch_lm_head_approx(pa, stream)); });
         timed(Q3A_KC_ARGMAX, 0, [&] { KCHK(launch_lm_head_rescore(pa, n_part, stream)); });
@@ -763,13 +790,7 @@
       n_part = 128;
       timed(Q3A_KC_ARGMAX, 0, [&] { KCHK(launch_argmax_partials(logits.as<float>(), V, S, part, n_part, stream)); });
     }
-    FinalizeArgs f{};
-    f.part = part; f.n_part = n_part; f.out_lp = part.sum ? out_lp.as<float>() : nullptr;
-    f.V = V; f.next_tok = next_tok.as<int>(); f.out_ids = out_ids.as<int>();
-    f.out_stride = max_new; f.step_count = step_count.as<int>(); f.pos = d_pos.as<int>(); f.advance = advance;
-    f.done = done.as<uint8_t>(); f.n_done = n_done.as<int>(); f.n_seq = S; f.host_progress = host_prog_dev; f.embed = wh(L.embed); f.H = H; f.x_next = x_dec.as<float>(); f.eos0 = kEos0; f.eos1 = kEos1;
-    f.cos_t = rope_cos.as<float>(); f.sin_t = rope_sin.as<float>(); f.rope_cur = rope_cur.as<float>();
-    f.nn = first_layer_norm_out();
+    f.n_part = n_part;
     timed(Q3A_KC_ARGMAX, 0, [&] { KCHK(launch_argmax_finalize(f, S, stream)); });
   }
 
@@ -1085,8 +1106,8 @@
       for (int i = 0; i < 8; ++i) { h ^= (v >> (8 * i)) & 0xff; h *= 1099511628211ull; }
     }
     char buf[256];
-    snprintf(buf, sizeof(buf), "%d.%d.%d.%d.%d.%d.%d.%d.%d.%d/%d/%d/%d/%p/%016llx", B, gsize, k_parallel_groups, k_skinny_q,
-             k_dattn_batched_min_wgs, k_skinny_glu_hp3, k_lm_head_prune, (int)(min_P_ < 256), (int)head_logits_, (int)token_lp(), live_nsplit_,
+    snprintf(buf, sizeof(buf), "%d.%d.%d.%d.%d.%d.%d.%d.%d.%d.%d/%d/%d/%d/%p/%016llx", B, gsize, k_parallel_groups, k_skinny_q,
+             k_dattn_batched_min_wgs, k_skinny_glu_hp3, k_lm_head_prune, k_lm_head_select, (int)(min_P_ < 256), (int)head_logits_, (int)token_lp(), live_nsplit_,
              max_ctx, max_new, (const void*)arena, (unsigned long long)h);
     return buf;
   }
@@ -1761,6 +1782,15 @@
     }
     return 0;
   }
+  if (strcmp(name, "lm_head_select_stats") == 0) {
+    if (actual) *actual = 16;
+    if (dst) {
+      if (bytes < 16) fail("q3a_debug_read: destination too small");
+      HIPCHK(hipStreamSynchronize(e->stream));
+      HIPCHK(hipMemcpy(dst, e->sel_stats.p, 16, hipMemcpyDeviceToHost));
+    }
+    return 0;
+  }
   if (strcmp(name, "align_head_ms") == 0) {
     if (actual) *actual = 4;
     if (dst) {
@@ -1795,6 +1825,7 @@
   if (strcmp(key, "eos_run_ahead") == 0) { kn.eos_run_ahead = value; return 0; }
   if (strcmp(key, "skinny_glu_hp3") == 0) { kn.skinny_glu_hp3 = value; return 0; }
   if (strcmp(key, "lm_head_prune") == 0) { kn.lm_head_prune = value; return 0; }
+  if (strcmp(key, "lm_head_select") == 0) { kn.lm_head_select = value; return 0; }
   g_last_error = std::string("q3a_debug_set: unknown key '") + key + "'";
   return 1;
 }
diff --git a/qwen3_asr_rs_amd/csrc/finalize.h b/qwen3_asr_rs_amd/csrc/finalize.h
--- /dev/null
+++ b/qwen3_asr_rs_amd/csrc/finalize.h
@@ -0,0 +1,87 @@
+#pragma once
+#include "argmax.h"
+
+namespace q3a {
+
+__device__ __forceinline__ void embed_row(const uint16_t* __restrict__ embed, int id, int H, float* __restrict__ x_next, int s,
+                                          const NextNormOut& nn, float* red) {
+  const int tid = threadIdx.x, nthr = blockDim.x;
+  const uint2* src = reinterpret_cast<const uint2*>(embed + (size_t)id * H);
+  float4* dst = reinterpret_cast<float4*>(x_next + (size_t)s * H);
+  const int gs = nn.group_size > 0 ? nn.group_size : 32;
+  const int sl = s % gs;
+  uint16_t* const xw = nn.next_xw16f + (size_t)(s / gs) * nn.group_stride_x;
+  float* const nss = nn.next_ss + (size_t)(s / gs) * nn.group_stride_ss;
+  float ss = 0.f;
+  for (int i = tid; i < H / 4; i += nthr) {
+    const uint2 v = src[i];
+    const float4 f = make_float4(bf16lo(v.x), bf16hi(v.x), bf16lo(v.y), bf16hi(v.y));
+    dst[i] = f;
+    if (nn.next_w) {
+      const float4 w = reinterpret_cast<const float4*>(nn.next_w)[i];
+      ss += f.x * f.x + f.y * f.y + f.z * f.z + f.w * f.w;
+      uint2 pk;
+      pk.x = pack_bf16x2(f.x * w.x, f.y * w.y);
+      pk.y = pack_bf16x2(f.z * w.z, f.w * w.w);
+      *reinterpret_cast<uint2*>(xw + skinny_frag_index(sl, 4 * i)) = pk;
+    }
+  }
+  if (nn.next_w) {
+    ss = wave_sum(ss);
+    if ((tid & 63) == 0) red[tid >> 6] = ss;
+    __syncthreads();
+    if (tid == 0) {
+      float t = 0.f;
+      for (int w = 0; w < (nthr + 63) / 64; ++w) t += red[w];
+      nss[sl] = t;
+    }
+    for (int p = 1 + tid; p < nn.nparts; p += nthr) nss[(size_t)p * 32 + sl] = 0.f;
+  }
+}
+
+struct FinSeq {
+  int np, sc, was_done;
+};
+__device__ __forceinline__ FinSeq fin_seq_load(const FinalizeArgs& a, int s) { return {a.pos[s] + a.advance, a.step_count[s], a.done[s]}; }
+__device__ __forceinline__ float fin_rope_load(const FinalizeArgs& a, int np) {
+  const int tid = threadIdx.x;
+  float rope_v = 0.f;
+  if (a.rope_cur && tid < 128) rope_v = tid < 64 ? a.cos_t[(size_t)np * 64 + tid] : a.sin_t[(size_t)np * 64 + tid - 64];
+  return rope_v;
+}
+
+template <bool LP>
+__device__ __forceinline__ void finalize_commit(const FinalizeArgs& a, int s, const ArgmaxAcc<LP>& m, const FinSeq& q, float rope_v,
+                                                int& tok_s, float* red) {
+  const int tid = threadIdx.x;
+  if (tid == 0) {
+    int idx = m.i;
+    float lp = 0.f;
+    if constexpr (LP) {
+      lp = -logf(m.s);
+      if (lp > 0.f) lp = 0.f;
+    }
+    if (idx < 0 || idx >= a.V) { idx = 0; lp = __int_as_float(0x7fc00000); }
+    tok_s = idx;
+    a.next_tok[s] = idx;
+    if (q.sc < a.out_stride) a.out_ids[(size_t)s * a.out_stride + q.sc] = idx;
+    if constexpr (LP) {
+      if (q.sc < a.out_stride) a.out_lp[(size_t)s * a.out_stride + q.sc] = lp;
+    }
+    a.step_count[s] = q.sc + 1;
+    a.pos[s] = q.np;
+    if ((idx == a.eos0 || idx == a.eos1) && !q.was_done) {
+      a.done[s] = 1;
+      if (a.n_done) {
+        const int n = atomicAdd(a.n_done, 1) + 1;
+        if (n == a.n_seq && a.host_progress) __hip_atomic_store(a.host_progress + 1, 1, __ATOMIC_RELAXED, __HIP_MEMORY_SCOPE_SYSTEM);
+      }
+    }
+    if (s == 0 && a.host_progress) __hip_atomic_store(a.host_progress, q.sc + 1, __ATOMIC_RELAXED, __HIP_MEMORY_SCOPE_SYSTEM);
+  }
+  __syncthreads();
+  if (a.rope_cur && tid < 128) a.rope_cur[(size_t)s * 128 + tid] = rope_v;
+  embed_row(a.embed, tok_s, a.H, a.x_next, s, a.nn, red);
+}
+
+}
diff --git a/qwen3_asr_rs_amd/csrc/k_decode.hip b/qwen3_asr_rs_amd/csrc/k_decode.hip
--- a/qwen3_asr_rs_amd/csrc/k_decode.hip
+++ b/qwen3_asr_rs_amd/csrc/k_decode.hip
@@ -1,4 +1,4 @@
-#include "argmax.h"
+#include "finalize.h"
 
 namespace q3a {
 
@@ -14,42 +14,6 @@
   for (int i = threadIdx.x; i < H / 4; i += blockDim.x) {
     const uint2 v = src[i];
     dst[i] = make_float4(bf16lo(v.x), bf16hi(v.x), bf16lo(v.y), bf16hi(v.y));
-  }
-}
-
-__device__ __forceinline__ void embed_row(const uint16_t* __restrict__ embed, int id, int H, float* __restrict__ x_next, int s,
-                                          const NextNormOut& nn, float* red) {
-  const int tid = threadIdx.x, nthr = blockDim.x;
-  const uint2* src = reinterpret_cast<const uint2*>(embed + (size_t)id * H);
-  float4* dst = reinterpret_cast<float4*>(x_next + (size_t)s * H);
-  const int gs = nn.group_size > 0 ? nn.group_size : 32;
-  const int sl = s % gs;
-  uint16_t* const xw = nn.next_xw16f + (size_t)(s / gs) * nn.group_stride_x;
-  float* const nss = nn.next_ss + (size_t)(s / gs) * nn.group_stride_ss;
-  float ss = 0.f;
-  for (int i = tid; i < H / 4; i += nthr) {
-    const uint2 v = src[i];
-    const float4 f = make_float4(bf16lo(v.x), bf16hi(v.x), bf16lo(v.y), bf16hi(v.y));
-    dst[i] = f;
-    if (nn.next_w) {
-      const float4 w = reinterpret_cast<const float4*>(nn.next_w)[i];
-      ss += f.x * f.x + f.y * f.y + f.z * f.z + f.w * f.w;
-      uint2 pk;
-      pk.x = pack_bf16x2(f.x * w.x, f.y * w.y);
-      pk.y = pack_bf16x2(f.z * w.z, f.w * w.w);
-      *reinterpret_cast<uint2*>(xw + skinny_frag_index(sl, 4 * i)) = pk;
-    }
-  }
-  if (nn.next_w) {
-    ss = wave_sum(ss);
-    if ((tid & 63) == 0) red[tid >> 6] = ss;
-    __syncthreads();
-    if (tid == 0) {
-      float t = 0.f;
-      for (int w = 0; w < (nthr + 63) / 64; ++w) t += red[w];
-      nss[sl] = t;
-    }
-    for (int p = 1 + tid; p < nn.nparts; p += nthr) nss[(size_t)p * 32 + sl] = 0.f;
   }
 }
 
@@ -129,17 +93,14 @@
   __shared__ int tok_s;
   const int s = blockIdx.x, tid = threadIdx.x, lane = tid & 63, wave = tid >> 6;
   constexpr int FIN_PRE = 10;
-  const int np = a.pos[s] + a.advance;
-  const int sc = a.step_count[s];
-  const int was_done = a.done[s];
+  const FinSeq q = fin_seq_load(a, s);
   ArgmaxAcc<LP> pre[FIN_PRE];
 #pragma unroll
   for (int j = 0; j < FIN_PRE; ++j) {
     const int i = tid + j * 1024;
     pre[j] = ArgmaxAcc<LP>::load(a.part, s, i < a.n_part ? i : a.n_part - 1);
   }
-  float rope_v = 0.f;
-  if (a.rope_cur && tid < 128) rope_v = tid < 64 ? a.cos_t[(size_t)np * 64 + tid] : a.sin_t[(size_t)np * 64 + tid - 64];
+  const float rope_v = fin_rope_load(a, q.np);
   ArgmaxAcc<LP> m;
 #pragma unroll
   for (int j = 0; j < FIN_PRE; ++j) {
@@ -154,35 +115,9 @@
     if constexpr (LP) bs[wave] = m.s;
   }
   __syncthreads();
-  if (tid == 0) {
+  if (tid == 0)
     for (int w = 1; w < 16; ++w) m.merge(bv[w], bi[w], bs[LP ? w : 0]);
-    int idx = m.i;
-    float lp = 0.f;
-    if constexpr (LP) {
-      lp = -logf(m.s);
-      if (lp > 0.f) lp = 0.f;
-    }
-    if (idx < 0 || idx >= a.V) { idx = 0; lp = __int_as_float(0x7fc00000); }
-    tok_s = idx;
-    a.next_tok[s] = idx;
-    if (sc < a.out_stride) a.out_ids[(size_t)s * a.out_stride + sc] = idx;
-    if constexpr (LP) {
-      if (sc < a.out_stride) a.out_lp[(size_t)s * a.out_stride + sc] = lp;
-    }
-    a.step_count[s] = sc + 1;
-    a.pos[s] = np;
-    if ((idx == a.eos0 || idx == a.eos1) && !was_done) {
-      a.done[s] = 1;
-      if (a.n_done) {
-        const int n = atomicAdd(a.n_done, 1) + 1;
-        if (n == a.n_seq && a.host_progress) __hip_atomic_store(a.host_progress + 1, 1, __ATOMIC_RELAXED, __HIP_MEMORY_SCOPE_SYSTEM);
-      }
-    }
-    if (s == 0 && a.host_progress) __hip_atomic_store(a.host_progress, sc + 1, __ATOMIC_RELAXED, __HIP_MEMORY_SCOPE_SYSTEM);
-  }
-  __syncthreads();
-  if (a.rope_cur && tid < 128) a.rope_cur[(size_t)s * 128 + tid] = rope_v;
-  embed_row(a.embed, tok_s, a.H, a.x_next, s, a.nn, bv);
+  finalize_commit<LP>(a, s, m, q, rope_v, tok_s, bv);
 }
 
 }
diff --git a/qwen3_asr_rs_amd/csrc/k_gemv.hip b/qwen3_asr_rs_amd/csrc/k_gemv.hip
--- a/qwen3_asr_rs_amd/csrc/k_gemv.hip
+++ b/qwen3_asr_rs_amd/csrc/k_gemv.hip
@@ -1,6 +1,6 @@
 #include <algorithm>
 
-#include "argmax.h"
+#include "finalize.h"
 
 
 namespace q3a {
@@ -414,6 +414,53 @@
   Q3A_STAMP_AT(a.stamp, blockIdx.x, 4);
 }
 
+template <int KI>
+__device__ __forceinline__ void head_cols(int K, int lane, bool (&kin)[KI], int (&kk)[KI]) {
+#pragma unroll
+  for (int it = 0; it < KI; ++it) {
+    const int k = lane * 8 + it * 512;
+    kin[it] = k < K;
+    kk[it] = kin[it] ? k : 0;
+  }
+}
+template <int KI>
+__device__ __forceinline__ void head_x_issue(const GemvArgs& a, const int (&kk)[KI], float4 (&xr)[KI][2], float4 (&nr)[KI][2]) {
+#pragma unroll
+  for (int it = 0; it < KI; ++it) {
+    xr[it][0] = *reinterpret_cast<const float4*>(a.x + kk[it]);
+    xr[it][1] = *reinterpret_cast<const float4*>(a.x + kk[it] + 4);
+    nr[it][0] = *reinterpret_cast<const float4*>(a.rms_w + kk[it]);
+    nr[it][1] = *reinterpret_cast<const float4*>(a.rms_w + kk[it] + 4);
+  }
+}
+template <int KI>
+__device__ __forceinline__ void head_x_form(int K, const bool (&kin)[KI], const float4 (&xr)[KI][2], const float4 (&nr)[KI][2],
+                                            float (&x)[KI][8], float& ss) {
+  ss = 0.f;
+#pragma unroll
+  for (int it = 0; it < KI; ++it) {
+    const float4 v0 = xr[it][0], v1 = xr[it][1];
+    const float xv[8] = {v0.x, v0.y, v0.z, v0.w, v1.x, v1.y, v1.z, v1.w};
+#pragma unroll
+    for (int e = 0; e < 8; ++e) x[it][e] = (K == KI * 512 || kin[it]) ? xv[e] : 0.f;
+    const float4 w0 = nr[it][0], w1 = nr[it][1];
+    const float wv[8] = {w0.x, w0.y, w0.z, w0.w, w1.x, w1.y, w1.z, w1.w};
+#pragma unroll
+    for (int e = 0; e < 8; ++e) { ss += x[it][e] * x[it][e]; x[it][e] *= wv[e]; }
+  }
+}
+__device__ __forceinline__ float head_rstd(const GemvArgs& a, float ss) {
+  return rstd_of(wave_sum_fast(ss) / (float)a.K + a.eps, a.fast_math != 0);
+}
+template <int KI>
+__device__ __forceinline__ float head_row_dot(const uint4 (&w)[KI], const float (&x)[KI][8]) {
+  float acc = 0.f;
+#pragma unroll
+  for (int it = 0; it < KI; ++it) acc = dot8(w[it], x[it], acc);
+  return acc;
+}
+__device__ __forceinline__ float head_row_logit(float acc, float rstd, float bv) { return wave_sum_fast(acc) * rstd + bv; }
+
 template <int PR, int KI, bool LP = false>
 __device__ __forceinline__ void gemv1_head_block(const GemvArgs& a, int blk, float (&am_v)[4][1], int (&am_i)[4][1], float* am_s,
                                                  ArgmaxAcc<LP>& out) {
@@ -424,21 +471,10 @@
   gemv_rows<PR>(a, g, prow);
   bool kin[KI];
   int kk[KI];
-#pragma unroll
-  for (int it = 0; it < KI; ++it) {
-    const int k = lane * 8 + it * 512;
-    kin[it] = k < K;
-    kk[it] = kin[it] ? k : 0;
-  }
+  head_cols<KI>(K, lane, kin, kk);
   float4 xr[KI][2], nr[KI][2];
   uint4 wq[KI][PR];
-#pragma unroll
-  for (int it = 0; it < KI; ++it) {
-    xr[it][0] = *reinterpret_cast<const float4*>(a.x + kk[it]);
-    xr[it][1] = *reinterpret_cast<const float4*>(a.x + kk[it] + 4);
-    nr[it][0] = *reinterpret_cast<const float4*>(a.rms_w + kk[it]);
-    nr[it][1] = *reinterpret_cast<const float4*>(a.rms_w + kk[it] + 4);
-  }
+  head_x_issue<KI>(a, kk, xr, nr);
 #pragma unroll
   for (int it = 0; it < KI; ++it)
 #pragma unroll
@@ -451,28 +487,19 @@
   for (int i = 0; i < PR; ++i) bv[i] = a.bias ? a.bias[prow[i] >= 0 ? prow[i] : 0] : 0.f;
   __builtin_amdgcn_sched_barrier(0);
   float x[KI][8];
-  float ss = 0.f;
-#pragma unroll
-  for (int it = 0; it < KI; ++it) {
-    const float4 v0 = xr[it][0], v1 = xr[it][1];
-    const float xv[8] = {v0.x, v0.y, v0.z, v0.w, v1.x, v1.y, v1.z, v1.w};
-#pragma unroll
-    for (int e = 0; e < 8; ++e) x[it][e] = (K == KI * 512 || kin[it]) ? xv[e] : 0.f;
-    const float4 w0 = nr[it][0], w1 = nr[it][1];
-    const float wv[8] = {w0.x, w0.y, w0.z, w0.w, w1.x, w1.y, w1.z, w1.w};
-#pragma unroll
-    for (int e = 0; e < 8; ++e) { ss += x[it][e] * x[it][e]; x[it][e] *= wv[e]; }
-  }
+  float ss;
+  head_x_form<KI>(K, kin, xr, nr, x, ss);
   float acc[PR];
 #pragma unroll
-  for (int i = 0; i < PR; ++i) acc[i] = 0.f;
-#pragma unroll
-  for (int it = 0; it < KI; ++it)
-#pragma unroll
-    for (int i = 0; i < PR; ++i) acc[i] = dot8(wq[it][i], x[it], acc[i]);
-  const float rstd = rstd_of(wave_sum_fast(ss) / (float)K + a.eps, a.fast_math != 0);
-#pragma unroll
-  for (int i = 0; i < PR; ++i) acc[i] = wave_sum_fast(acc[i]) * rstd + bv[i];
+  for (int i = 0; i < PR; ++i) {
+    uint4 w[KI];
+#pragma unroll
+    for (int it = 0; it < KI; ++it) w[it] = wq[it][i];
+    acc[i] = head_row_dot<KI>(w, x);
+  }
+  const float rstd = head_rstd(a, ss);
+#pragma unroll
+  for (int i = 0; i < PR; ++i) acc[i] = head_row_logit(acc[i], rstd, bv[i]);
   ArgmaxAcc<LP> m;
 #pragma unroll
   for (int i = 0; i < PR; ++i) {
@@ -511,6 +538,8 @@
   float* blk_lo; float* blk_hi; int n_blk;
   float* dbg;
   int* stats;
+  float* row_hi;
+  float* grp_lo; float* grp_hi;
 };
 
 __device__ __forceinline__ float dotq8(uint32_t lo, uint32_t hi, const float (&x)[8], float s) {
@@ -559,24 +588,15 @@
   constexpr int R = 16, NQ = KI / 2;
   const GemvArgs& a = p.g;
   const int lane = threadIdx.x & 63, wave = threadIdx.x >> 6;
-  const int K = a.K, blk = blockIdx.x * 4 + wave;
-  if (blk >= p.n_blk) return;
+  const int K = a.K, blk0 = blockIdx.x * 4 + wave;
+  const bool live = blk0 < p.n_blk;
+  if (!live && !p.grp_lo) return;
+  const int blk = live ? blk0 : p.n_blk - 1;
   bool kin[KI];
   int kk[KI];
-#pragma unroll
-  for (int it = 0; it < KI; ++it) {
-    const int k = lane * 8 + it * 512;
-    kin[it] = k < K;
-    kk[it] = kin[it] ? k : 0;
-  }
+  head_cols<KI>(K, lane, kin, kk);
   float4 xr[KI][2], nr[KI][2];
-#pragma unroll
-  for (int it = 0; it < KI; ++it) {
-    xr[it][0] = *reinterpret_cast<const float4*>(a.x + kk[it]);
-    xr[it][1] = *reinterpret_cast<const float4*>(a.x + kk[it] + 4);
-    nr[it][0] = *reinterpret_cast<const float4*>(a.rms_w + kk[it]);
-    nr[it][1] = *reinterpret_cast<const float4*>(a.rms_w + kk[it] + 4);
-  }
+  head_x_issue<KI>(a, kk, xr, nr);
   uint4 wq[R][NQ];
 #pragma unroll
   for (int i = 0; i < R; ++i) {
@@ -585,24 +605,16 @@
     for (int j = 0; j < NQ; ++j) wq[i][j] = ld_stream16(p.Wq + (size_t)row * p.qcols + lane * (KI * 8) + j * 16);
   }
   const int my_r = blk * R + lane;
-  const bool my_valid = lane < R && my_r < a.N;
+  const bool my_valid = live && lane < R && my_r < a.N;
   const float4 q = reinterpret_cast<const float4*>(p.qs)[my_valid ? my_r : 0];
   __builtin_amdgcn_sched_barrier(0);
   float x[KI][8];
-  float ss = 0.f, yy = 0.f;
-#pragma unroll
-  for (int it = 0; it < KI; ++it) {
-    const float4 v0 = xr[it][0], v1 = xr[it][1];
-    const float xv[8] = {v0.x, v0.y, v0.z, v0.w, v1.x, v1.y, v1.z, v1.w};
-#pragma unroll
-    for (int e = 0; e < 8; ++e) x[it][e] = (K == KI * 512 || kin[it]) ? xv[e] : 0.f;
-    const float4 w0 = nr[it][0], w1 = nr[it][1];
-    const float wv[8] = {w0.x, w0.y, w0.z, w0.w, w1.x, w1.y, w1.z, w1.w};
-#pragma unroll
-    for (int e = 0; e < 8; ++e) { ss += x[it][e] * x[it][e]; x[it][e] *= wv[e]; }
+  float ss, yy = 0.f;
+  head_x_form<KI>(K, kin, xr, nr, x, ss);
+#pragma unroll
+  for (int it = 0; it < KI; ++it)
 #pragma unroll
     for (int e = 0; e < 8; ++e) yy += x[it][e] * x[it][e];
-  }
   float acc[R];
 #pragma unroll
   for (int i = 0; i < R; ++i) {
@@ -613,7 +625,7 @@
       acc[i] = dotq8(wq[i][j].z, wq[i][j].w, x[2 * j + 1], acc[i]);
     }
   }
-  const float rstd = rstd_of(wave_sum_fast(ss) / (float)K + a.eps, a.fast_math != 0);
+  const float rstd = head_rstd(a, ss);
   const float ny = sqrtf(wave_sum_fast(yy));
   float mine = 0.f;
 #pragma unroll
@@ -629,10 +641,20 @@
     hi = av + ev;
     if (!(lo <= hi) || hi == INFINITY) { lo = -INFINITY; hi = INFINITY; }
     if (p.dbg) { p.dbg[(size_t)my_r * 2] = av; p.dbg[(size_t)my_r * 2 + 1] = ev; }
+    if (p.row_hi) p.row_hi[my_r] = hi;
   }
   lo = wave_max(lo);
   hi = wave_max(hi);
-  if (lane == 0) { p.blk_lo[blk] = lo; p.blk_hi[blk] = hi; }
+  if (lane == 0 && live) { p.blk_lo[blk] = lo; p.blk_hi[blk] = hi; }
+  if (p.grp_lo) {
+    __shared__ float g_lo[4], g_hi[4];
+    if (lane == 0) { g_lo[wave] = lo; g_hi[wave] = hi; }
+    __syncthreads();
+    if (threadIdx.x == 0) {
+      p.grp_lo[blockIdx.x] = fmaxf(fmaxf(g_lo[0], g_lo[1]), fmaxf(g_lo[2], g_lo[3]));
+      p.grp_hi[blockIdx.x] = fmaxf(fmaxf(g_hi[0], g_hi[1]), fmaxf(g_hi[2], g_hi[3]));
+    }
+  }
 }
 
 template <int PR, int KI>
@@ -691,6 +713,197 @@
   }
 }
 
+constexpr int SEL_GPRE = 4;
+constexpr int SEL_GROUPS = 16;
+struct LmHeadSelectArgsDev {
+  LmHeadArgsDev p;
+  FinalizeArgs f;
+  int n_grp;
+  int* sel_stats;
+  unsigned int* arrive;
+  int force_dist;
+};
+
+__device__ __forceinline__ int wave_scan_incl(int v) {
+  const int lane = threadIdx.x & 63;
+#pragma unroll
+  for (int o = 1; o < 64; o <<= 1) {
+    const int u = __shfl_up(v, o, 64);
+    if (lane >= o) v += u;
+  }
+  return v;
+}
+
+template <int KI>
+__global__ __launch_bounds__(1024) void lm_head_select_kernel(LmHeadSelectArgsDev sa) {
+  constexpr int NW = 16, RPW = 8 / KI, ROUND = NW * RPW;
+  static_assert(SEL_GPRE * NW == 64 && SEL_GROUPS == NW, "one lane per (slab, wave) count; one group per wave");
+  const LmHeadArgsDev& p = sa.p;
+  const GemvArgs& a = p.g;
+  const FinalizeArgs& f = sa.f;
+  __shared__ int cg[SEL_GPRE * 1024];
+  __shared__ int crow[SEL_GROUPS * 64];
+  __shared__ int cnt[2 * 64];
+  __shared__ float red_v[NW];
+  __shared__ int red_i[NW];
+  __shared__ int tok_s, last_s;
+  const int tid = threadIdx.x, lane = tid & 63, wave = tid >> 6, G = gridDim.x, N = a.N, n_grp = sa.n_grp;
+  const uint64_t below = (1ull << lane) - 1;
+  const FinSeq q = fin_seq_load(f, 0);
+  float gl[SEL_GPRE], gh[SEL_GPRE];
+#pragma unroll
+  for (int j = 0; j < SEL_GPRE; ++j) {
+    const int i = tid + j * 1024, ic = i < n_grp ? i : n_grp - 1;
+    gl[j] = p.grp_lo[ic];
+    gh[j] = p.grp_hi[ic];
+  }
+  bool kin[KI];
+  int kk[KI];
+  head_cols<KI>(a.K, lane, kin, kk);
+  float4 xr[KI][2], nr[KI][2];
+  head_x_issue<KI>(a, kk, xr, nr);
+  const float rope_v = fin_rope_load(f, q.np);
+  float t = -INFINITY;
+#pragma unroll
+  for (int j = 0; j < SEL_GPRE; ++j)
+    if (tid + j * 1024 < n_grp) t = fmaxf(t, gl[j]);
+  t = wave_max(t);
+  if (lane == 0) red_v[wave] = t;
+  __syncthreads();
+  float T = red_v[0];
+#pragma unroll
+  for (int w = 1; w < NW; ++w) T = fmaxf(T, red_v[w]);
+  uint64_t gm[SEL_GPRE];
+#pragma unroll
+  for (int j = 0; j < SEL_GPRE; ++j) {
+    gm[j] = __ballot(tid + j * 1024 < n_grp && !(gh[j] < T));
+    if (lane == 0) cnt[j * NW + wave] = __popcll(gm[j]);
+  }
+  __syncthreads();
+  int n_cg;
+  {
+    const int c = cnt[lane], incl = wave_scan_incl(c);
+    n_cg = __shfl(incl, 63, 64);
+    int off[SEL_GPRE];
+#pragma unroll
+    for (int j = 0; j < SEL_GPRE; ++j) off[j] = __shfl(incl - c, j * NW + wave, 64);
+#pragma unroll
+    for (int j = 0; j < SEL_GPRE; ++j)
+      if ((gm[j] >> lane) & 1) cg[off[j] + __popcll(gm[j] & below)] = tid + j * 1024;
+  }
+  __syncthreads();
+  float x[KI][8];
+  float ss;
+  head_x_form<KI>(a.K, kin, xr, nr, x, ss);
+  const float rstd = head_rstd(a, ss);
+
+  auto gather = [&](int slot, int& nb) -> int {
+    const int grp = slot < n_cg ? cg[slot] : -1;
+    const int r = grp * 64 + lane;
+    const bool in = grp >= 0 && r < N;
+    const float h = in ? p.row_hi[r] : -INFINITY;
+    const uint64_t m = __ballot(in && !(h < T));
+    if (lane == 0) {
+      cnt[wave] = __popcll(m);
+      cnt[64 + wave] = ((m & 0xffffull) != 0) + (((m >> 16) & 0xffffull) != 0) + (((m >> 32) & 0xffffull) != 0) + ((m >> 48) != 0);
+    }
+    __syncthreads();
+    const int c = lane < NW ? cnt[lane] : 0, incl = wave_scan_incl(c);
+    nb = wave_scan_incl(lane < NW ? cnt[64 + lane] : 0);
+    nb = __shfl(nb, 63, 64);
+    const int off = __shfl(incl - c, wave, 64), rows = __shfl(incl, 63, 64);
+    if ((m >> lane) & 1) crow[off + __popcll(m & below)] = r;
+    __syncthreads();
+    return rows;
+  };
+  auto rescore = [&](int rows, ArgmaxAcc<false>& acc) {
+    for (int r0 = 0; r0 < rows; r0 += ROUND) {
+      const int k0 = r0 + wave * RPW;
+      if (k0 >= rows) break;
+      int rid[RPW];
+      uint4 w[RPW][KI];
+#pragma unroll
+      for (int i = 0; i < RPW; ++i) {
+        rid[i] = k0 + i < rows ? crow[k0 + i] : -1;
+        const int row = rid[i] >= 0 ? rid[i] : crow[k0];
+#pragma unroll
+        for (int it = 0; it < KI; ++it) w[i][it] = ld_stream16(a.W + (size_t)row * a.K + kk[it]);
+      }
+#pragma unroll
+      for (int i = 0; i < RPW; ++i) {
+        const float l = head_row_logit(head_row_dot<KI>(w[i], x), rstd, 0.f);
+        if (rid[i] >= 0 && l > -INFINITY) acc.merge(l, rid[i], 0.f);
+      }
+    }
+  };
+  auto merge_waves = [&](const ArgmaxAcc<false>& acc, ArgmaxAcc<false>& out) {
+    if (lane == 0) { red_v[wave] = acc.v; red_i[wave] = acc.i; }
+    __syncthreads();
+    if (tid == 0)
+      for (int w = 0; w < NW; ++w) out.merge(red_v[w], red_i[w], 0.f);
+  };
+
+  if (!sa.force_dist && n_cg <= SEL_GROUPS) {
+    int nb;
+    const int rows = gather(wave, nb);
+    if (rows <= ROUND) {
+      if (blockIdx.x != 0) return;
+      ArgmaxAcc<false> acc, best;
+      rescore(rows, acc);
+      merge_waves(acc, best);
+      if (tid == 0) {
+        if (p.stats) { atomicAdd(&p.stats[0], nb); atomicAdd(&p.stats[1], 1); }
+        if (sa.sel_stats) { atomicAdd(&sa.sel_stats[0], rows); atomicAdd(&sa.sel_stats[1], 1); }
+      }
+      finalize_commit<false>(f, 0, best, q, rope_v, tok_s, red_v);
+      return;
+    }
+    __syncthreads();
+  }
+  ArgmaxAcc<false> acc;
+  int my_rows = 0, my_blocks = 0;
+  for (int b = 0; blockIdx.x + b * NW * G < n_cg; ++b) {
+    int nb;
+    const int rows = gather(blockIdx.x + (b * NW + wave) * G, nb);
+    rescore(rows, acc);
+    my_rows += rows;
+    my_blocks += nb;
+  }
+  ArgmaxAcc<false> part;
+  merge_waves(acc, part);
+  if (tid == 0) {
+    part.store(f.part, 0, blockIdx.x);
+    if (p.stats && my_blocks) atomicAdd(&p.stats[0], my_blocks);
+    if (sa.sel_stats && my_rows) atomicAdd(&sa.sel_stats[0], my_rows);
+  }
+  asm volatile("s_waitcnt vmcnt(0)" ::: "memory");
+  __syncthreads();
+  if (tid == 0) {
+    __builtin_amdgcn_fence(__ATOMIC_RELEASE, "agent");
+    asm volatile("s_waitcnt vmcnt(0)" ::: "memory");
+    const unsigned int prev = __hip_atomic_fetch_add(sa.arrive, 1u, __ATOMIC_RELAXED, __HIP_MEMORY_SCOPE_AGENT);
+    const int last = prev == (unsigned int)G - 1;
+    if (last) {
+      __builtin_amdgcn_fence(__ATOMIC_ACQUIRE, "agent");
+      asm volatile("s_waitcnt vmcnt(0)" ::: "memory");
+      __hip_atomic_store(sa.arrive, 0u, __ATOMIC_RELAXED, __HIP_MEMORY_SCOPE_AGENT);
+    }
+    last_s = last;
+  }
+  __syncthreads();
+  if (!last_s) return;
+  ArgmaxAcc<false> m, best;
+  for (int i = tid; i < G; i += 1024) m.merge(ArgmaxAcc<false>::load(f.part, 0, i));
+#pragma unroll
+  for (int o = 32; o > 0; o >>= 1) m.merge_lane(o);
+  merge_waves(m, best);
+  if (tid == 0) {
+    if (p.stats) atomicAdd(&p.stats[1], 1);
+    if (sa.sel_stats) { atomicAdd(&sa.sel_stats[1], 1); atomicAdd(&sa.sel_stats[2], 1); }
+  }
+  finalize_commit<false>(f, 0, best, q, rope_v, tok_s, red_v);
+}
+
 template <int NB, int PR, int PF, bool LP = false>
 __global__ __launch_bounds__(256) void gemvn_kernel(GemvArgs a) {
   extern __shared__ __attribute__((aligned(16))) float xs[];
@@ -818,7 +1031,7 @@
 static LmHeadArgsDev lm_head_dev_args(const LmHeadPruneArgs& a) {
   LmHeadArgsDev p{};
   p.g = a.g; p.Wq = a.Wq; p.qs = a.qs; p.qcols = a.qcols; p.blk_lo = a.blk_lo; p.blk_hi = a.blk_hi; p.n_blk = lm_head_prune_blocks(a.g);
-  p.dbg = a.dbg; p.stats = a.stats;
+  p.dbg = a.dbg; p.stats = a.stats; p.row_hi = a.row_hi; p.grp_lo = a.grp_lo; p.grp_hi = a.grp_hi;
   const double nu = (double)a.qcols * 0x1p-24;
   p.gamma = (float)(nu / (1.0 - nu)) * (1.0f + 0x1p-20f);
   return p;
@@ -859,6 +1072,26 @@
   if (groups < 1 || groups > a.g.part.stride || (p.n_blk + groups - 1) / groups > 256) return "lm_head_prune: bad rescore grid";
   if (a.qcols == 1024) hipLaunchKernelGGL((lm_head_rescore_kernel<4, 2>), dim3(groups), dim3(256), 0, s, p);
   else hipLaunchKernelGGL((lm_head_rescore_kernel<4, 4>), dim3(groups), dim3(256), 0, s, p);
+  return nullptr;
+}
+
+int lm_head_select_groups(const ArgmaxPartials& part, int n_cu) { return std::max(1, std::min(n_cu > 0 ? n_cu : 256, part.stride)); }
+const char* lm_head_select_check(const LmHeadPruneArgs& a, const FinalizeArgs& f, const LmHeadSelectArgs& sel) {
+  if (const char* e = lm_head_prune_check(a)) return e;
+  if (!a.row_hi || !a.grp_lo || !a.grp_hi || !sel.arrive) return "lm_head_select: missing buffer";
+  if ((lm_head_prune_blocks(a.g) + 3) / 4 > SEL_GPRE * 1024) return "lm_head_select: vocabulary beyond the select launch";
+  if (f.part.sum || f.out_lp) return "lm_head_select: no log-sum channel";
+  if (f.part.val != a.g.part.val || f.part.idx != a.g.part.idx) return "lm_head_select: partials differ from the GEMV's";
+  if (sel.groups < 1 || sel.groups > f.part.stride) return "lm_head_select: bad grid";
+  return nullptr;
+}
+const char* launch_lm_head_select(const LmHeadPruneArgs& a, const FinalizeArgs& f, const LmHeadSelectArgs& sel, hipStream_t s) {
+  if (const char* e = lm_head_select_check(a, f, sel)) return e;
+  LmHeadSelectArgsDev d{};
+  d.p = lm_head_dev_args(a); d.f = f; d.n_grp = (d.p.n_blk + 3) / 4;
+  d.sel_stats = sel.stats; d.arrive = sel.arrive; d.force_dist = sel.force_dist;
+  if (a.qcols == 1024) hipLaunchKernelGGL(lm_head_select_kernel<2>, dim3(sel.groups), dim3(1024), 0, s, d);
+  else hipLaunchKernelGGL(lm_head_select_kernel<4>, dim3(sel.groups), dim3(1024), 0, s, d);
   return nullptr;
 }
 
diff --git a/qwen3_asr_rs_amd/csrc/kernels.h b/qwen3_asr_rs_amd/csrc/kernels.h
--- a/qwen3_asr_rs_amd/csrc/kernels.h
+++ b/qwen3_asr_rs_amd/csrc/kernels.h
@@ -83,6 +83,7 @@
   std::atomic<int> eos_run_ahead{1};
   std::atomic<int> skinny_glu_hp3{1};
   std::atomic<int> lm_head_prune{1};
+  std::atomic<int> lm_head_select{1};
 };
 Knobs& knobs();
 const char* launch_gemm256(const uint16_t* X, int lda, const uint16_t* W, int M, int N, int K, const GemmEpilogue& ep,
@@ -182,6 +183,7 @@
   float* blk_lo; float* blk_hi;
   float* dbg;
   int* stats;
+  float* row_hi; float* grp_lo; float* grp_hi;
 };
 inline int lm_head_q_cols(int hidden) { return hidden <= 1024 ? 1024 : hidden <= 2048 ? 2048 : 0; }
 const char* launch_lm_head_quantize(const uint16_t* W, int N, int K, int8_t* Q, float* qs, hipStream_t s);
@@ -277,6 +279,15 @@
 };
 const char* launch_argmax_partials(const float* logits, int V, int S, const ArgmaxPartials& p, int nblk, hipStream_t s);
 const char* launch_argmax_finalize(const FinalizeArgs& a, int S, hipStream_t s);
+struct LmHeadSelectArgs {
+  int groups;
+  int* stats;
+  unsigned int* arrive;
+  int force_dist;
+};
+int lm_head_select_groups(const ArgmaxPartials& part, int n_cu);
+const char* lm_head_select_check(const LmHeadPruneArgs& a, const FinalizeArgs& f, const LmHeadSelectArgs& sel);
+const char* launch_lm_head_select(const LmHeadPruneArgs& a, const FinalizeArgs& f, const LmHeadSelectArgs& sel, hipStream_t s);
 const char* launch_set_tokens(const int* tok, int S, const uint16_t* embed, int H, float* x_next, int* next_tok, hipStream_t s,
                               const NextNormOut& nn = NextNormOut{});
 
```

New measurement: 488.3 audio-seconds/sec (median of 5 runs). Within noise of the previous version (+0.5%).
